# zmoon/crt1d

Hardware: AMD Instinct MI355X
Metric: (column x band) solves/sec at 60 layers (higher is better)
Workload: dtype f64

## Files before the change

crt1d_amd/_lib.py:

```python

import ctypes
import os

_HERE = os.path.dirname(os.path.abspath(__file__))
LIB_PATH = os.environ.get("CRT1D_HIP_LIB") or os.path.join(_HERE, "libcrt1d_hip.so")

SCHEME_IDS = {"2s": 0, "4s": 1, "n79": 2, "zq": 3, "bl": 4, "g77": 5, "bf": 6, "zq_pa": 7}
F32_SCHEMES = ("2s", "4s", "n79", "zq", "bl", "g77", "bf", "zq_pa")
TAU_D_METHODS = {"quad": 0, "9sky": 1}
NQ_TAU, NQ_G4, NQ_9SKY = 96, 32, 9
NQ = NQ_TAU + NQ_G4 + NQ_9SKY

FLAG_SKIP_PRECOMPUTE = 1
FLAG_PRECOMPUTE_ONLY = 2
FLAG_DIRECT_STORES = 4

MAX_LEVEL_SELECT = 64

CRT_OK = 0
CRT_ERR_BAD_ARG = -1
CRT_ERR_WORKSPACE = -2
CRT_ERR_UNSUPPORTED = -3
CRT_ERR_LAUNCH = -4
CRT_ERR_SHAPE = -5

_vp = ctypes.c_void_p


class CrtColumns(ctypes.Structure):
    _fields_ = [
        ("ncol", ctypes.c_int32),
        ("nz", ctypes.c_int32),
        ("psi", _vp),
        ("lai", _vp),
        ("mla", _vp),
        ("g_kind", _vp),
        ("g_param", _vp),
        ("g_at_psi", _vp),
        ("g_table", _vp),
    ]


class CrtBands(ctypes.Structure):
    _fields_ = [
        ("nb", ctypes.c_int32),
        ("col_stride", ctypes.c_int64),
        ("I_dr0", _vp),
        ("I_df0", _vp),
        ("leaf_r", _vp),
        ("leaf_t", _vp),
        ("soil_r", _vp),
    ]


class CrtSunSeries(ctypes.Structure):

    _fields_ = [
        ("nt", ctypes.c_int32),
        ("psi", _vp),
        ("g_at_psi", _vp),
        ("col_stride", ctypes.c_int64),
        ("I_dr0", _vp),
        ("I_df0", _vp),
    ]


class CrtSunSeriesF32(CrtSunSeries):
    """crt_sun_series_f32: the layout of crt_sun_series with float I_dr0 / I_df0 behind the pointers (crt_hip_levels_series_f32)."""


NTUNE = 16

TUNE_TILE_LDS = 0
TUNE_TILE_T = 1
TUNE_TILE_FLAGS = 2
TUNE_CLOSED_STORE_WAVES = 3
TUNE_CLOSED_PIPE_T = 4
TUNE_PACK = 5
TUNE_PACK_COMPUTE_WAVES = 6
TUNE_TRI_M = 8
TUNE_TRI_T = 9
TUNE_TRI_FAMILY = 10
TUNE_TRI_STORE_WAVES = 11
TUNE_MIN_TILE_NB = 12
TUNE_FLAT_FLUSH = 13
TUNE_K0_SEPARATE = 15
TILE_FLAG_SYNC_BARRIERS = 1
TILE_FLAG_GENERIC_FLUSH = 2
TILE_FLAG_NO_PIPELINE = 4
TILE_FLAG_NO_GENERIC_PIPELINE = 8
TILE_FLAG_FOUR_PAIR_STORE = 16
PACK_OFF = 1
PACK_FORCE = 2
TRI_FAMILY_NO_PIPELINE = 1
TRI_FAMILY_DOUBLE_BUFFERED = 2
TRI_FAMILY_REG_STAGED = 3
TRI_FAMILY_GENERIC_PIPELINE = 4
TRI_FAMILY_ZQPA_TWO_KERNEL = 1
TRI_FAMILY_ZQPA_PIPE = 5
TRI_FAMILY_ZQPA_PIPE2_DB = 6
TRI_FAMILY_ZQPA_PIPE2_RS = 7
FLAT_FLUSH_OFF = 1
FLAT_FLUSH_PART_LINE = 2
FLAT_FLUSH_WHOLE_LINE = 3


class CrtOptions(ctypes.Structure):
    _fields_ = [("mu_s", ctypes.c_double), ("tau_d_method", ctypes.c_int32), ("flags", ctypes.c_int32), ("tune", ctypes.c_int32 * NTUNE)]


def set_tune(opts, tune):
    for k in tune:
        if not isinstance(k, int) or not 0 <= k < NTUNE:
            raise ValueError(f"unknown crt_options.tune key {k!r}: keys are the TUNE_* constants, 0 .. {NTUNE - 1}")
    for k in range(NTUNE):
        opts.tune[k] = int(tune.get(k, 0))
    return opts


class CrtOutputs(ctypes.Structure):
    _fields_ = [(k, _vp) for k in ("I_dr", "I_df_d", "I_df_u", "F", "x0", "x1", "x2")]


class CrtBandsumOut(ctypes.Structure):

    _fields_ = [(k, _vp) for k in ("aI", "aI_sl", "aI_sh", "totals", "aI_dr", "I_dr", "I_df_d", "I_df_u", "F", "I_d")]


ABI_VERSION = 3


def _signatures():
    P = ctypes.POINTER
    i, i32, i64, sz, dbl, ok = ctypes.c_int, ctypes.c_int32, ctypes.c_int64, ctypes.c_size_t, ctypes.c_double, ctypes.c_int
    cols, bands, opts, outs, sums = P(CrtColumns), P(CrtBands), P(CrtOptions), P(CrtOutputs), P(CrtBandsumOut)
    solve = [cols, bands, opts, outs, _vp, sz, _vp]
    t = {
        "crt_hip_abi_version": (i, None),
        "crt_hip_strerror": (ctypes.c_char_p, [i]),
        "crt_hip_workspace_bytes": (sz, [i, i32, i32]),
        "crt_hip_workspace_bytes_nb": (sz, [i, i32, i32, i32]),
        "crt_hip_series_workspace_bytes": (sz, [i, i32, i32, i32, i32]),
        "crt_hip_levels_series_workspace_bytes": (sz, [i, i32, i32, i32]),
        "crt_hip_quad_nodes": (ok, [dbl, P(dbl)]),
        "crt_hip_integrated_series_f64": (ok, [i, cols, bands, P(CrtSunSeries), opts, _vp, i32, sums, _vp, sz, _vp]),
    }
    for suffix, sun_t in (("f64", CrtSunSeries), ("f32", CrtSunSeriesF32)):
        t[f"crt_hip_solve_{suffix}"] = (ok, [i] + solve)
        for s in SCHEME_IDS if suffix == "f64" else F32_SCHEMES:
            t[f"crt_hip_{s}_{suffix}"] = (ok, solve)
        t[f"crt_hip_absorb_{suffix}"] = (ok, [cols, bands, _vp, _vp, _vp, P(_vp), _vp, _vp, _vp])
        t[f"crt_hip_absorb_bandsum_{suffix}"] = (ok, [cols, bands, _vp, _vp, _vp, _vp, i32, _vp, _vp, _vp, _vp, _vp])
        t[f"crt_hip_absorb_bandsum2_{suffix}"] = (ok, [cols, bands, _vp, _vp, _vp, _vp, i32, sums, _vp])
        t[f"crt_hip_integrated_{suffix}"] = (ok, [i, cols, bands, opts, _vp, i32, _vp, _vp, _vp, _vp, _vp, sz, _vp])
        t[f"crt_hip_integrated2_{suffix}"] = (ok, [i, cols, bands, opts, _vp, i32, sums, _vp, sz, _vp])
        t[f"crt_hip_levels_{suffix}"] = (ok, [i, cols, bands, opts, P(i32), i32, outs, _vp, sz, _vp])
        t[f"crt_hip_levels_series_{suffix}"] = (ok, [i, cols, bands, P(sun_t), opts, P(i32), i32, outs, _vp, sz, _vp])
    t.update({
        "crt_hip_bandsum_finish_f64": (ok, [cols, i32, sums, _vp]),
        "crt_hip_band_reduce_f64": (ok, [_vp, i64, i32, _vp, i32, _vp, _vp]),
        "crt_hip_tau_d_f64": (ok, [_vp, _vp, i64, i32, _vp, _vp]),
        "crt_hip_smear_tuv_f64": (ok, [_vp, i64, i32, _vp, i32, _vp, i32, _vp, _vp]),
        "crt_hip_lai_beta_f64": (ok, [_vp, _vp, _vp, i32, i32, _vp, _vp, _vp, _vp]),
        "crt_hip_buffer_alloc_set": (ok, [i32, P(sz), P(_vp)]),
        "crt_hip_buffer_alloc": (ok, [sz, P(_vp)]),
        "crt_hip_buffer_free": (ok, [_vp]),
        "crt_hip_buffer_trim": (ok, []),
        "crt_hip_buffer_set_retain": (ok, [sz]),
        "crt_hip_buffer_describe": (ok, [_vp, ctypes.c_char_p, sz]),
        "crt_hip_buffer_stats": (ok, [P(i64)]),
        "crt_hip_last_kernel": (ctypes.c_char_p, []),
        "crt_hip_probe_fill_f64": (ok, [_vp, sz, dbl, _vp]),
        "crt_hip_probe_copy_f64": (ok, [_vp, _vp, sz, _vp]),
        "crt_hip_probe_store_set_f64": (ok, [P(_vp), i32, i64, i64, i32, dbl, _vp]),
        "crt_hip_probe_math_f64": (ok, [_vp, sz, _vp, _vp, _vp, _vp]),
    })
    return t


_SIGNATURES = _signatures()
EXPORTS = list(_SIGNATURES)

LEAF_NGL, LEAF_NMLA = 48, 64


def _leaf_signatures():
    dp, i32, dbl, ok = ctypes.POINTER(ctypes.c_double), ctypes.c_int32, ctypes.c_double, ctypes.c_int
    return {
        "crt_hip_leaf_pdf_nodes_f64": (ok, [dp, dp, dp, dp]),
        "crt_hip_g_from_pdf_f64": (ok, [_vp, _vp, i32, dbl, _vp, i32, _vp, _vp, _vp, _vp]),
    }


_LEAF_SIGNATURES = _leaf_signatures()
LEAF_EXPORTS = list(_LEAF_SIGNATURES)

LIGHT_UNIFORM, LIGHT_PLANCK, LIGHT_TABLE = 0, 1, 2
LIGHT_KINDS = {"uniform": LIGHT_UNIFORM, "planck": LIGHT_PLANCK, "table": LIGHT_TABLE}
SPECTRA_NGL = 16
SPECTRA_MAX_NB = 512
SPECTRA_MAX_ITEMS = 65536
SPECTRA_BLOCK = 512
SPECTRA_LDS_BYTES = 160 * 1024


def _spectra_signatures():
    dp, ip, i32, i64, dbl, ok = ctypes.POINTER(ctypes.c_double), ctypes.POINTER(ctypes.c_int32), ctypes.c_int32, ctypes.c_int64, ctypes.c_double, ctypes.c_int
    return {
        "crt_hip_planck_nodes_f64": (ok, [dp, dp]),
        "crt_hip_avg_optical_prop_f64": (ok, [_vp, i32, _vp, i32, _vp, i32, ip, i32, dbl, _vp, i32, _vp, i32, i32, _vp, _vp, _vp]),
        "crt_hip_bands_from_spectra_f64": (ok, [_vp, i32, _vp, i64, _vp, i64, _vp, i64, _vp, i32, _vp, i64, _vp, i64, i32, _vp, i32, ip, i32, dbl,
                                                _vp, _vp, _vp, _vp, _vp, _vp]),
    }


_SPECTRA_SIGNATURES = _spectra_signatures()
SPECTRA_EXPORTS = list(_SPECTRA_SIGNATURES)

MAX_SENSOR_BANDS = 64


class CrtSensorSet(ctypes.Structure):

    _fields_ = [("nsens", ctypes.c_int32), ("first", ctypes.POINTER(ctypes.c_int32)), ("count", ctypes.POINTER(ctypes.c_int32)), ("w", _vp)]


class CrtSensorOut(ctypes.Structure):
    _fields_ = [(k, _vp) for k in ("I_dr", "I_df_d", "I_df_u", "F")]


def _sensor_signatures():
    P = ctypes.POINTER
    i, i32, sz, ok = ctypes.c_int, ctypes.c_int32, ctypes.c_size_t, ctypes.c_int
    cols, bands, opts = P(CrtColumns), P(CrtBands), P(CrtOptions)
    tail = [opts, P(i32), i32, P(CrtSensorSet), P(CrtSensorOut), _vp, sz, _vp]
    return {
        "crt_hip_sensor_workspace_bytes": (sz, [i, i32, i32, i32, i32, i32]),
        "crt_hip_sensor_levels_f64": (ok, [i, cols, bands] + tail),
        "crt_hip_sensor_levels_f32": (ok, [i, cols, bands] + tail),
        "crt_hip_sensor_series_workspace_bytes": (sz, [i, i32, i32, i32, i32, i32, i32]),
        "crt_hip_sensor_levels_series_f64": (ok, [i, cols, bands, P(CrtSunSeries)] + tail),
    }


_SENSOR_SIGNATURES = _sensor_signatures()
SENSOR_EXPORTS = list(_SENSOR_SIGNATURES)

_lib = None


class HipLibraryMissing(RuntimeError):
    pass


def load():
    global _lib
    if _lib is not None:
        return _lib
    if not os.path.exists(LIB_PATH):
        raise HipLibraryMissing(
            f"{LIB_PATH} not found: the HIP kernels are not built. Run "
            "`python -c 'import __graft_entry__ as g; g.build()'` (or `make -C crt1d_amd/csrc`). "
            "crt1d_amd has no CPU fallback."
        )
    import torch

    lib = ctypes.CDLL(LIB_PATH)
    for name, (restype, argtypes) in {**_SIGNATURES, **_LEAF_SIGNATURES, **_SPECTRA_SIGNATURES, **_SENSOR_SIGNATURES}.items():
        f = getattr(lib, name)
        f.restype = restype
        if argtypes is not None:
            f.argtypes = argtypes
    if lib.crt_hip_abi_version() != ABI_VERSION:
        raise HipLibraryMissing(f"{LIB_PATH}: ABI version mismatch, rebuild")
    _lib = lib
    return lib


def strerror(status):
    return load().crt_hip_strerror(int(status)).decode()


def check(status, what):
    if status == CRT_OK:
        return
    msg = f"{what}: {strerror(status)} (status {status})"
    if status == CRT_ERR_SHAPE:
        raise AssertionError(msg)
    if status == CRT_ERR_BAD_ARG:
        raise ValueError(msg)
    raise RuntimeError(msg)


def quad_nodes(mu_s=0.501):
    import numpy as np

    buf = (ctypes.c_double * NQ)()
    check(load().crt_hip_quad_nodes(float(mu_s), buf), "crt_hip_quad_nodes")
    return np.frombuffer(buf, dtype=np.float64).copy()


def leaf_pdf_nodes():
    import numpy as np

    x, w = (ctypes.c_double * LEAF_NGL)(), (ctypes.c_double * LEAF_NGL)()
    xm, wm = (ctypes.c_double * LEAF_NMLA)(), (ctypes.c_double * LEAF_NMLA)()
    check(load().crt_hip_leaf_pdf_nodes_f64(x, w, xm, wm), "crt_hip_leaf_pdf_nodes_f64")
    return tuple(np.frombuffer(b, dtype=np.float64).copy() for b in (x, w, xm, wm))


def planck_nodes():
    import numpy as np

    x, w = (ctypes.c_double * SPECTRA_NGL)(), (ctypes.c_double * SPECTRA_NGL)()
    check(load().crt_hip_planck_nodes_f64(x, w), "crt_hip_planck_nodes_f64")
    return np.frombuffer(x, dtype=np.float64).copy(), np.frombuffer(w, dtype=np.float64).copy()
```

crt1d_amd/batched.py:

```python

import ctypes
import os
from dataclasses import dataclass
from typing import Optional

import torch

from . import _lib

SCHEMES = tuple(_lib.SCHEME_IDS)

OUT_KEYS = {
    "2s": ("I_dr", "I_df_d", "I_df_u", "F"),
    "4s": ("I_dr", "I_df_d", "I_df_u", "F"),
    "bl": ("I_dr", "I_df_d", "I_df_u", "F"),
    "n79": ("I_dr", "I_df_d", "I_df_u", "F", "aI_lsl", "aI_lsh"),
    "zq": ("I_dr", "I_df_d", "I_df_u", "F", "I_df_d_ss", "I_df_u_ss", "F_ss"),
    "g77": ("I_dr", "I_df_d", "I_df_u", "F", "aI_lsl", "aI_lsh", "aI_l"),
    "bf": ("I_dr", "I_df_d", "I_df_u", "F", "aI_lsl", "aI_lsh", "aI_l"),
    "zq_pa": ("I_dr", "I_df_d", "I_df_u", "F"),
}
_MID_KEYS = {"n79": ("aI_lsl", "aI_lsh")}


# ... 513 lines not shown
    def _tail(self):
        return (ctypes.byref(self._out),)


def solve(scheme, cols: Columns, bands: Bands, *, mu_s=0.501, tau_d_method="quad", out=None, workspace=None, placement="none"):
    with torch.cuda.device(cols.device):
        return Plan(scheme, cols, bands, mu_s=mu_s, tau_d_method=tau_d_method, out=out, workspace=workspace, placement=placement)()


def _io_suffix(bands):
    return "f32" if bands.dtype == torch.float32 else "f64"


def _check_epilogue_inputs(cols, bands, sol):
    _check_band_device(bands, cols.device)
    bands.col_stride(cols.ncol)
    cols.check_tables()
    for k in ("I_dr", "I_df_d", "I_df_u"):
        if k not in sol:
            raise ValueError(f"`sol` lacks {k!r}")
        if isinstance(sol[k], torch.Tensor) and sol[k].dtype != bands.dtype:
            raise TypeError(f"sol[{k!r}] is {sol[k].dtype} but the bands are {bands.dtype}: profiles and bands must share one storage type")
        _check_profile(sol[k], f"sol[{k!r}]", (cols.ncol, cols.nz, bands.nb), cols.device, bands.dtype)


BANDSUM_KEYS = ("aI", "aI_sl", "aI_sh", "totals")
PROFILE_KEYS = ("aI_dr", "I_dr", "I_df_d", "I_df_u", "F", "I_d")


def bandsum_shapes(ncol, nz, ngroup, profiles=False):
    sh = {"aI": (ncol, nz - 1, ngroup), "aI_sl": (ncol, nz - 1, ngroup), "aI_sh": (ncol, nz - 1, ngroup), "totals": (ncol, ngroup, 4)}
    if profiles:
        sh["aI_dr"] = (ncol, nz - 1, ngroup)
        for k in PROFILE_KEYS[1:]:
            sh[k] = (ncol, nz, ngroup)
    return sh


def _bandsum_out_struct(out, profiles):
    keys = BANDSUM_KEYS + (PROFILE_KEYS if profiles else ())
    return _lib.CrtBandsumOut(**{k: out[k].data_ptr() for k in keys})


def absorption_from_bandsums(res):
    return {"aI": res["aI"], "aI_dr": res["aI_dr"], "aI_df": res["aI"] - res["aI_dr"], "aI_sl": res["aI_sl"], "aI_sh": res["aI_sh"],
            "aI_df_sl": res["aI_sl"] - res["aI_dr"], "aI_df_sh": res["aI_sh"]}


class BandSumPlan:

    def __init__(self, cols: Columns, bands: Bands, sol, band_w, out=None, profiles=False):
        self.lib = _lib.load()
        ncol, nz, dev = cols.ncol, cols.nz, cols.device
        band_w = _band_weights(band_w, bands.nb, dev)
        ng = band_w.shape[0]
        _check_epilogue_inputs(cols, bands, sol)
        out = _outputs(bandsum_shapes(ncol, nz, ng, profiles), out, torch.float64, dev)
        self.cols, self.bands, self.sol, self.band_w, self.out, self.ng, self.profiles = cols, bands, sol, band_w, out, ng, profiles
        self._c, self._b = cols.c_struct(), bands.c_struct(ncol)
        self._o = _bandsum_out_struct(out, profiles)
        self._entry = f"crt_hip_absorb_bandsum2_{_io_suffix(bands)}"
        self._fn = getattr(self.lib, self._entry)

    def __call__(self, stream=None):
        dev = self.cols.device
        s = torch.cuda.current_stream(dev) if stream is None else stream
        sol = self.sol
        with torch.cuda.device(dev):
            st = self._fn(ctypes.byref(self._c), ctypes.byref(self._b), sol["I_dr"].data_ptr(), sol["I_df_d"].data_ptr(),
                          sol["I_df_u"].data_ptr(), self.band_w.data_ptr(), self.ng, ctypes.byref(self._o), s.cuda_stream)
        _lib.check(st, self._entry)
        return self.out


def absorb_bandsum(cols: Columns, bands: Bands, sol, band_w, out=None, profiles=False):
    return dict(BandSumPlan(cols, bands, sol, band_w, out=out, profiles=profiles)())


class BandSumFinishPlan:

    def __init__(self, cols: Columns, out):
        self.lib = _lib.load()
        ncol, nz, dev = cols.ncol, cols.nz, cols.device
        ng = out["aI"].shape[-1] if out["aI"].ndim == 3 else 0
        if not 1 <= ng <= 4:
            raise ValueError("out['aI'] must be (ncol, nz-1, ngroup <= 4)")
        for k, sh in bandsum_shapes(ncol, nz, ng, profiles=True).items():
            if k not in ("totals", "aI_dr"):
                _check_profile(out[k], f"out[{k!r}]", sh, dev)
        self.cols, self.out, self.ng = cols, out, ng
        self._c = cols.c_struct()
        self._o = _lib.CrtBandsumOut(**{k: out[k].data_ptr() for k in ("aI", "aI_sl", "aI_sh", "I_dr", "I_df_d", "I_df_u", "F", "I_d")})

    def __call__(self, stream=None):
        dev = self.cols.device
        s = torch.cuda.current_stream(dev) if stream is None else stream
        with torch.cuda.device(dev):
            st = self.lib.crt_hip_bandsum_finish_f64(ctypes.byref(self._c), self.ng, ctypes.byref(self._o), s.cuda_stream)
        _lib.check(st, "crt_hip_bandsum_finish_f64")
        return self.out


def bandsum_finish(cols: Columns, out):
    return BandSumFinishPlan(cols, out)()


ABSORPTION_KEYS = ("aI", "aI_df", "aI_dr", "aI_sh", "aI_sl", "aI_df_sl", "aI_df_sh")


def absorb(cols: Columns, bands: Bands, sol):
    lib = _lib.load()
    ncol, nz, nb = cols.ncol, cols.nz, bands.nb
    dev = cols.device
    _check_epilogue_inputs(cols, bands, sol)
    entry = f"crt_hip_absorb_{_io_suffix(bands)}"
    out = {k: torch.empty((ncol, nz - 1, nb), dtype=bands.dtype, device=dev) for k in ABSORPTION_KEYS}
    laim = torch.empty((ncol, nz - 1), dtype=torch.float64, device=dev)
    f_slm = torch.empty_like(laim)
    ptrs = (ctypes.c_void_p * 7)(*[out[k].data_ptr() for k in ABSORPTION_KEYS])
    c, b = cols.c_struct(), bands.c_struct(ncol)
    with torch.cuda.device(dev):
        st = getattr(lib, entry)(ctypes.byref(c), ctypes.byref(b), sol["I_dr"].data_ptr(), sol["I_df_d"].data_ptr(),
                                 sol["I_df_u"].data_ptr(), ptrs, laim.data_ptr(), f_slm.data_ptr(),
                                 torch.cuda.current_stream(dev).cuda_stream)
    _lib.check(st, entry)
    out["laim"] = laim
    out["f_slm"] = f_slm
    return out


class IntegratedPlan(_SolvePlan):

    _bad_scheme = "scheme {!r} has no integrated kernel"

    def __init__(self, scheme, cols: Columns, bands: Bands, band_w, *, mu_s=0.501, tau_d_method="quad", workspace=None, out=None,
                 profiles=False):
        self._check_options(scheme, tau_d_method)
        self._bind_sums(scheme, cols, bands, band_w, mu_s, tau_d_method, out, profiles)
        self._finish(f"crt_hip_integrated2_{_io_suffix(bands)}", workspace_bytes(scheme, cols.ncol, cols.nz, bands.nb), workspace)

    def _bind_sums(self, scheme, cols, bands, band_w, mu_s, tau_d_method, out, profiles, sun=None):
        self.band_w = _band_weights(band_w, bands.nb, cols.device)
        self._bind(scheme, cols, bands, mu_s, tau_d_method, sun=sun)
        ncol, nz, ng = cols.ncol, cols.nz, self.band_w.shape[0]
        shapes = bandsum_shapes(ncol, nz, ng, profiles) if sun is None else series_shapes(ncol, sun.nt, nz, ng, profiles)
        self.out = _outputs(shapes, out, torch.float64, cols.device)
        self.profiles = profiles
        self._out = _bandsum_out_struct(self.out, profiles)

    def _tail(self):
        return self.band_w.data_ptr(), self.band_w.shape[0], ctypes.byref(self._out)


def solve_integrated(scheme, cols: Columns, bands: Bands, band_w, **kw):
    with torch.cuda.device(cols.device):
        return IntegratedPlan(scheme, cols, bands, band_w, **kw)()


@dataclass
class SunSeries:

    psi: torch.Tensor
    I_dr0: torch.Tensor
    I_df0: torch.Tensor
    g_at_psi: Optional[torch.Tensor] = None

    _c_type = _lib.CrtSunSeries

    @staticmethod
    def _spectrum(t, name):
        return _f64(t, name)

    def __post_init__(self):
        self.psi = _f64(self.psi, "psi")
        if self.psi.ndim != 2 or self.psi.shape[1] < 1:
            raise ValueError("psi must be (ncol, nt) with nt >= 1")
        if self.g_at_psi is not None:
            self.g_at_psi = _f64(self.g_at_psi, "g_at_psi")
            if self.g_at_psi.shape != self.psi.shape:
                raise ValueError("g_at_psi must be (ncol, nt)")
        shape = None
        for name in ("I_dr0", "I_df0"):
            v = self._spectrum(getattr(self, name), name)
            if v.ndim == 2:
                v = v[None]
            if v.ndim != 3 or v.shape[1] != self.nt or v.shape[0] not in (1, self.ncol):
                raise ValueError(f"{name} must be (ncol, nt, nb) or (nt, nb) with ncol = {self.ncol}, nt = {self.nt}")
            if shape is None:
                shape = v.shape
            elif v.shape != shape:
                raise ValueError("I_dr0 and I_df0 must have the same shape")
            setattr(self, name, v)
        for name in ("I_dr0", "I_df0", "g_at_psi"):
            v = getattr(self, name)
            if v is not None and v.device != self.psi.device:
                raise ValueError(f"{name} lives on {v.device} but psi on {self.psi.device}")

    @property
    def ncol(self):
        return self.psi.shape[0]

    @property
    def nt(self):
        return self.psi.shape[1]

    @property
    def nb(self):
        return self.I_dr0.shape[2]

    @property
    def col_stride(self):
        return 0 if (self.I_dr0.shape[0] == 1 and self.ncol != 1) else self.nt * self.nb

    def slice(self, lo, hi):
        g = lambda t: t if t.shape[0] == 1 else t[lo:hi]
        return type(self)(self.psi[lo:hi], g(self.I_dr0), g(self.I_df0), None if self.g_at_psi is None else self.g_at_psi[lo:hi])

    def c_struct(self):
        return self._c_type(self.nt, self.psi.data_ptr(), None if self.g_at_psi is None else self.g_at_psi.data_ptr(), self.col_stride,
                                 self.I_dr0.data_ptr(), self.I_df0.data_ptr())

    @classmethod
    def from_host(cls, d, device="cuda"):
        t = _host_reader(d, device)
        return cls(t("psi"), t("I_dr0"), t("I_df0"), t("g_at_psi"))


def _check_sun(cols, bands, sun, f32_ok):
    ncol, nb, dev = cols.ncol, bands.nb, cols.device
    if bands.dtype != sun.I_dr0.dtype:
        if not f32_ok:
            raise TypeError("the sun-angle series has no f32 storage form: bands must be float64")
        want = "SunSeriesF32" if bands.dtype == torch.float32 else "SunSeries"
        raise TypeError(f"{bands.dtype} bands need a {want}: the spectra of sun are {sun.I_dr0.dtype}")
    if sun.ncol != ncol or sun.nb != nb:
        raise ValueError(f"sun must have ncol = {ncol} rows and nb = {nb} bands, got {sun.ncol} and {sun.nb}")
    if sun.psi.device != dev:
        raise ValueError(f"sun lives on {sun.psi.device} but the columns on {dev}")
    if bands.leaf_r is None or bands.leaf_t is None:
        raise ValueError("bands needs leaf_r and leaf_t")
    if (cols.g_table is not None or cols.g_at_psi is not None) and sun.g_at_psi is None and bool((cols.g_kind == 6).any()):
        raise ValueError("columns with g_kind = G_TABLE need sun.g_at_psi (ncol, nt)")
    if cols.g_table is None and bool((cols.g_kind == 6).any()):
        raise ValueError("columns with g_kind = G_TABLE need g_table")


@dataclass
class SunSeriesF32(SunSeries):

    _c_type = _lib.CrtSunSeriesF32

    @staticmethod
    def _spectrum(t, name):
        return _f32(t, name)

    @classmethod
    def from_host(cls, d, device="cuda"):
        t = _host_reader(d, device)
        return cls(t("psi"), t("I_dr0").to(torch.float32), t("I_df0").to(torch.float32), t("g_at_psi"))


def series_workspace_bytes(scheme, ncol, nz, nb, nt):
    return int(_lib.load().crt_hip_series_workspace_bytes(_lib.SCHEME_IDS[scheme], ncol, nz, nb, nt))


def series_shapes(ncol, nt, nz, ngroup, profiles=False):
    return {k: (sh[0], nt) + tuple(sh[1:]) for k, sh in bandsum_shapes(ncol, nz, ngroup, profiles).items()}


class IntegratedSeriesPlan(IntegratedPlan):

    def __init__(self, scheme, cols: Columns, bands: Bands, sun: SunSeries, band_w, *, mu_s=0.501, tau_d_method="quad", workspace=None,
                 out=None, profiles=False):
        self._check_options(scheme, tau_d_method)
        if not isinstance(sun, SunSeries) or isinstance(sun, SunSeriesF32):
            raise TypeError("sun must be a SunSeries (float64 spectra)")
        self._bind_sums(scheme, cols, bands, band_w, mu_s, tau_d_method, out, profiles, sun=sun)
        self._finish("crt_hip_integrated_series_f64", series_workspace_bytes(scheme, cols.ncol, cols.nz, bands.nb, sun.nt), workspace)


def solve_integrated_series(scheme, cols: Columns, bands: Bands, sun: SunSeries, band_w, **kw):
    with torch.cuda.device(cols.device):
        return IntegratedSeriesPlan(scheme, cols, bands, sun, band_w, **kw)()


LEVEL_KEYS = ("I_dr", "I_df_d", "I_df_u", "F")


def normalize_levels(levels, nz):
    import operator

    if hasattr(levels, "tolist"):
        levels = levels.tolist()
    if not hasattr(levels, "__iter__"):
        levels = [levels]
    try:
        raw = [operator.index(v) for v in levels]
    except TypeError as e:
        raise ValueError(f"levels must be integers: {e}") from None
    if not raw:
        raise ValueError("levels is empty: select at least one level")
    out = []
    for v in raw:
        if not -nz <= v < nz:
            raise ValueError(f"level {v} is out of range for nz = {nz} (valid: {-nz} .. {nz - 1})")
        out.append(v + nz if v < 0 else v)
# ... 235 lines not shown
```

crt1d_amd/csrc/api.hip:

```cpp
#include <math.h>

#include <algorithm>
#include <cstring>

#include "epilogue.hpp"

namespace crt {
namespace {

__global__ __launch_bounds__(256) void k_probe_math(const double* x, size_t n, double* e, double* sn, double* cs) {
  const size_t i = (size_t)blockIdx.x * 256 + threadIdx.x;
  if (i >= n) return;
  e[i] = fexp(x[i]);
  double s_, c_;
  fast_sincos(x[i], s_, c_);
  sn[i] = s_;
  cs[i] = c_;
}

__global__ __launch_bounds__(256) void k_fill(d2* dst, size_t n2, double v) {
  d2 t;
  t.x = v;
  t.y = v;
  for (size_t i = (size_t)blockIdx.x * 256 + threadIdx.x; i < n2; i += (size_t)gridDim.x * 256)
    __builtin_nontemporal_store(t, dst + i);
}

__global__ __launch_bounds__(256) void k_copy(d2* dst, const d2* src, size_t n2) {
  for (size_t i = (size_t)blockIdx.x * 256 + threadIdx.x; i < n2; i += (size_t)gridDim.x * 256)
    __builtin_nontemporal_store(__builtin_nontemporal_load(src + i), dst + i);
}

struct StoreSetArgs {
  double* p[8];
  int na;
  long long ncol, col;
  int run;
};
__global__ __launch_bounds__(192) void k_store_set(StoreSetArgs a, double v) {
  d2 t;
  t.x = v;
  t.y = v;
  const long long c = blockIdx.x;
  const long long base = c * a.col;
  for (long long r0 = 0; r0 < a.col; r0 += a.run) {
    const int n2 = (int)(min((long long)a.run, a.col - r0) >> 1);
    for (int k = 0; k < a.na; ++k) {
      d2* dst = reinterpret_cast<d2*>(a.p[k] + base + r0);
      for (int i = threadIdx.x; i < n2; i += 192) __builtin_nontemporal_store(t, dst + i);
    }
  }
}

bool scheme_ok(int s) { return s >= 0 && s < CRT_NUM_SCHEMES; }

}
}

using namespace crt;

static int bandsum_nopt(const crt_bandsum_out& o) {
  const int n = (o.aI_dr != nullptr) + (o.I_dr != nullptr) + (o.I_df_d != nullptr) + (o.I_df_u != nullptr) + (o.F != nullptr) + (o.I_d != nullptr);
  return n == 0 || n == 6 ? n : -1;
}

static crt_bandsum_out bandsum_out4(double* aI, double* aI_sl, double* aI_sh, double* totals) {
  crt_bandsum_out o = {};
  o.aI = aI;
  o.aI_sl = aI_sl;
  o.aI_sh = aI_sh;
  o.totals = totals;
  return o;
}

template <typename TIO>
static int bandsum_impl(const crt_columns* cols, int32_t nb, int64_t col_stride, const TIO* leaf_r, const TIO* leaf_t, const TIO* I_dr,
                        const TIO* I_df_d, const TIO* I_df_u, const double* band_w, int32_t ngroup, const crt_bandsum_out* out,
                        crt_stream_t stream) {
  if (!cols || !I_dr || !I_df_d || !I_df_u || !band_w || !out || !out->aI || !out->aI_sl || !out->aI_sh) return CRT_ERR_BAD_ARG;
  if (bandsum_nopt(*out) < 0) return CRT_ERR_BAD_ARG;
  if (cols->ncol <= 0 || cols->nz < 2 || nb <= 0 || ngroup <= 0 || ngroup > MAXG) return CRT_ERR_BAD_ARG;
  if (!cols->psi || !cols->lai || !cols->g_kind || !leaf_r || !leaf_t) return CRT_ERR_BAD_ARG;
  EpiArgsT<TIO> a;
  a.ncol = cols->ncol;
  a.nb = nb;
  a.nz = cols->nz;
  a.ngroup = ngroup;
  a.col_stride = col_stride;
  a.psi = cols->psi;
  a.lai = cols->lai;
  a.g_kind = cols->g_kind;
  a.g_param = cols->g_param;
  a.g_at_psi = cols->g_at_psi;
  a.leaf_r = leaf_r;
  a.leaf_t = leaf_t;
  a.I_dr = I_dr;
  a.I_df_d = I_df_d;
  a.I_df_u = I_df_u;
  a.band_w = band_w;
  a.aI = out->aI;
  a.aI_sl = out->aI_sl;
  a.aI_sh = out->aI_sh;
  a.totals = out->totals;
  a.aI_dr = out->aI_dr;
  a.L_dr = out->I_dr;
  a.L_dn = out->I_df_d;
  a.L_up = out->I_df_u;
  a.L_F = out->F;
  a.L_Id = out->I_d;
  return launch_bandsum(a, static_cast<hipStream_t>(stream));
}

template <typename TIO>
static int absorb_impl(const crt_columns* cols, int32_t nb, int64_t col_stride, const TIO* leaf_r, const TIO* leaf_t, const TIO* I_dr,
                       const TIO* I_df_d, const TIO* I_df_u, TIO* const* out7, double* laim, double* f_slm, crt_stream_t stream) {
  if (!cols || !I_dr || !I_df_d || !I_df_u || !out7 || !laim || !f_slm) return CRT_ERR_BAD_ARG;
  if (cols->ncol <= 0 || cols->nz < 2 || nb <= 0) return CRT_ERR_BAD_ARG;
  if (!cols->psi || !cols->lai || !cols->g_kind || !leaf_r || !leaf_t) return CRT_ERR_BAD_ARG;
  AbsArgsT<TIO> a;
  a.ncol = cols->ncol;
  a.nb = nb;
  a.nz = cols->nz;
  a.col_stride = col_stride;
  a.psi = cols->psi;
  a.lai = cols->lai;
  a.g_kind = cols->g_kind;
  a.g_param = cols->g_param;
  a.g_at_psi = cols->g_at_psi;
  a.leaf_r = leaf_r;
  a.leaf_t = leaf_t;
  a.I_dr = I_dr;
  a.I_df_d = I_df_d;
  a.I_df_u = I_df_u;
  for (int i = 0; i < 7; ++i) {
    if (!out7[i]) return CRT_ERR_BAD_ARG;
    a.o[i] = out7[i];
  }
  a.laim = laim;
  a.f_slm = f_slm;
  return launch_absorb(a, static_cast<hipStream_t>(stream));
}

extern "C" {

int crt_hip_abi_version(void) { return CRT_ABI_VERSION; }

const char* crt_hip_strerror(int st) {
  switch (st) {
    case CRT_OK: return "ok";
    case CRT_ERR_BAD_ARG: return "bad argument (null pointer, non-positive size or invalid option)";
    case CRT_ERR_WORKSPACE: return "workspace too small (see crt_hip_workspace_bytes)";
    case CRT_ERR_UNSUPPORTED: return "shape not supported by the gfx950 kernels (nz too large for LDS, or grid overflow)";
    case CRT_ERR_LAUNCH: return "HIP runtime / launch error";
    case CRT_ERR_SHAPE: return "shape violates a reference assertion";
    default: return "unknown status";
  }
}
// ... 40 lines not shown
  int method = CRT_TAU_D_QUAD, flags = 0;
  int32_t tune[CRT_NTUNE] = {};
};

static bool is_tri(int scheme) { return scheme == CRT_SCHEME_N79 || scheme == CRT_SCHEME_ZQ; }

static int check_solve(int scheme, const crt_columns* cols, const crt_bands* bands, const crt_options* opts, const crt_outputs* out,
                       const void* workspace, size_t workspace_bytes, const IntArgs* integ, const LevArgs* lev, const crt_sun_series* ser,
                       SolveOpts& o, size_t extra_ws = 0) {
  if (!scheme_ok(scheme) || !cols || !bands || !out) return CRT_ERR_BAD_ARG;
  const int ncol = cols->ncol, nz = cols->nz, nb = bands->nb;
  if (ncol <= 0 || nz <= 0 || nb <= 0) return CRT_ERR_BAD_ARG;
  if (!cols->lai || !cols->g_kind) return CRT_ERR_BAD_ARG;
  if (scheme == CRT_SCHEME_2S && !cols->mla) return CRT_ERR_BAD_ARG;
  if (!bands->leaf_r || !bands->leaf_t) return CRT_ERR_BAD_ARG;
  if (ser) {
    if ((!integ && !lev) || !ser->psi || !ser->I_dr0 || !ser->I_df0 || ser->nt < 1) return CRT_ERR_BAD_ARG;
    if (ser->col_stride != 0 && ser->col_stride < (int64_t)ser->nt * nb) return CRT_ERR_BAD_ARG;
    if (cols->g_table && !ser->g_at_psi) return CRT_ERR_BAD_ARG;
  } else if (!cols->psi || !bands->I_dr0 || !bands->I_df0) {
    return CRT_ERR_BAD_ARG;
  }
  if (scheme != CRT_SCHEME_BL && !bands->soil_r) return CRT_ERR_BAD_ARG;
  if (bands->col_stride != 0 && bands->col_stride < nb) return CRT_ERR_BAD_ARG;
  if (!integ && !lev) {
    if (!out->I_dr || !out->I_df_d || !out->I_df_u || !out->F) return CRT_ERR_BAD_ARG;
    const int nextra = scheme == CRT_SCHEME_N79 ? 2 : (scheme == CRT_SCHEME_ZQ || scheme == CRT_SCHEME_G77 || scheme == CRT_SCHEME_BF) ? 3 : 0;
    if (nextra >= 1 && !out->x0) return CRT_ERR_BAD_ARG;
    if (nextra >= 2 && !out->x1) return CRT_ERR_BAD_ARG;
    if (nextra >= 3 && !out->x2) return CRT_ERR_BAD_ARG;
  }
  if (nz < 2) return CRT_ERR_SHAPE;
  if (scheme == CRT_SCHEME_N79 && nz < 3) return CRT_ERR_SHAPE;
  if (opts) {
    o.mu_s = opts->mu_s;
    o.method = opts->tau_d_method;
    o.flags = opts->flags;
    std::memcpy(o.tune, opts->tune, sizeof o.tune);
  }
  {
    static const struct { int key, lo, hi, step; } accepted[] = {
        {CRT_TUNE_TILE_LDS, 1, 160 * 1024, 1},           {CRT_TUNE_TILE_T, 1, 64, 1},
        {CRT_TUNE_TILE_FLAGS, 1, 255, 1},                {CRT_TUNE_CLOSED_STORE_WAVES, 1, 12, 1},
        {CRT_TUNE_CLOSED_PIPE_T, 1, 32, 1},              {CRT_TUNE_PACK, CRT_PACK_OFF, CRT_PACK_FORCE, 1},
        {CRT_TUNE_PACK_COMPUTE_WAVES, 1, 4, 1},          {CRT_TUNE_TRI_M, 8, 16, 4},
        {CRT_TUNE_TRI_T, 4, 12, 4},                      {CRT_TUNE_TRI_FAMILY, 1, CRT_TRI_FAMILY_ZQPA_PIPE2_RS, 1},
        {CRT_TUNE_TRI_STORE_WAVES, 1, 12, 1},            {CRT_TUNE_MIN_TILE_NB, 1, 1024, 1},
        {CRT_TUNE_FLAT_FLUSH, CRT_FLAT_FLUSH_OFF, CRT_FLAT_FLUSH_WHOLE_LINE, 1}, {CRT_TUNE_K0_SEPARATE, 1, 1, 1}};
    bool known[CRT_NTUNE] = {};
    for (const auto& r : accepted) {
      const int v = o.tune[r.key];
      known[r.key] = true;
      if (v != 0 && (v < r.lo || v > r.hi || (v - r.lo) % r.step != 0)) return CRT_ERR_BAD_ARG;
    }
    for (int i = 0; i < CRT_NTUNE; ++i)
      if (!known[i] && o.tune[i] != 0) return CRT_ERR_BAD_ARG;
  }
  if (scheme == CRT_SCHEME_4S && !(o.mu_s > 0.0 && o.mu_s < 1.0)) return CRT_ERR_BAD_ARG;
  if (o.method != CRT_TAU_D_QUAD && o.method != CRT_TAU_D_9SKY) return CRT_ERR_BAD_ARG;
  const size_t need = !ser ? crt_hip_workspace_bytes_nb(scheme, ncol, nz, nb)
                      : lev ? crt_hip_levels_series_workspace_bytes(scheme, ncol, nz, ser->nt)
                            : crt_hip_series_workspace_bytes(scheme, ncol, nz, nb, ser->nt);
  if (need == 0 || extra_ws > SIZE_MAX - need) return CRT_ERR_UNSUPPORTED;
  if (!workspace || workspace_bytes < need + extra_ws) return CRT_ERR_WORKSPACE;
  if (ser && integ && nb > 1024) return CRT_ERR_UNSUPPORTED;
  if (ser && lev && (long long)ncol * ser->nt > 0x7fffffffLL) return CRT_ERR_UNSUPPORTED;
  return CRT_OK;
}

static void build_args(int scheme, const crt_columns* cols, const crt_bands* bands, const crt_outputs* out, void* workspace, int f32,
                       const SolveOpts& o, ColArgs& ca, SolveArgs& sa) {
  ca = {cols->ncol, cols->nz, scheme, o.method, o.mu_s, cols->psi, cols->lai, cols->mla, cols->g_kind, cols->g_param, cols->g_at_psi,
        cols->g_table, static_cast<double*>(workspace)};
  sa = {};
  sa.ncol = cols->ncol;
  sa.nb = bands->nb;
  sa.nz = cols->nz;
  sa.reclen = rec_len(scheme, cols->nz);
  sa.col_stride = bands->col_stride;
  sa.ws = static_cast<const double*>(workspace);
  sa.I_dr0 = bands->I_dr0;
  sa.I_df0 = bands->I_df0;
  sa.leaf_r = bands->leaf_r;
  sa.leaf_t = bands->leaf_t;
  sa.soil_r = bands->soil_r;
  void* const o7[7] = {out->I_dr, out->I_df_d, out->I_df_u, out->F, out->x0, out->x1, out->x2};
  std::memcpy(sa.o, o7, sizeof sa.o);
  sa.mu_s = o.mu_s;
  sa.f32 = f32;
  std::memcpy(&sa.tune, o.tune, sizeof sa.tune);
}

static int dispatch_series(int scheme, ColArgs ca, SolveArgs sa, int flags, const IntArgs* integ, const LevArgs* lev, const crt_sun_series* ser,
                           hipStream_t s, SensLaunch* sl) {
  double* const sunrec = ca.ws + (size_t)ca.ncol * can_len(scheme, ca.nz);
  ca.psi = ser->psi;
  ca.g_at_psi = ser->g_at_psi;
  sa.I_dr0 = sa.I_df0 = nullptr;
  const SeriesArgs sr = {ser->nt, scheme, ca.nz, can_len(scheme, ca.nz), sun_len(scheme, ca.nz), sa.ws, sunrec, ser->col_stride, ser->I_dr0, ser->I_df0};
  const bool tri = is_tri(scheme);
  auto lev_series = [&](bool probe) {
    if (scheme == CRT_SCHEME_ZQ_PA) return launch_zqpa_lev(sa, *lev, s, &sr, probe, sl);
    return tri ? launch_tridiag_lev(scheme, sa, *lev, s, &sr, probe, sl) : launch_closed_lev(scheme, sa, *lev, s, &sr, probe, sl);
  };
  if (lev) {
    const int st = lev_series(true);
    if (st != CRT_OK) return st;
  }
  const int st = (flags & CRT_FLAG_SKIP_PRECOMPUTE) ? init_quadrature(s) : launch_colpre_series(ca, ser->nt, sunrec, s);
  if (st != CRT_OK) return st;
  if (flags & CRT_FLAG_PRECOMPUTE_ONLY) {
    note_kernel("k_colpre<canopy> + k_colsun nt=%d", ser->nt);
    return CRT_OK;
  }
  if (lev) return lev_series(false);
  if (scheme == CRT_SCHEME_ZQ_PA) return launch_zqpa_int(sa, *integ, s, &sr);
  return tri ? launch_tridiag_int(scheme, sa, *integ, s, &sr) : launch_closed_int(scheme, sa, *integ, s, &sr);
}

static int dispatch_step(int scheme, const ColArgs& ca, const SolveArgs& sa, int flags, const IntArgs* integ, const LevArgs* lev, hipStream_t s,
                         SensLaunch* sl) {
  const bool tri = is_tri(scheme);
  auto lev_step = [&](bool probe) {
    if (scheme == CRT_SCHEME_ZQ_PA) return launch_zqpa_lev(sa, *lev, s, nullptr, probe, sl);
    return tri ? launch_tridiag_lev(scheme, sa, *lev, s, nullptr, probe, sl) : launch_closed_lev(scheme, sa, *lev, s, nullptr, probe, sl);
  };
  if (sl) {
    const int st = lev_step(true);
    if (st != CRT_OK) return st;
  }
  const bool k0_in_solve = scheme == CRT_SCHEME_2S && !integ && !lev && !(flags & (CRT_FLAG_SKIP_PRECOMPUTE | CRT_FLAG_PRECOMPUTE_ONLY)) &&
                           sa.tune.k0_separate == 0;
  if (k0_in_solve) {
    const int st = init_quadrature(s);
    if (st != CRT_OK) return st;
  } else if (!(flags & CRT_FLAG_SKIP_PRECOMPUTE)) {
    const int st = launch_colpre(ca, s);
    if (st != CRT_OK) return st;
  }
  if (flags & CRT_FLAG_PRECOMPUTE_ONLY) return CRT_OK;
  if (integ) {
    if (scheme == CRT_SCHEME_ZQ_PA) return launch_zqpa_int(sa, *integ, s);
    return tri ? launch_tridiag_int(scheme, sa, *integ, s) : launch_closed_int(scheme, sa, *integ, s);
  }
  if (lev) return lev_step(false);
  if (scheme == CRT_SCHEME_ZQ_PA) return launch_zqpa(sa, ca.ws + (size_t)sa.ncol * sa.reclen, s);
  const int force = (flags & CRT_FLAG_DIRECT_STORES) ? 1 : 0;
  return tri ? launch_tridiag(scheme, sa, s, force) : launch_closed(scheme, sa, s, force, k0_in_solve ? &ca : nullptr);
}

static int solve_impl(int scheme, const crt_columns* cols, const crt_bands* bands, const crt_options* opts,
                      const crt_outputs* out, void* workspace, size_t workspace_bytes, crt_stream_t stream, int f32,
                      const IntArgs* integ = nullptr, const LevArgs* lev = nullptr, const crt_sun_series* ser = nullptr,
                      SensLaunch* sl = nullptr, size_t extra_ws = 0) {
  SolveOpts o;
  if (const int st = check_solve(scheme, cols, bands, opts, out, workspace, workspace_bytes, integ, lev, ser, o, extra_ws)) return st;
  ColArgs ca;
  SolveArgs sa;
  build_args(scheme, cols, bands, out, workspace, f32, o, ca, sa);
  hipStream_t s = static_cast<hipStream_t>(stream);
  return ser ? dispatch_series(scheme, ca, sa, o.flags, integ, lev, ser, s, sl) : dispatch_step(scheme, ca, sa, o.flags, integ, lev, s, sl);
}

int crt_hip_solve_f64(int scheme, const crt_columns* cols, const crt_bands* bands, const crt_options* opts,
                      const crt_outputs* out, void* workspace, size_t workspace_bytes, crt_stream_t stream) {
  return solve_impl(scheme, cols, bands, opts, out, workspace, workspace_bytes, stream, 0);
}

int crt_hip_solve_f32(int scheme, const crt_columns* cols, const crt_bands_f32* bands, const crt_options* opts,
                      const crt_outputs_f32* out, void* workspace, size_t workspace_bytes, crt_stream_t stream) {
  static_assert(sizeof(crt_bands_f32) == sizeof(crt_bands) && sizeof(crt_outputs_f32) == sizeof(crt_outputs), "layout");
  return solve_impl(scheme, cols, reinterpret_cast<const crt_bands*>(bands), opts, reinterpret_cast<const crt_outputs*>(out), workspace,
                    workspace_bytes, stream, 1);
}

#define CRT_ENTRY(name, id)                                                                                        \
  int name(const crt_columns* c, const crt_bands* b, const crt_options* o, const crt_outputs* out, void* ws,       \
           size_t wsb, crt_stream_t s) {                                                                           \
    return crt_hip_solve_f64(id, c, b, o, out, ws, wsb, s);                                                        \
  }
CRT_ENTRY(crt_hip_2s_f64, CRT_SCHEME_2S)
CRT_ENTRY(crt_hip_4s_f64, CRT_SCHEME_4S)
CRT_ENTRY(crt_hip_n79_f64, CRT_SCHEME_N79)
CRT_ENTRY(crt_hip_zq_f64, CRT_SCHEME_ZQ)
CRT_ENTRY(crt_hip_bl_f64, CRT_SCHEME_BL)
CRT_ENTRY(crt_hip_g77_f64, CRT_SCHEME_G77)
CRT_ENTRY(crt_hip_bf_f64, CRT_SCHEME_BF)
CRT_ENTRY(crt_hip_zq_pa_f64, CRT_SCHEME_ZQ_PA)
#undef CRT_ENTRY

#define CRT_ENTRY32(name, id)                                                                                      \
  int name(const crt_columns* c, const crt_bands_f32* b, const crt_options* o, const crt_outputs_f32* out, void* ws, \
           size_t wsb, crt_stream_t s) {                                                                           \
    return crt_hip_solve_f32(id, c, b, o, out, ws, wsb, s);                                                        \
  }
CRT_ENTRY32(crt_hip_2s_f32, CRT_SCHEME_2S)
CRT_ENTRY32(crt_hip_4s_f32, CRT_SCHEME_4S)
CRT_ENTRY32(crt_hip_n79_f32, CRT_SCHEME_N79)
CRT_ENTRY32(crt_hip_zq_f32, CRT_SCHEME_ZQ)
CRT_ENTRY32(crt_hip_bl_f32, CRT_SCHEME_BL)
CRT_ENTRY32(crt_hip_g77_f32, CRT_SCHEME_G77)
CRT_ENTRY32(crt_hip_bf_f32, CRT_SCHEME_BF)
CRT_ENTRY32(crt_hip_zq_pa_f32, CRT_SCHEME_ZQ_PA)
#undef CRT_ENTRY32

int crt_hip_absorb_bandsum2_f64(const crt_columns* cols, const crt_bands* bands, const double* I_dr, const double* I_df_d,
                                const double* I_df_u, const double* band_w, int32_t ngroup, const crt_bandsum_out* out, crt_stream_t stream) {
  if (!bands) return CRT_ERR_BAD_ARG;
  return bandsum_impl<double>(cols, bands->nb, bands->col_stride, bands->leaf_r, bands->leaf_t, I_dr, I_df_d, I_df_u, band_w, ngroup, out,
                              stream);
}

int crt_hip_absorb_bandsum2_f32(const crt_columns* cols, const crt_bands_f32* bands, const float* I_dr, const float* I_df_d,
                                const float* I_df_u, const double* band_w, int32_t ngroup, const crt_bandsum_out* out, crt_stream_t stream) {
  if (!bands) return CRT_ERR_BAD_ARG;
  return bandsum_impl<float>(cols, bands->nb, bands->col_stride, bands->leaf_r, bands->leaf_t, I_dr, I_df_d, I_df_u, band_w, ngroup, out,
                             stream);
}

int crt_hip_absorb_bandsum_f64(const crt_columns* cols, const crt_bands* bands, const double* I_dr, const double* I_df_d,
                               const double* I_df_u, const double* band_w, int32_t ngroup, double* aI, double* aI_sl,
                               double* aI_sh, double* totals, crt_stream_t stream) {
  const crt_bandsum_out o = bandsum_out4(aI, aI_sl, aI_sh, totals);
  return crt_hip_absorb_bandsum2_f64(cols, bands, I_dr, I_df_d, I_df_u, band_w, ngroup, &o, stream);
}

int crt_hip_absorb_bandsum_f32(const crt_columns* cols, const crt_bands_f32* bands, const float* I_dr, const float* I_df_d,
                               const float* I_df_u, const double* band_w, int32_t ngroup, double* aI, double* aI_sl,
                               double* aI_sh, double* totals, crt_stream_t stream) {
  const crt_bandsum_out o = bandsum_out4(aI, aI_sl, aI_sh, totals);
  return crt_hip_absorb_bandsum2_f32(cols, bands, I_dr, I_df_d, I_df_u, band_w, ngroup, &o, stream);
}

static int integrated_impl(int scheme, const crt_columns* cols, const crt_bands* bands, const crt_options* opts, const double* band_w,
                           int32_t ngroup, const crt_bandsum_out* out, void* workspace, size_t workspace_bytes, crt_stream_t stream, int f32,
                           const crt_sun_series* ser = nullptr) {
  if (!band_w || !out || !out->aI || !out->aI_sl || !out->aI_sh || ngroup <= 0 || ngroup > INT_MAXG || !cols) return CRT_ERR_BAD_ARG;
  if (bandsum_nopt(*out) < 0) return CRT_ERR_BAD_ARG;
  IntArgs ia;
  ia.lai = cols->lai;
  ia.band_w = band_w;
  ia.ngroup = ngroup;
  ia.aI = out->aI;
  ia.aI_sl = out->aI_sl;
  ia.aI_sh = out->aI_sh;
  ia.totals = out->totals;
  ia.aI_dr = out->aI_dr;
  ia.L_dr = out->I_dr;
  ia.L_dn = out->I_df_d;
  ia.L_up = out->I_df_u;
  ia.L_F = out->F;
  ia.L_Id = out->I_d;
  crt_outputs none = {};
  return solve_impl(scheme, cols, bands, opts, &none, workspace, workspace_bytes, stream, f32, &ia, nullptr, ser);
}

int crt_hip_integrated_series_f64(int scheme, const crt_columns* cols, const crt_bands* bands, const crt_sun_series* sun,
                                  const crt_options* opts, const double* band_w, int32_t ngroup, const crt_bandsum_out* out, void* workspace,
                                  size_t workspace_bytes, crt_stream_t stream) {
  if (!sun) return CRT_ERR_BAD_ARG;
  return integrated_impl(scheme, cols, bands, opts, band_w, ngroup, out, workspace, workspace_bytes, stream, 0, sun);
}

int crt_hip_integrated2_f64(int scheme, const crt_columns* cols, const crt_bands* bands, const crt_options* opts,
                            const double* band_w, int32_t ngroup, const crt_bandsum_out* out, void* workspace, size_t workspace_bytes,
                            crt_stream_t stream) {
  return integrated_impl(scheme, cols, bands, opts, band_w, ngroup, out, workspace, workspace_bytes, stream, 0);
}

int crt_hip_integrated2_f32(int scheme, const crt_columns* cols, const crt_bands_f32* bands, const crt_options* opts,
                            const double* band_w, int32_t ngroup, const crt_bandsum_out* out, void* workspace, size_t workspace_bytes,
                            crt_stream_t stream) {
  return integrated_impl(scheme, cols, reinterpret_cast<const crt_bands*>(bands), opts, band_w, ngroup, out, workspace, workspace_bytes,
                         stream, 1);
}

int crt_hip_integrated_f64(int scheme, const crt_columns* cols, const crt_bands* bands, const crt_options* opts,
                           const double* band_w, int32_t ngroup, double* aI, double* aI_sl, double* aI_sh, double* totals,
                           void* workspace, size_t workspace_bytes, crt_stream_t stream) {
  const crt_bandsum_out o = bandsum_out4(aI, aI_sl, aI_sh, totals);
  return crt_hip_integrated2_f64(scheme, cols, bands, opts, band_w, ngroup, &o, workspace, workspace_bytes, stream);
}

int crt_hip_integrated_f32(int scheme, const crt_columns* cols, const crt_bands_f32* bands, const crt_options* opts,
                           const double* band_w, int32_t ngroup, double* aI, double* aI_sl, double* aI_sh, double* totals,
                           void* workspace, size_t workspace_bytes, crt_stream_t stream) {
  const crt_bandsum_out o = bandsum_out4(aI, aI_sl, aI_sh, totals);
  return crt_hip_integrated2_f32(scheme, cols, bands, opts, band_w, ngroup, &o, workspace, workspace_bytes, stream);
}

static int levels_impl(int scheme, const crt_columns* cols, const crt_bands* bands, const crt_options* opts, const int32_t* levels,
                       int32_t nsel, const crt_outputs* out, void* workspace, size_t workspace_bytes, crt_stream_t stream, int f32,
                       const crt_sun_series* ser = nullptr, SensLaunch* sl = nullptr, size_t extra_ws = 0) {
  if (!scheme_ok(scheme) || !cols || !levels || !out) return CRT_ERR_BAD_ARG;
  if (nsel < 1 || nsel > CRT_MAX_LEVEL_SELECT) return CRT_ERR_BAD_ARG;
  if (out->x0 || out->x1 || out->x2) return CRT_ERR_BAD_ARG;
  if (!sl && !out->I_dr && !out->I_df_d && !out->I_df_u && !out->F) return CRT_ERR_BAD_ARG;
  LevArgs la = {};
  la.o[0] = out->I_dr;
  la.o[1] = out->I_df_d;
  la.o[2] = out->I_df_u;
  la.o[3] = out->F;
  la.nsel = nsel;
  for (int r = 0; r < nsel; ++r) {
    if (levels[r] < 0 || levels[r] >= cols->nz) return CRT_ERR_BAD_ARG;
    if (r > 0 && levels[r] <= levels[r - 1]) return CRT_ERR_BAD_ARG;
    la.lev[r] = levels[r];
  }
  crt_outputs none = {};
  return solve_impl(scheme, cols, bands, opts, &none, workspace, workspace_bytes, stream, f32, nullptr, &la, ser, sl, extra_ws);
}

int crt_hip_levels_series_f64(int scheme, const crt_columns* cols, const crt_bands* bands, const crt_sun_series* sun, const crt_options* opts,
                              const int32_t* levels, int32_t nsel, const crt_outputs* out, void* workspace, size_t workspace_bytes,
                              crt_stream_t stream) {
  if (!sun) return CRT_ERR_BAD_ARG;
  return levels_impl(scheme, cols, bands, opts, levels, nsel, out, workspace, workspace_bytes, stream, 0, sun);
}

int crt_hip_levels_series_f32(int scheme, const crt_columns* cols, const crt_bands_f32* bands, const crt_sun_series_f32* sun,
                              const crt_options* opts, const int32_t* levels, int32_t nsel, const crt_outputs_f32* out, void* workspace,
                              size_t workspace_bytes, crt_stream_t stream) {
  static_assert(sizeof(crt_sun_series_f32) == sizeof(crt_sun_series) && offsetof(crt_sun_series_f32, I_dr0) == offsetof(crt_sun_series, I_dr0) &&
                    offsetof(crt_sun_series_f32, I_df0) == offsetof(crt_sun_series, I_df0) &&
                    offsetof(crt_sun_series_f32, col_stride) == offsetof(crt_sun_series, col_stride),
                "layout");
  if (!sun) return CRT_ERR_BAD_ARG;
  return levels_impl(scheme, cols, reinterpret_cast<const crt_bands*>(bands), opts, levels, nsel, reinterpret_cast<const crt_outputs*>(out),
                     workspace, workspace_bytes, stream, 1, reinterpret_cast<const crt_sun_series*>(sun));
}

int crt_hip_levels_f64(int scheme, const crt_columns* cols, const crt_bands* bands, const crt_options* opts, const int32_t* levels,
                       int32_t nsel, const crt_outputs* out, void* workspace, size_t workspace_bytes, crt_stream_t stream) {
  return levels_impl(scheme, cols, bands, opts, levels, nsel, out, workspace, workspace_bytes, stream, 0);
}

int crt_hip_levels_f32(int scheme, const crt_columns* cols, const crt_bands_f32* bands, const crt_options* opts, const int32_t* levels,
                       int32_t nsel, const crt_outputs_f32* out, void* workspace, size_t workspace_bytes, crt_stream_t stream) {
  return levels_impl(scheme, cols, reinterpret_cast<const crt_bands*>(bands), opts, levels, nsel, reinterpret_cast<const crt_outputs*>(out),
                     workspace, workspace_bytes, stream, 1);
}


static size_t sens_partial_bytes(int scheme, int32_t ncol, int32_t nz, int32_t nb, int32_t nt, int32_t nsel, int32_t nsens) {
  if (!scheme_ok(scheme) || ncol <= 0 || nz <= 0 || nb <= 0 || nt < 1 || nsel < 1 || nsel > CRT_MAX_LEVEL_SELECT || nsens < 1 ||
      nsens > CRT_MAX_SENSOR_BANDS)
    return 0;
  SolveArgs sa = {};
  sa.ncol = ncol;
  sa.nb = nb;
  sa.nz = nz;
  sa.reclen = rec_len(scheme, nz);
  LevArgs la = {};
  la.nsel = nsel;
  SensLaunch sl = {};
  const int st = scheme == CRT_SCHEME_ZQ_PA ? launch_zqpa_lev(sa, la, nullptr, nullptr, true, &sl)
                 : is_tri(scheme)           ? launch_tridiag_lev(scheme, sa, la, nullptr, nullptr, true, &sl)
                                            : launch_closed_lev(scheme, sa, la, nullptr, nullptr, true, &sl);
  if (st != CRT_OK || sl.nslice <= 1) return 0;
  const size_t per = (size_t)sl.nslice * (size_t)nsel * 4 * (size_t)nsens * sizeof(double);
  const size_t nv = (size_t)ncol * (size_t)nt;
  return nv > SIZE_MAX / per ? 0 : nv * per;
}

size_t crt_hip_sensor_workspace_bytes(int scheme, int32_t ncol, int32_t nz, int32_t nb, int32_t nsel, int32_t nsens) {
  const size_t rec = crt_hip_workspace_bytes_nb(scheme, ncol, nz, nb);
  return rec == 0 ? 0 : rec + sens_partial_bytes(scheme, ncol, nz, nb, 1, nsel, nsens);
}

size_t crt_hip_sensor_series_workspace_bytes(int scheme, int32_t ncol, int32_t nz, int32_t nb, int32_t nt, int32_t nsel, int32_t nsens) {
  const size_t rec = crt_hip_levels_series_workspace_bytes(scheme, ncol, nz, nt);
  return rec == 0 || nb <= 0 ? 0 : rec + sens_partial_bytes(scheme, ncol, nz, nb, nt, nsel, nsens);
}

static int sensor_impl(int scheme, const crt_columns* cols, const crt_bands* bands, const crt_options* opts, const int32_t* levels, int32_t nsel,
                       const crt_sensor_set* sensors, const crt_sensor_out* out, void* workspace, size_t workspace_bytes, crt_stream_t stream,
                       int f32, const crt_sun_series* ser = nullptr) {
  if (!scheme_ok(scheme) || !cols || !bands || !sensors || !out) return CRT_ERR_BAD_ARG;
  if (!sensors->first || !sensors->count || !sensors->w) return CRT_ERR_BAD_ARG;
  const int nsens = sensors->nsens, nb = bands->nb;
  if (nsens < 1 || nsens > CRT_MAX_SENSOR_BANDS || nb <= 0) return CRT_ERR_BAD_ARG;
  if (!out->I_dr && !out->I_df_d && !out->I_df_u && !out->F) return CRT_ERR_BAD_ARG;
  SensLaunch sl = {};
  SensArgs& sn = sl.sn;
// ... 134 lines not shown
```

crt1d_amd/csrc/crt_internal.hpp:

```cpp
#pragma once
#include <hip/hip_runtime.h>
#include <math.h>
#include <stddef.h>
#include <stdint.h>

#include <type_traits>

#include "crt1d_hip.h"
#include "crt1d_hip_sensor.h"

namespace crt {

enum RecScalar {
  S_KB = 0,
  S_MU = 1,
  S_G = 2,
  S_MUBAR = 3,
  S_GINT1 = 4,
  S_GINT2 = 5,
  S_DLM = 6,
  S_TAUI = 7,
  S_TPSI = 8,
  S_COS2 = 9,
  S_LT = 10,
// ... 204 lines not shown
  q = fma_vvs(q, r, 0x1.5555555553d68p-5);
  q = fma_vvs(q, r, 0x1.5555555555556p-3);
  q = fma_vvs(q, r, 0x1.0000000000001p-1);
  q = __builtin_fma(q, r, 1.0);
  q = __builtin_fma(q, r, 1.0);
  return __builtin_ldexp(q, (int)k);
}

__device__ __forceinline__ double fexpm1(double x) {
  if (__builtin_fabs(x) > 0.34657359027997264) return fexp(x) - 1.0;
  double q = fma_vvs(x, 0x1.af389ecfc4b9cp-26, 0x1.28917c89a43a7p-22);
  q = fma_vvs(q, x, 0x1.71de0db2f6b19p-19);
  q = fma_vvs(q, x, 0x1.a019b9149a41cp-16);
  q = fma_vvs(q, x, 0x1.a01a01a7c2efep-13);
  q = fma_vvs(q, x, 0x1.6c16c17889ef1p-10);
  q = fma_vvs(q, x, 0x1.11111111109b5p-7);
  q = fma_vvs(q, x, 0x1.5555555553d68p-5);
  q = fma_vvs(q, x, 0x1.5555555555556p-3);
  q = fma_vvs(q, x, 0x1.0000000000001p-1);
  return __builtin_fma(x * x, q, x);
}

__device__ inline void fast_sincos(double th, double& sn, double& cs) {
  const double k = __builtin_rint(mul_vs(th, 0.63661977236758134308));
  double r = fma_vsv(k, -1.57079632679489655800e+00, th);
  r = fma_vsv(k, -6.12323399573676603587e-17, r);
  const double z = r * r;
  double ps = fma_vvs(z, 1.58969099521155010221e-10, -2.50507602534068634195e-08);
  ps = fma_vvs(z, ps, 2.75573137070700676789e-06);
  ps = fma_vvs(z, ps, -1.98412698298579493134e-04);
  ps = fma_vvs(z, ps, 8.33333333332248946124e-03);
  ps = fma_vvs(z, ps, -1.66666666666666324348e-01);
  const double sr = __builtin_fma(z * r, ps, r);
  double pc = fma_vvs(z, -1.13596475577881948265e-11, 2.08757232129817482790e-09);
  pc = fma_vvs(z, pc, -2.75573143513906633035e-07);
  pc = fma_vvs(z, pc, 2.48015872894767294178e-05);
  pc = fma_vvs(z, pc, -1.38888888888741095749e-03);
  pc = fma_vvs(z, pc, 4.16666666666666019037e-02);
  const double cr = __builtin_fma(z * z, pc, __builtin_fma(-0.5, z, 1.0));
  const int n = (int)k;
  const bool swap = (n & 1) != 0;
  const double ss = swap ? cr : sr, cc = swap ? sr : cr;
  sn = (n & 2) ? -ss : ss;
  cs = ((n + 1) & 2) ? -cc : cc;
}

__device__ inline bool exact_level(int j) { return (j & 7) == 0; }

constexpr int INT_MAXG = 4;

struct IntArgs {
  const double* lai;
  const double* band_w;
  int ngroup;
  double* aI;
  double* aI_sl;
  double* aI_sh;
  double* totals;
  double* aI_dr;
  double* L_dr;
  double* L_dn;
  double* L_up;
  double* L_F;
  double* L_Id;
};

template <int CTRL>
__device__ inline double dpp_add(double v) {
  const int lo = __builtin_amdgcn_update_dpp(0, __double2loint(v), CTRL, 0xf, 0xf, false);
  const int hi = __builtin_amdgcn_update_dpp(0, __double2hiint(v), CTRL, 0xf, 0xf, false);
  return v + __hiloint2double(hi, lo);
}
__device__ inline double row_sum16(double v) {
  v = dpp_add<0xB1>(v);
  v = dpp_add<0x4E>(v);
  v = dpp_add<0x141>(v);
  v = dpp_add<0x140>(v);
  return v;
}
template <int CTRL, int ROW_MASK>
__device__ inline double dpp_add_rows(double v) {
  const int lo = __builtin_amdgcn_update_dpp(0, __double2loint(v), CTRL, ROW_MASK, 0xf, false);
  const int hi = __builtin_amdgcn_update_dpp(0, __double2hiint(v), CTRL, ROW_MASK, 0xf, false);
  return v + __hiloint2double(hi, lo);
}
__device__ inline double wave_sum_lane63(double v) {
  v = row_sum16(v);
  v = dpp_add_rows<0x142, 0xA>(v);
  v = dpp_add_rows<0x143, 0xC>(v);
  return v;
}
__device__ inline double swap_add32(double x, double y) {
  const auto lo = __builtin_amdgcn_permlane32_swap(__double2loint(x), __double2loint(y), false, false);
  const auto hi = __builtin_amdgcn_permlane32_swap(__double2hiint(x), __double2hiint(y), false, false);
  return __hiloint2double(hi[0], lo[0]) + __hiloint2double(hi[1], lo[1]);
}
__device__ inline double swap_add16(double x, double y) {
  const auto lo = __builtin_amdgcn_permlane16_swap(__double2loint(x), __double2loint(y), false, false);
  const auto hi = __builtin_amdgcn_permlane16_swap(__double2hiint(x), __double2hiint(y), false, false);
  return __hiloint2double(hi[0], lo[0]) + __hiloint2double(hi[1], lo[1]);
}
__device__ inline double wave_sum4(double a, double b, double c, double d) {
  return row_sum16(swap_add16(swap_add32(a, b), swap_add32(c, d)));
}
__device__ inline int wave_sum4_slot(int row) { return ((row & 1) << 1) | (row >> 1); }
template <int N>
__device__ inline void wave_sum_store(const double (&v)[N], double* dst, int nvalid, int lane) {
  const int slot = wave_sum4_slot(lane >> 4);
#pragma unroll
  for (int j = 0; j < (N + 3) / 4; ++j) {
    const double z = wave_sum4(v[4 * j], 4 * j + 1 < N ? v[4 * j + 1] : 0.0, 4 * j + 2 < N ? v[4 * j + 2] : 0.0, 4 * j + 3 < N ? v[4 * j + 3] : 0.0);
    const int idx = 4 * j + slot;
    if ((lane & 15) == 0 && idx < nvalid) dst[idx] = z;
  }
}

__device__ inline double half_sum2(double x, double y) { return row_sum16(swap_add16(x, y)); }
template <int N>
__device__ inline void half_sum_store(const double (&v)[N], double* dst, int nvalid, int lane) {
  const int which = (lane >> 4) & 1;
#pragma unroll
  for (int j = 0; j < (N + 1) / 2; ++j) {
    const double z = half_sum2(v[2 * j], 2 * j + 1 < N ? v[2 * j + 1] : 0.0);
    const int idx = 2 * j + which;
    if ((lane & 15) == 0 && idx < nvalid) dst[idx] = z;
  }
}

__device__ inline double wave_sum_all(double v) {
#pragma unroll
  for (int off = 32; off > 0; off >>= 1) v += __shfl_xor(v, off, 64);
  return v;
}

struct IntLds {
  double* part;
  double* ends;
  double* pdr;
  double* lev;
  double* pi0;
};
__device__ inline IntLds int_lds_carve(double* base, int nz, int nwave, bool prof) {
  IntLds L;
  L.part = base;
  L.ends = L.part + (size_t)nz * nwave * INT_MAXG;
  L.pdr = L.ends + (size_t)2 * nwave * 2 * INT_MAXG;
  L.lev = L.pdr + (size_t)nwave * INT_MAXG;
  L.pi0 = L.lev + (prof ? (size_t)nz * nwave * 2 * INT_MAXG : 0);
  return L;
}

template <bool ROWS, bool PROF = false>
__device__ inline void int_accumulate(const IntLds& L, int nwave, int wave, int lane, int nz, int j, int ng, const double (&w)[INT_MAXG],
                                      bool active, double idr, double dn, double up) {
  if constexpr (!ROWS) {
    if constexpr (PROF) {
      const int g2 = wave_sum4_slot(lane >> 4);
      const double dd = active ? dn : 0.0, uu = active ? up : 0.0;
      const double zd = wave_sum4(w[0] * dd, w[1] * dd, w[2] * dd, w[3] * dd);
      const double zu = wave_sum4(w[0] * uu, w[1] * uu, w[2] * uu, w[3] * uu);
      if ((lane & 15) == 0 && g2 < ng) {
        L.lev[((j * nwave + wave) * 2 + 0) * INT_MAXG + g2] = zd;
        L.lev[((j * nwave + wave) * 2 + 1) * INT_MAXG + g2] = zu;
      }
    }
    const int g = wave_sum4_slot(lane >> 4);
    const bool writer = (lane & 15) == 0 && g < ng;
    const double net = active ? idr + dn - up : 0.0;
    const double z = wave_sum4(w[0] * net, w[1] * net, w[2] * net, w[3] * net);
    if (writer) L.part[(j * nwave + wave) * INT_MAXG + g] = z;
    if (j == 0 || j == nz - 1) {
      const int e = j == 0 ? 0 : 1;
      const double dd = active ? idr + dn : 0.0, uu = active ? up : 0.0;
      const double z0 = wave_sum4(w[0] * dd, w[1] * dd, w[2] * dd, w[3] * dd);
      const double z1 = wave_sum4(w[0] * uu, w[1] * uu, w[2] * uu, w[3] * uu);
      if (writer) {
        L.ends[((e * nwave + wave) * 2 + 0) * INT_MAXG + g] = z0;
        L.ends[((e * nwave + wave) * 2 + 1) * INT_MAXG + g] = z1;
      }
    }
    return;
  }
  const int nslot = ROWS ? nwave * 4 : nwave;
  const int slot = ROWS ? wave * 4 + (lane >> 4) : wave;
  const bool writer = ROWS ? (lane & 15) == 0 : lane == 63;
  auto red = [](double v) { return ROWS ? row_sum16(v) : wave_sum_lane63(v); };
  const double net = active ? idr + dn - up : 0.0;
#pragma unroll
  for (int g = 0; g < INT_MAXG; ++g)
    if (g < ng) {
      const double t = red(w[g] * net);
      if (writer) L.part[(j * nslot + slot) * INT_MAXG + g] = t;
    }
  if (j == 0 || j == nz - 1) {
    const int e = j == 0 ? 0 : 1;
#pragma unroll
    for (int g = 0; g < INT_MAXG; ++g)
      if (g < ng) {
        const double t0 = red(active ? w[g] * (idr + dn) : 0.0);
        const double t1 = red(active ? w[g] * up : 0.0);
        if (writer) {
          L.ends[((e * nslot + slot) * 2 + 0) * INT_MAXG + g] = t0;
          L.ends[((e * nslot + slot) * 2 + 1) * INT_MAXG + g] = t1;
        }
      }
  }
}

template <bool ROWS, bool PROF = false>
__device__ inline void int_finish(const IntLds& L, const IntArgs& ia, int nwave, int nz, int c, double Kb, double invmu = 0.0) {
  __syncthreads();
  if constexpr (PROF) {
    const int ngp = ia.ngroup;
    for (int i = threadIdx.x; i < nz * ngp; i += blockDim.x) {
      const int j = i / ngp, g = i - j * ngp;
      double p0 = 0.0, sD = 0.0, sU = 0.0;
      for (int wv = 0; wv < nwave; ++wv) {
        p0 += L.pi0[wv * INT_MAXG + g];
        sD += L.lev[((j * nwave + wv) * 2 + 0) * INT_MAXG + g];
        sU += L.lev[((j * nwave + wv) * 2 + 1) * INT_MAXG + g];
      }
      const double sR = exp(-Kb * ia.lai[(long long)c * nz + j]) * p0;
      const long long o = ((long long)c * nz + j) * ngp + g;
      ia.L_dr[o] = sR;
      ia.L_dn[o] = sD;
      ia.L_up[o] = sU;
      ia.L_F[o] = sR * invmu + 2 * (sU + sD);
      ia.L_Id[o] = sR + sD;
    }
  }
  const int ng = ia.ngroup, nrow = ROWS ? nwave * 4 : nwave;
  const double* lai = ia.lai + (long long)c * nz;
  for (int i = threadIdx.x; i < (nz - 1) * ng; i += blockDim.x) {
    const int k = i / ng, g = i - k * ng;
    double p0 = 0.0, p1 = 0.0, pd = 0.0;
    for (int r = 0; r < nrow; ++r) {
      p0 += L.part[(k * nrow + r) * INT_MAXG + g];
      p1 += L.part[((k + 1) * nrow + r) * INT_MAXG + g];
    }
    for (int wv = 0; wv < nwave; ++wv) pd += L.pdr[wv * INT_MAXG + g];
    const double dl = lai[k] - lai[k + 1];
    const double fsl = exp(-Kb * ((lai[k] + lai[k + 1]) / 2));
    const double adr = (1 - exp(-Kb * dl)) * exp(-Kb * lai[k + 1]) * pd;
    const double a = p1 - p0;
    const double adf = a - adr;
    const long long o = ((long long)c * (nz - 1) + k) * ng + g;
    ia.aI[o] = a;
    ia.aI_sl[o] = adf * fsl + adr;
    ia.aI_sh[o] = adf * (1 - fsl);
    if constexpr (PROF) ia.aI_dr[o] = adr;
  }
  if (ia.totals) {
    for (int i = threadIdx.x; i < ng * 4; i += blockDim.x) {
      const int g = i >> 2, q = i & 3;
      const int e = q < 2 ? 1 : 0, which = q & 1;
      double t = 0.0;
      for (int r = 0; r < nrow; ++r) t += L.ends[((e * nrow + r) * 2 + which) * INT_MAXG + g];
      ia.totals[((long long)c * ng + g) * 4 + q] = t;
    }
  }
}

__host__ __device__ inline size_t int_lds_doubles(int nz, int nwave, bool rows = false, bool prof = false) {
  const size_t nslot = rows ? (size_t)nwave * 4 : (size_t)nwave;
  return (size_t)nz * nslot * INT_MAXG + 2 * nslot * 2 * INT_MAXG + (size_t)nwave * INT_MAXG +
         (prof ? (size_t)nz * nwave * 2 * INT_MAXG + (size_t)nwave * INT_MAXG : 0);
}

constexpr int SUN_HDR = 8;
constexpr int SER_XI = 104;
__host__ __device__ inline int sun_nvec(int scheme) {
  switch (scheme) {
    case CRT_SCHEME_N79: return 5;
    case CRT_SCHEME_ZQ_PA: return 2;
    default: return 1;
  }
}
__host__ __device__ inline int sun_vec_slot(int scheme, int sv) {
  switch (scheme) {
    case CRT_SCHEME_N79: return sv < 2 ? sv : sv + 1;
    case CRT_SCHEME_ZQ: return 0;
    case CRT_SCHEME_ZQ_PA: return sv;
    default: return 1;
  }
}
__host__ __device__ inline int sun_len(int scheme, int nz) { return SUN_HDR + sun_nvec(scheme) * nz; }
__host__ __device__ inline int can_len(int scheme, int nz) { return rec_len(scheme, nz) + (scheme == CRT_SCHEME_ZQ_PA ? SER_XI : 0); }
__device__ inline int sun_hdr_slot(int i) { return i == 0 ? S_KB : i == 1 ? S_MU : i == 2 ? S_G : i == 3 ? S_INVMU : S_TPSI; }

__host__ __device__ inline int rec_vec_sun(int scheme, int vec) {
  switch (scheme) {
    case CRT_SCHEME_N79: return vec < 2 ? vec : (vec >= 3 && vec <= 5) ? vec - 1 : -1;
    case CRT_SCHEME_ZQ: return vec == 0 ? 0 : -1;
    case CRT_SCHEME_ZQ_PA: return vec < 2 ? vec : -1;
    default: return vec == 1 ? 0 : -1;
  }
}

struct SeriesArgs {
  int nt, scheme, nz;
  int canlen, sunlen;
  const double* can;
  const double* sun;
  long long col_stride;
  const void* I_dr0;
  const void* I_df0;
};

int launch_colpre_series(const ColArgs& ca, int nt, double* sun, hipStream_t s);

inline dim3 series_grid(int ncol, int nt) {
  const unsigned gy = nt < 65535 ? (unsigned)nt : 65535u;
  return dim3((unsigned)ncol, gy, (unsigned)((nt + (long long)gy - 1) / gy));
}

inline void gauss_unit(int n, double* x, double* w) {
  for (int i = 0; i < (n + 1) / 2; ++i) {
    double z = cos(3.14159265358979323846 * (i + 0.75) / (n + 0.5)), pp = 1.0;
    for (int it = 0; it < 100; ++it) {
      double p1 = 1.0, p2 = 0.0;
      for (int j = 0; j < n; ++j) {
        const double p3 = p2;
        p2 = p1;
        p1 = ((2.0 * j + 1.0) * z * p2 - j * p3) / (j + 1.0);
      }
      pp = n * (z * p1 - p2) / (z * z - 1.0);
      const double dz = p1 / pp;
      z -= dz;
      if (fabs(dz) < 1e-16) break;
    }
    const double wt = 2.0 / ((1.0 - z * z) * pp * pp);
    x[i] = 0.5 * (1.0 - z);
    x[n - 1 - i] = 0.5 * (1.0 + z);
    w[i] = w[n - 1 - i] = 0.5 * wt;
  }
}

template <class K, class... Args>
inline int launch_kernel(K kern, dim3 grid, int nthr, size_t sh, hipStream_t s, Args... args) {
  if (sh > 64 * 1024 &&
      hipFuncSetAttribute(reinterpret_cast<const void*>(kern), hipFuncAttributeMaxDynamicSharedMemorySize, (int)sh) != hipSuccess)
    return (int)CRT_ERR_LAUNCH;
  hipLaunchKernelGGL(kern, grid, dim3(nthr), sh, s, args...);
  return hipGetLastError() == hipSuccess ? (int)CRT_OK : (int)CRT_ERR_LAUNCH;
}

__device__ __forceinline__ void series_assemble(const SeriesArgs& sr, int reclen, int c, long long v, double* lds) {
  const int tid = threadIdx.x, nthr = blockDim.x, nz = sr.nz;
  {
    const double* can = sr.can + (long long)c * sr.canlen;
    const double* sun = sr.sun + v * sr.sunlen;
    if (tid < REC_HDR) {
      int si = -1;
#pragma unroll
      for (int i = 0; i < 5; ++i)
        if (sun_hdr_slot(i) == tid) si = i;
      lds[tid] = si >= 0 ? sun[si] : can[tid];
    }
    const int nvec = (reclen - REC_HDR) / nz;
    for (int vec = 0; vec < nvec; ++vec) {
      const int sv = rec_vec_sun(sr.scheme, vec);
      const double* src = sv >= 0 ? sun + SUN_HDR + sv * nz : can + REC_HDR + vec * nz;
      for (int j = tid; j < nz; j += nthr) lds[REC_HDR + vec * nz + j] = src[j];
    }
  }
  __syncthreads();
}

template <class Body>
__device__ __forceinline__ void series_step(const SolveArgs& a, const IntArgs& ia, const SeriesArgs& sr, double* lds, Body body) {
  const int c = blockIdx.x, nz = sr.nz, ng = ia.ngroup;
  const long long tl = (long long)blockIdx.z * gridDim.y + blockIdx.y;
  if (tl >= sr.nt) return;
  const int t = (int)tl;
  const long long v = (long long)c * sr.nt + t;
  series_assemble(sr, a.reclen, c, v, lds);
  SolveArgs at = a;
  IntArgs it = ia;
  const long long din = (long long)c * sr.col_stride + (long long)t * a.nb - (long long)c * a.col_stride;
  at.I_dr0 = static_cast<const double*>(sr.I_dr0) + din;
  at.I_df0 = static_cast<const double*>(sr.I_df0) + din;
  const long long sh = v - c, sa = sh * (nz - 1) * ng, sl = sh * nz * ng;
  it.aI += sa;
  it.aI_sl += sa;
  it.aI_sh += sa;
  if (it.totals) it.totals += sh * ng * 4;
  if (it.L_dr) {
    it.aI_dr += sa;
    it.L_dr += sl;
    it.L_dn += sl;
    it.L_up += sl;
    it.L_F += sl;
    it.L_Id += sl;
  }
  body(at, it);
}

int launch_closed_int(int scheme, const SolveArgs& a, const IntArgs& ia, hipStream_t s, const SeriesArgs* sr = nullptr);
int launch_tridiag_int(int scheme, const SolveArgs& a, const IntArgs& ia, hipStream_t s, const SeriesArgs* sr = nullptr);

struct LevArgs {
  void* o[4];
  int nsel;
  int32_t lev[CRT_MAX_LEVEL_SELECT];
};

struct LevSlices {
  int nslice, per, nthr;
};
inline LevSlices lev_slices(int nb, int wmax) {
  LevSlices ls;
  ls.nslice = (nb + wmax - 1) / wmax;
  ls.per = (nb + ls.nslice - 1) / ls.nslice;
  ls.nthr = ((ls.per + 63) / 64) * 64;
  return ls;
}

inline bool lev_series_grid(int ncol, int nt, int nslice, dim3* grid) {
  const unsigned gy = nt < 65535 ? (unsigned)nt : 65535u;
// ... 130 lines not shown
```

crt1d_amd/csrc/solve_closed.hip:

```cpp
#include <algorithm>
#include <type_traits>

#include "col_record.hpp"

namespace crt {
namespace {

constexpr double PI = 3.14159265358979323846;

struct BandIn {
  double I_dr0, I_df0, r, t, s;
};

template <int MODE>
__device__ __forceinline__ bool exact_here(bool unif, int j) {
  if constexpr (MODE == 0) return true;
  if constexpr (MODE == 1) return exact_level(j);
  return !unif || exact_level(j);
}

template <typename TIO>
__device__ inline BandIn load_band(const SolveArgs& a, int c, int b, bool need_soil) {
  const long long i = (long long)c * a.col_stride + b;
  BandIn in;
// ... 391 lines not shown
        p4 = fexp(-lam2 * (LT - x));
      } else {
        p2 = E1L * fast_rcp(p1);
        p4 = E2L * fast_rcp(p3);
      }
      if (osc) fast_sincos(lam2 * x, p4, p3);
    } else {
      p1 *= q1p;
      p2 *= q1m;
      if (osc) {
        const double c = p3 * q2a + p4 * q2b;
        p4 = p4 * q2a - p3 * q2b;
        p3 = c;
      } else {
        p3 *= q2a;
        p4 *= q2b;
      }
    }
    const double dn = __builtin_fma(d[0], p1, __builtin_fma(d[1], p2, __builtin_fma(d[2], p3, __builtin_fma(d[3], p4, d[4] * eK))));
    const double up = __builtin_fma(u[0], p1, __builtin_fma(u[1], p2, __builtin_fma(u[2], p3, __builtin_fma(u[3], p4, u[4] * eK))));
    const double idr = I0 * eK;
    o[0] = idr;
    o[1] = dn;
    o[2] = up;
    o[3] = __builtin_fma(idr, invmu, 2 * (up + dn));
  }
};

constexpr int DBLOCK = 256;

template <class S, typename TIO, int VEC, bool USE_LDS>
__global__ __launch_bounds__(DBLOCK) void k_direct(SolveArgs a) {
  extern __shared__ double lds[];
  const Item it = locate<DBLOCK, VEC>(a.ncol, a.nb);
  const double* rec = stage_records<DBLOCK, VEC, USE_LDS>(a, it, lds);
  if (!it.active) return;
  S st[VEC];
#pragma unroll
  for (int v = 0; v < VEC; ++v) st[v].init(rec, load_band<TIO>(a, it.c, it.b + v, S::SOIL), a);
  const int nz = a.nz;
  long long o = ((long long)it.c * nz) * a.nb + it.b;
  for (int j = 0; j < nz; ++j, o += a.nb) {
    double val[VEC][S::NARR];
#pragma unroll
    for (int v = 0; v < VEC; ++v) st[v].level(j, rec, nz, val[v]);
#pragma unroll
    for (int k = 0; k < S::NARR; ++k) {
      double pk[VEC];
#pragma unroll
      for (int v = 0; v < VEC; ++v) pk[v] = val[v][k];
      store_stream<TIO, VEC>(outp<TIO>(a.o[k]) + o, pk);
    }
  }
}

struct TileCfg {
  int CB;
  int T;
  int rec_dbl;
  int flags;
};


template <class S, typename TIO, int MAXT, bool FUSED>
__global__ __launch_bounds__(MAXT) void k_tile(SolveArgs a, TileCfg cfg) {
  constexpr int VW = 16 / (int)sizeof(TIO);
  typedef TIO vt __attribute__((ext_vector_type(VW)));
  extern __shared__ double lds[];
  const int nb = a.nb, nz = a.nz, CB = cfg.CB, T = cfg.T;
  const int tid = threadIdx.x, nthr = blockDim.x;
  const int c0 = blockIdx.x * CB;
  const int ncb = min(CB, a.ncol - c0);
  const int cl = tid / nb, b = tid - cl * nb;
  const bool active = cl < ncb;
  BandIn bin = {};
  if (active) bin = load_band<TIO>(a, c0 + cl, b, S::SOIL);
  {
    const double* src = a.ws + (long long)c0 * a.reclen;
    const int n = ncb * a.reclen;
    for (int i = tid; i < n; i += nthr) lds[i] = src[i];
  }
  __syncthreads();
  TIO* tile = reinterpret_cast<TIO*>(lds + cfg.rec_dbl);
  const double* rec = lds + (active ? cl : 0) * a.reclen;
  S st;
  if (active) st.init(rec, bin, a);
  const int colrun = T * nb;
  const int nbv = nb / VW;
  const int f_toff = FUSED ? tid / nbv : 0;
  const int f_p = FUSED ? tid - f_toff * nbv : 0;
  const int f_rpi = FUSED ? nthr / nbv : 1;

  for (int j0 = 0; j0 < nz; j0 += T) {
    const int Tc = min(T, nz - j0);
    if (active) {
      TIO* tl = tile + cl * colrun + b;
      for (int t = 0; t < Tc; ++t) {
        double val[S::NARR];
        st.level(j0 + t, rec, nz, val);
#pragma unroll
        for (int k = 0; k < S::NARR; ++k) tl[k * (CB * colrun) + t * nb] = (TIO)val[k];
      }
    }
    if (cfg.flags & CRT_TILE_FLAG_SYNC_BARRIERS) __syncthreads(); else lds_barrier();
    if constexpr (FUSED) {
      if (f_toff < f_rpi) {
        const vt* tv = reinterpret_cast<const vt*>(tile);
        for (int t = f_toff; t < Tc; t += f_rpi) {
          const long long go = ((long long)c0 * nz + j0 + t) * nbv + f_p;
          vt v[S::NARR];
#pragma unroll
          for (int k = 0; k < S::NARR; ++k) v[k] = tv[(k * colrun + t * nb) / VW + f_p];
#pragma unroll
          for (int k = 0; k < S::NARR; ++k) __builtin_nontemporal_store(v[k], reinterpret_cast<vt*>(a.o[k]) + go);
        }
      }
    } else {
    const int n = Tc * nb;
    for (int k = 0; k < S::NARR; ++k) {
      for (int q = 0; q < ncb; ++q) {
        TIO* g = outp<TIO>(a.o[k]) + ((long long)(c0 + q) * nz + j0) * nb;
        const TIO* s = tile + k * (CB * colrun) + q * colrun;
        int mis = (int)(((16 - (reinterpret_cast<uintptr_t>(g) & 15)) & 15) / sizeof(TIO));
        if (mis > n) mis = n;
        const int nvec = (n - mis) / VW;
        const int tail = (n - mis) - nvec * VW;
        vt* gv = reinterpret_cast<vt*>(g + mis);
        if ((reinterpret_cast<uintptr_t>(s + mis) & 15) == 0) {
          const vt* sv = reinterpret_cast<const vt*>(s + mis);
          for (int i = tid; i < nvec; i += nthr) gv[i] = sv[i];
        } else {
          for (int i = tid; i < nvec; i += nthr) {
            vt v;
#pragma unroll
            for (int w = 0; w < VW; ++w) v[w] = s[mis + VW * i + w];
            gv[i] = v;
          }
        }
        if (tid < mis) g[tid] = s[tid];
        if (tid < tail) g[mis + nvec * VW + tid] = s[mis + nvec * VW + tid];
      }
    }
    }
    if (cfg.flags & CRT_TILE_FLAG_SYNC_BARRIERS) __syncthreads(); else lds_barrier();
  }
}

struct PipeTileCfg {
  int ncomp;
  int T;
  int rec_dbl;
};

template <class S, typename TIO, int MAXT, bool FUSED, bool K0 = false>
__global__ __launch_bounds__(MAXT) void k_pipe(SolveArgs a, PipeTileCfg cfg, ColArgs ca) {
  static_assert(!K0 || std::is_same<S, Sch2s>::value, "the record prologue forms the 2s record only");
  constexpr int VW = 16 / (int)sizeof(TIO);
  typedef TIO vt __attribute__((ext_vector_type(VW)));
  extern __shared__ double lds[];
  const int nb = a.nb, nz = a.nz, T = cfg.T;
  const int c = blockIdx.x;
  const int tid = threadIdx.x;
#ifdef CRT_STAMP
  if ((threadIdx.x & 63) == 0) {
    double* dbg = const_cast<double*>(a.ws) + (long long)c * a.reclen + 100 + 3 * (threadIdx.x >> 6);
    dbg[0] = (double)__builtin_amdgcn_s_getreg((31 << 11) | 4);
    dbg[1] = (double)__builtin_amdgcn_s_getreg((31 << 11) | 6);
    dbg[2] = (double)(tid >> 6);
  }
#endif
  BandIn bin = {};
  if (tid < cfg.ncomp) bin = load_band<TIO>(a, c, tid < nb ? tid : 0, S::SOIL);
  if constexpr (K0) {
    col_record_2s(ca, c, lds, tid, blockDim.x);
  } else {
    const double* src = a.ws + (long long)c * a.reclen;
    for (int i = threadIdx.x; i < a.reclen; i += blockDim.x) lds[i] = src[i];
  }
  __syncthreads();
  const double* rec = lds;
  constexpr int HEAD = FUSED ? 0 : 128 / (int)sizeof(TIO);
  TIO* tile = reinterpret_cast<TIO*>(lds + cfg.rec_dbl) + HEAD;
  const int colrun = HEAD + T * nb, bufrun = S::NARR * colrun;
  if (tid < cfg.ncomp) {
    const bool active = tid < nb;
    const int b = active ? tid : 0;
#ifdef CRT_STAMP
    double* stamp = const_cast<double*>(a.ws) + (long long)c * a.reclen;
    int nstamp = 0;
    const bool stamper = tid == 0;
#define STAMP() do { if (stamper && nstamp < 60) stamp[nstamp++] = (double)wall_clock64(); } while (0)
    STAMP();
#else
#define STAMP() do {} while (0)
#endif
    S st;
    st.init(rec, bin, a);
    STAMP();
    const bool unif = __builtin_amdgcn_readfirstlane((int)(rec[S_UNIF] != 0.0)) != 0;
    auto sweep = [&](auto mode) {
      constexpr int MODE = decltype(mode)::value;
      int buf = 0;
      for (int j0 = 0; j0 < nz; j0 += T) {
        const int Tc = min(T, nz - j0);
        TIO* tl = tile + buf * bufrun + b;
        for (int t = 0; t < Tc; ++t) {
          double val[S::NARR];
          st.template level<MODE>(j0 + t, rec, nz, val);
          if (active) {
#pragma unroll
            for (int k = 0; k < S::NARR; ++k) tl[k * colrun + t * nb] = (TIO)val[k];
          }
        }
        STAMP();
        lds_barrier();
        STAMP();
        buf ^= 1;
      }
    };
    if (unif)
      sweep(std::integral_constant<int, 1>{});
    else
      sweep(std::integral_constant<int, 0>{});
  } else if constexpr (!FUSED) {
    constexpr int LINE = 128 / (int)sizeof(TIO);
    const int sid = tid - cfg.ncomp, nst = blockDim.x - cfg.ncomp;
    const long long col0 = (long long)c * nz * nb;
    int F[S::NARR];
#pragma unroll
    for (int k = 0; k < S::NARR; ++k) F[k] = 0;
    int buf = 0;
    for (int j0 = 0; j0 < nz; j0 += T) {
      const int Tc = min(T, nz - j0);
      lds_barrier();
      const int t0e = j0 * nb;
      const int avail = t0e + Tc * nb;
      const bool last = j0 + Tc >= nz;
#pragma unroll
      for (int k = 0; k < S::NARR; ++k) {
        TIO* gk = outp<TIO>(a.o[k]) + col0;
        const int f = F[k];
        const TIO* src = tile + buf * bufrun + k * colrun - (t0e - f);
        int end = avail;
        if (!last) end -= (int)((reinterpret_cast<uintptr_t>(gk + avail) / sizeof(TIO)) % LINE);
        if (end < f) end = f;
        const int n = end - f;
        TIO* g = gk + f;
        int mis = (int)(((16 - (reinterpret_cast<uintptr_t>(g) & 15)) & 15) / sizeof(TIO));
        if (mis > n) mis = n;
        const int nvec = (n - mis) / VW;
        const int tail = (n - mis) - nvec * VW;
        vt* gv = reinterpret_cast<vt*>(g + mis);
        for (int i = sid; i < nvec; i += nst) {
          vt v;
#pragma unroll
          for (int w = 0; w < VW; ++w) v[w] = src[mis + VW * i + w];
          __builtin_nontemporal_store(v, gv + i);
        }
        if (sid < mis) __builtin_nontemporal_store(src[sid], g + sid);
        if (sid < tail) __builtin_nontemporal_store(src[mis + nvec * VW + sid], g + mis + nvec * VW + sid);
        const int npark = avail - end;
        if (sid < npark) tile[(buf ^ 1) * bufrun + k * colrun - npark + sid] = src[n + sid];
        F[k] = end;
      }
      buf ^= 1;
    }
  } else {
    const int nbv = nb / VW;
    const int sid = tid - cfg.ncomp, nst = blockDim.x - cfg.ncomp;
    const int dt = nst / nbv, dp = nst - dt * nbv;
    const int t0 = sid / nbv, p0 = sid - t0 * nbv;
#ifdef CRT_STAMP
    double* sstamp = const_cast<double*>(a.ws) + (long long)c * a.reclen + 64;
    int nsstamp = 0;
#define SSTAMP() do { if (sid == 0 && nsstamp < 60) sstamp[nsstamp++] = (double)wall_clock64(); } while (0)
#else
#define SSTAMP() do {} while (0)
#endif
    SSTAMP();
    int buf = 0;
    for (int j0 = 0; j0 < nz; j0 += T) {
      const int Tc = min(T, nz - j0);
      lds_barrier();
      SSTAMP();
      const vt* tv = reinterpret_cast<const vt*>(tile + buf * bufrun);
      int t = t0, p = p0;
      while (t < Tc) {
        const long long go = ((long long)c * nz + j0 + t) * nbv + p;
        vt v[S::NARR];
#pragma unroll
        for (int k = 0; k < S::NARR; ++k) v[k] = tv[(k * colrun + t * nb) / VW + p];
#pragma unroll
        for (int k = 0; k < S::NARR; ++k) __builtin_nontemporal_store(v[k], reinterpret_cast<vt*>(a.o[k]) + go);
        p += dp;
        t += dt;
        if (p >= nbv) {
          p -= nbv;
          ++t;
        }
      }
      SSTAMP();
      buf ^= 1;
    }
#ifdef CRT_STAMP
    asm volatile("s_waitcnt vmcnt(0)" ::: "memory");
    SSTAMP();
#endif
  }
}

struct PackCfg {
  int ncw;
  int cpw;
  int T;
};

template <class S, typename TIO, int MAXT>
__global__ __launch_bounds__(MAXT) void k_pipe_pack(SolveArgs a, PackCfg cfg) {
  constexpr int VW = 16 / (int)sizeof(TIO);
  typedef TIO vt __attribute__((ext_vector_type(VW)));
  extern __shared__ double lds[];
  const int nb = a.nb, nz = a.nz, T = cfg.T;
  const int tid = threadIdx.x;
  const int cpw = cfg.cpw;
  const int c0 = blockIdx.x * cpw;
  const int ncol_here = min(cpw, a.ncol - c0);
  const int ncomp = 64 * cfg.ncw;
  const int cl = tid / nb;
  const bool active = tid < ncomp && cl < ncol_here;
  const int b = active ? tid - cl * nb : 0;
  BandIn bin = {};
  if (tid < ncomp) bin = load_band<TIO>(a, c0 + (active ? cl : 0), b, S::SOIL);
  {
    const double* src = a.ws + (long long)c0 * a.reclen;
    for (int i = tid; i < ncol_here * a.reclen; i += blockDim.x) lds[i] = src[i];
  }
  __syncthreads();
  const int rec_dbl = (cpw * a.reclen + 1) & ~1;
  TIO* tile = reinterpret_cast<TIO*>(lds + rec_dbl);
  const int arrrun = T * nb, colrun = S::NARR * arrrun, bufrun = cpw * colrun;
  if (tid < ncomp) {
    const double* rec = lds + (active ? cl : 0) * a.reclen;
    S st;
    st.init(rec, bin, a);
    int buf = 0;
    for (int j0 = 0; j0 < nz; j0 += T) {
      const int Tc = min(T, nz - j0);
      TIO* tl = tile + buf * bufrun + (active ? cl : 0) * colrun + b;
      for (int t = 0; t < Tc; ++t) {
        double val[S::NARR];
        st.template level<2>(j0 + t, rec, nz, val);
        if (active) {
#pragma unroll
          for (int k = 0; k < S::NARR; ++k) tl[k * arrrun + t * nb] = (TIO)val[k];
        }
      }
      lds_barrier();
      buf ^= 1;
    }
  } else {
    const int sid = tid - ncomp, nst = blockDim.x - ncomp;
    const int nbv = nb / VW, arrv = arrrun / VW;
    int buf = 0;
    for (int j0 = 0; j0 < nz; j0 += T) {
      const int Tc = min(T, nz - j0);
      lds_barrier();
      const int per = Tc * nbv;
      const int total = ncol_here * per;
      int c = sid / per, v = sid - c * per;
      const int dc = nst / per, dv = nst - dc * per;
      for (int idx = sid; idx < total; idx += nst) {
        const vt* src = reinterpret_cast<const vt*>(tile + buf * bufrun + c * colrun) + v;
        const long long go = ((long long)(c0 + c) * nz + j0) * nbv + v;
        vt x[S::NARR];
#pragma unroll
        for (int k = 0; k < S::NARR; ++k) x[k] = src[k * arrv];
#pragma unroll
        for (int k = 0; k < S::NARR; ++k) __builtin_nontemporal_store(x[k], reinterpret_cast<vt*>(a.o[k]) + go);
        v += dv;
        c += dc;
        if (v >= per) {
          v -= per;
          ++c;
        }
      }
      buf ^= 1;
    }
  }
}

constexpr int MAX_DIRECT_LDS = 64 * 1024;
constexpr int DEFAULT_TILE_LDS = 78 * 1024;
constexpr int MIN_TILE_NB = 4;

int gcd(int x, int y) { return y ? gcd(y, x % y) : x; }

int k0_before(const ColArgs* k0, hipStream_t s) { return k0 ? launch_colpre(*k0, s) : (int)CRT_OK; }

template <class S, typename TIO>
int launch_tile(const SolveArgs& a, hipStream_t s, bool& done, const ColArgs* k0) {
  done = false;
  const int nb = a.nb;
  const Tune& tune = a.tune;
  if (nb < tune.min_nb(MIN_TILE_NB) || nb > 1024) return CRT_OK;
  if ((nb <= 32 || tune.pack == CRT_PACK_FORCE) && nb <= 128 && tune.pack != CRT_PACK_OFF) {
    constexpr int VWp = 16 / (int)sizeof(TIO);
    bool ok = nb % VWp == 0 && (a.nz * nb) % VWp == 0;
    for (int i = 0; i < S::NARR && ok; ++i)
      if (reinterpret_cast<uintptr_t>(a.o[i]) & 15) ok = false;
    if (ok) {
      PackCfg pc;
      pc.ncw = tune.pack_compute_waves > 0 ? tune.pack_compute_waves : (nb <= 32 ? 1 : 2);
      if (64 * pc.ncw < nb) pc.ncw = (nb + 63) / 64;
      pc.cpw = 64 * pc.ncw / nb;
      const int linep = 128 / (int)sizeof(TIO);
      const int Tap = linep / gcd(nb, linep);
      int Tp = tune.closed_pipe_t > 0 ? tune.closed_pipe_t : std::max(4, Tap);
      if (Tp > a.nz) Tp = a.nz;
      pc.T = Tp;
      const int cpw = pc.cpw;
      const int nswp = tune.closed_store_waves > 0 ? tune.closed_store_waves : 1;
      const size_t shp = (size_t)((cpw * a.reclen + 1) & ~1) * sizeof(double) + (size_t)2 * cpw * S::NARR * Tp * nb * sizeof(TIO);
      const int thr = 64 * (pc.ncw + nswp);
      if (shp <= 160 * 1024 && thr <= 512 && (Tp * nb) % VWp == 0) {
        if (const int st = k0_before(k0, s)) return st;
        if (const int st = launch_kernel(k_pipe_pack<S, TIO, 512>, dim3((a.ncol + cpw - 1) / cpw), thr, shp, s, a, pc)) return st;
        note_kernel("k_pipe_pack<%s,%s> columns=%d compute_waves=%d T=%d store_waves=%d lds=%zu", S::NAME, sizeof(TIO) == 8 ? "f64" : "f32", pc.cpw,
                    pc.ncw, Tp, nswp, shp);
        done = true;
        return (int)CRT_OK;
      }
    }
  }
  const int CB = nb <= 256 ? 256 / nb : 1;
  const int nthr = CB > 1 ? 256 : ((nb + 63) / 64) * 64;
  const int line = 128 / (int)sizeof(TIO);
  const int Ta = line / gcd(nb, line);
  const size_t per_level = (size_t)S::NARR * CB * nb * sizeof(TIO);
  const size_t target = (size_t)(tune.tile_lds > 0 ? tune.tile_lds : DEFAULT_TILE_LDS);
  int T = Ta;
  if (per_level * Ta > target) {
    T = (int)(target / per_level);
    if (T < 2) return CRT_OK;
  } else {
    while (per_level * (T + Ta) <= target && T + Ta <= a.nz) T += Ta;
  }
  if (tune.tile_t > 0) T = tune.tile_t;
  if (T > a.nz) T = a.nz;
  TileCfg cfg;
  cfg.CB = CB;
  cfg.T = T;
  cfg.rec_dbl = (CB * a.reclen + 1) & ~1;
  cfg.flags = tune.tile_flags;
  const size_t sh = cfg.rec_dbl * sizeof(double) + (size_t)S::NARR * CB * T * nb * sizeof(TIO);
  if (sh > 160 * 1024) return CRT_OK;
  constexpr int VW = 16 / (int)sizeof(TIO);
  bool fused = CB == 1 && nb % VW == 0 && !(tune.tile_flags & CRT_TILE_FLAG_GENERIC_FLUSH);
  for (int i = 0; i < S::NARR && fused; ++i)
    if (reinterpret_cast<uintptr_t>(a.o[i]) & 15) fused = false;
  const int grid = (a.ncol + CB - 1) / CB;
  bool pfused = nb % VW == 0 && !(tune.tile_flags & CRT_TILE_FLAG_GENERIC_FLUSH);
  for (int i = 0; i < S::NARR && pfused; ++i)
    if (reinterpret_cast<uintptr_t>(a.o[i]) & 15) pfused = false;
  if (!(tune.tile_flags & CRT_TILE_FLAG_NO_PIPELINE) && (pfused || !(tune.tile_flags & CRT_TILE_FLAG_NO_GENERIC_PIPELINE))) {
    const bool fused = pfused;
    const int pcomp = ((nb + 63) / 64) * 64;
    const size_t plevel = (size_t)S::NARR * nb * sizeof(TIO);
    int nsw = tune.closed_store_waves > 0 ? tune.closed_store_waves : (pcomp <= 64 || (S::HEAVY_INIT && pcomp <= 128 && !fused) ? 1 : pcomp <= 128 ? 2 : 3);
    if (pcomp + 64 * nsw > 1024) nsw = (1024 - pcomp) / 64;
    size_t budget = target;
    if (S::HEAVY_INIT && 2 * plevel * 4 <= 40 * 1024) budget = 40 * 1024;
    if (sizeof(TIO) == 4 && std::is_same<S, Sch2s>::value && 2 * plevel * 4 <= 40 * 1024) budget = 40 * 1024;
    if (!fused && pcomp <= 128 && budget > 32 * 1024) budget = 32 * 1024;
    int Tmax = (int)std::min<size_t>(8, budget / (2 * plevel));
    if (fused && pcomp <= 64 && nb >= 32 && Tmax > 4) Tmax = 4;
    if (Tmax < 4 && 2 * plevel * 4 <= target) Tmax = 4;
    int Tp = Ta <= Tmax ? (Tmax / Ta) * Ta : Tmax;
    if (tune.closed_pipe_t > 0) Tp = tune.closed_pipe_t;
    if (Tp > a.nz) Tp = a.nz;
    PipeTileCfg pc;
    pc.ncomp = pcomp;
    pc.T = Tp;
    pc.rec_dbl = (a.reclen + 1) & ~1;
    const size_t psh = pc.rec_dbl * sizeof(double) + 2 * plevel * Tp + (fused ? 0 : 2 * S::NARR * 128);
    if (nsw >= 1 && Tp >= 2 && psh <= 160 * 1024 && (fused ? (2 * plevel * Ta <= target || tune.closed_pipe_t > 0) : true)) {
      const int pthr = pcomp + 64 * nsw;
      constexpr bool can_k0 = std::is_same<S, Sch2s>::value;
      const bool own_k0 = can_k0 && k0 != nullptr;
      auto gop = [&](auto kern) {
        if (!own_k0)
          if (const int st = k0_before(k0, s)) return st;
        if (const int st = launch_kernel(kern, dim3(a.ncol), pthr, psh, s, a, pc, own_k0 ? *k0 : ColArgs{})) return st;
        note_kernel("k_pipe<%s,%s>%s T=%d store_waves=%d lds=%zu%s", S::NAME, sizeof(TIO) == 8 ? "f64" : "f32", fused ? "" : " generic-flush", Tp, nsw, psh,
                    own_k0 ? " k0=fused" : "");
        return (int)CRT_OK;
      };
      int st;
      if (own_k0) {
        if (fused) st = pthr <= 512 ? gop(k_pipe<S, TIO, 512, true, can_k0>) : gop(k_pipe<S, TIO, 1024, true, can_k0>);
        else st = pthr <= 512 ? gop(k_pipe<S, TIO, 512, false, can_k0>) : gop(k_pipe<S, TIO, 1024, false, can_k0>);
      } else {
        if (fused) st = pthr <= 512 ? gop(k_pipe<S, TIO, 512, true>) : gop(k_pipe<S, TIO, 1024, true>);
        else st = pthr <= 512 ? gop(k_pipe<S, TIO, 512, false>) : gop(k_pipe<S, TIO, 1024, false>);
      }
      done = st == CRT_OK;
      return st;
    }
  }
  auto go = [&](auto kern) {
    if (const int st = k0_before(k0, s)) return st;
    if (const int st = launch_kernel(kern, dim3(grid), nthr, sh, s, a, cfg)) return st;
    note_kernel("k_tile<%s,%s>%s CB=%d T=%d lds=%zu", S::NAME, sizeof(TIO) == 8 ? "f64" : "f32", fused ? "" : " generic-flush", CB, T, sh);
    return (int)CRT_OK;
  };
  int st;
  if (fused) {
    if (nthr <= 256) st = go(k_tile<S, TIO, 256, true>);
    else if (nthr <= 512) st = go(k_tile<S, TIO, 512, true>);
    else st = go(k_tile<S, TIO, 1024, true>);
  } else {
    if (nthr <= 256) st = go(k_tile<S, TIO, 256, false>);
    else if (nthr <= 512) st = go(k_tile<S, TIO, 512, false>);
    else st = go(k_tile<S, TIO, 1024, false>);
  }
  done = st == CRT_OK;
  return st;
}

template <class S, typename TIO, int VEC, bool USE_LDS>
int launch_direct_v(const SolveArgs& a, size_t lds_bytes, hipStream_t s) {
  const long long items = (long long)a.ncol * (a.nb / VEC);
  const long long nblk = (items + DBLOCK - 1) / DBLOCK;
  if (nblk > 0x7fffffffLL) return CRT_ERR_UNSUPPORTED;
  hipLaunchKernelGGL((k_direct<S, TIO, VEC, USE_LDS>), dim3((unsigned)nblk), dim3(DBLOCK), USE_LDS ? lds_bytes : 0, s, a);
  if (hipGetLastError() != hipSuccess) return CRT_ERR_LAUNCH;
  note_kernel("k_direct<%s,%s> VEC=%d", S::NAME, sizeof(TIO) == 8 ? "f64" : "f32", VEC);
  return CRT_OK;
}

template <class S, typename TIO>
int launch_scheme(const SolveArgs& a, hipStream_t s, int force, const ColArgs* k0) {
  if (force != 1) {
    bool done;
    int st = launch_tile<S, TIO>(a, s, done, k0);
    if (st != CRT_OK || done) return st;
  }
  if (const int st = k0_before(k0, s)) return st;
  bool vec2 = (a.nb % 2 == 0) && (a.col_stride % 2 == 0);
  for (int i = 0; i < S::NARR && vec2; ++i)
    if (reinterpret_cast<uintptr_t>(a.o[i]) & (2 * sizeof(TIO) - 1)) vec2 = false;
  const int nbv = a.nb / (vec2 ? 2 : 1);
  const long long cols_per_block = (DBLOCK - 1) / nbv + 2;
  const size_t lds_bytes = (size_t)cols_per_block * a.reclen * sizeof(double);
  const bool use_lds = lds_bytes <= (size_t)MAX_DIRECT_LDS;
  if (vec2)
    return use_lds ? launch_direct_v<S, TIO, 2, true>(a, lds_bytes, s) : launch_direct_v<S, TIO, 2, false>(a, lds_bytes, s);
  return use_lds ? launch_direct_v<S, TIO, 1, true>(a, lds_bytes, s) : launch_direct_v<S, TIO, 1, false>(a, lds_bytes, s);
}

template <class S>
int launch_io(const SolveArgs& a, hipStream_t s, int force, const ColArgs* k0) {
  return a.f32 ? launch_scheme<S, float>(a, s, force, k0) : launch_scheme<S, double>(a, s, force, k0);
}

template <class S, typename TIO, bool PROF>
__device__ __forceinline__ void int_body(const SolveArgs& a, const IntArgs& ia, int rec_dbl, double* lds) {
  const int nb = a.nb, nz = a.nz, ng = ia.ngroup;
  const int tid = threadIdx.x, nthr = blockDim.x, lane = tid & 63, wave = tid >> 6, nwave = nthr >> 6;
  const int c = blockIdx.x;
  const double* rec = lds;
  const IntLds L = int_lds_carve(lds + rec_dbl, nz, nwave, PROF);
  const bool active = tid < nb;
  const int b = active ? tid : 0;
  const BandIn in = load_band<TIO>(a, c, b, S::SOIL);
  S st;
  st.init(rec, in, a);
  double w[INT_MAXG];
#pragma unroll
  for (int g = 0; g < INT_MAXG; ++g) w[g] = (g < ng && active) ? ia.band_w[(long long)g * nb + b] : 0.0;
#pragma unroll
  for (int g = 0; g < INT_MAXG; ++g)
    if (g < ng) {
      const double t = wave_sum_all(w[g] * (1 - (in.r + in.t)) * in.I_dr0);
      if (lane == 0) L.pdr[wave * INT_MAXG + g] = t;
      if constexpr (PROF) {
        const double t0 = wave_sum_all(w[g] * in.I_dr0);
        if (lane == 0) L.pi0[wave * INT_MAXG + g] = t0;
      }
    }
  for (int j = 0; j < nz; ++j) {
    double val[S::NARR];
    st.level(j, rec, nz, val);
    int_accumulate<false, PROF>(L, nwave, wave, lane, nz, j, ng, w, active, val[0], val[1], val[2]);
  }
  int_finish<false, PROF>(L, ia, nwave, nz, c, rec[S_KB], rec[S_INVMU]);
}

template <class S, typename TIO, int MAXT, bool PROF>
__global__ __launch_bounds__(MAXT) void k_int(SolveArgs a, IntArgs ia, int rec_dbl) {
  extern __shared__ double lds[];
  {
    const double* src = a.ws + (long long)blockIdx.x * a.reclen;
    for (int i = threadIdx.x; i < a.reclen; i += blockDim.x) lds[i] = src[i];
  }
  __syncthreads();
  int_body<S, TIO, PROF>(a, ia, rec_dbl, lds);
}

template <class S, int MAXT, bool PROF>
__global__ __launch_bounds__(MAXT) void k_int_series(SolveArgs a, IntArgs ia, SeriesArgs sr, int rec_dbl) {
  extern __shared__ double lds[];
  series_step(a, ia, sr, lds, [&](const SolveArgs& at, const IntArgs& it) { int_body<S, double, PROF>(at, it, rec_dbl, lds); });
}

template <class S, typename TIO>
int launch_int(const SolveArgs& a, const IntArgs& ia, hipStream_t s, const SeriesArgs* sr) {
  if (a.nb > 1024) return CRT_ERR_UNSUPPORTED;
  const int nthr = ((a.nb + 63) / 64) * 64;
  const int rec_dbl = (a.reclen + 1) & ~1;
  const bool prof = ia.L_dr != nullptr;
  const size_t sh = (rec_dbl + int_lds_doubles(a.nz, nthr / 64, false, prof)) * sizeof(double);
  if (sh > 160 * 1024) return CRT_ERR_UNSUPPORTED;
  if (sr) {
    if constexpr (sizeof(TIO) == 8) {
      auto gos = [&](auto kern) {
        const int st = launch_kernel(kern, series_grid(a.ncol, sr->nt), nthr, sh, s, a, ia, *sr, rec_dbl);
        if (st == CRT_OK) note_kernel("k_colpre<canopy> + k_colsun + k_int_series<%s>%s nt=%d", S::NAME, prof ? " + level profiles" : " wave totals", sr->nt);
        return st;
      };
      if (prof) return nthr <= 256 ? gos(k_int_series<S, 256, true>) : nthr <= 512 ? gos(k_int_series<S, 512, true>) : gos(k_int_series<S, 1024, true>);
      return nthr <= 256 ? gos(k_int_series<S, 256, false>) : nthr <= 512 ? gos(k_int_series<S, 512, false>) : gos(k_int_series<S, 1024, false>);
    }
    return CRT_ERR_UNSUPPORTED;
  }
  auto go = [&](auto kern) {
    if (const int st = launch_kernel(kern, dim3(a.ncol), nthr, sh, s, a, ia, rec_dbl)) return st;
    note_kernel("k_int<%s>%s%s", S::NAME, sizeof(TIO) == 8 ? "" : " f32", prof ? " + level profiles" : " wave totals");
    return (int)CRT_OK;
  };
  if (prof) {
    if (nthr <= 256) return go(k_int<S, TIO, 256, true>);
    if (nthr <= 512) return go(k_int<S, TIO, 512, true>);
    return go(k_int<S, TIO, 1024, true>);
  }
  if (nthr <= 256) return go(k_int<S, TIO, 256, false>);
  if (nthr <= 512) return go(k_int<S, TIO, 512, false>);
  return go(k_int<S, TIO, 1024, false>);
}

// ... 189 lines not shown
```

crt1d_amd/csrc/solve_tridiag_tile.hip:

```cpp
#include "crt_internal.hpp"

namespace crt {

#include <stdarg.h>
#include <stdio.h>

namespace {
thread_local char g_last_kernel[192] = "";
}

void note_kernel(const char* fmt, ...) {
  va_list ap;
  va_start(ap, fmt);
  vsnprintf(g_last_kernel, sizeof g_last_kernel, fmt, ap);
  va_end(ap);
}
const char* last_kernel() { return g_last_kernel; }

int launch_tridiag_int(int scheme, const SolveArgs& a, const IntArgs& ia, hipStream_t s, const SeriesArgs* sr) {
  if (scheme == CRT_SCHEME_N79) return a.f32 ? launch_tri_int_n79_f32(a, ia, s, sr) : launch_tri_int_n79_f64(a, ia, s, sr);
  if (scheme == CRT_SCHEME_ZQ) return a.f32 ? launch_tri_int_zq_f32(a, ia, s, sr) : launch_tri_int_zq_f64(a, ia, s, sr);
  return CRT_ERR_BAD_ARG;
}

int launch_tridiag_lev(int scheme, const SolveArgs& a, const LevArgs& la, hipStream_t s, const SeriesArgs* sr, bool probe, SensLaunch* sl) {
  if (scheme == CRT_SCHEME_N79) return a.f32 ? launch_tri_lev_n79_f32(a, la, s, sr, probe, sl) : launch_tri_lev_n79_f64(a, la, s, sr, probe, sl);
  if (scheme == CRT_SCHEME_ZQ) return a.f32 ? launch_tri_lev_zq_f32(a, la, s, sr, probe, sl) : launch_tri_lev_zq_f64(a, la, s, sr, probe, sl);
  return CRT_ERR_BAD_ARG;
}

int launch_tridiag_tile(int scheme, const SolveArgs& a, hipStream_t s, bool& done) {
  if (scheme == CRT_SCHEME_N79) return a.f32 ? launch_tri_tile_n79_f32(a, s, done) : launch_tri_tile_n79_f64(a, s, done);
  if (scheme == CRT_SCHEME_ZQ) return a.f32 ? launch_tri_tile_zq_f32(a, s, done) : launch_tri_tile_zq_f64(a, s, done);
  done = false;
  return CRT_ERR_BAD_ARG;
}

}
```

crt1d_amd/csrc/tri_tile_impl.hpp:

```cpp
#pragma once
#include <type_traits>

#include "crt_internal.hpp"
#include "tri_schemes.hpp"

namespace crt {
namespace {

constexpr size_t MAX_WG_LDS = 160 * 1024;

struct TriCfg {
  int T;
  int nck;
  int off_bc;
  int off_ck;
  int off_tile;
  int flat;
};

template <class S, typename TIO, int ARR>
__device__ inline void flush_array(const SolveArgs& a, const double* rec, const double* bandc, const double* tile, int tstride,
                                   int c, int j0, int nrows, double invmu, float inv_nb, int tid, int nthr) {
  if (nrows <= 0) return;
  typedef TIO vt __attribute__((ext_vector_type(2)));
// ... 655 lines not shown
  series_lev_step<double>(a, la, sr, nslice, lds, [&](const SolveArgs& at, int slice, long long, long long vcol) {
    if constexpr (!std::is_same<S, SU>::value) {
      if (lds[S_UNIF] != 0.0) {
        tri_lev_body<SU, double, M, true>(at, la, per, off_ck, lds, slice, 0, &sn, lds + off_st, nslice, vcol);
        return;
      }
    }
    tri_lev_body<S, double, M, true>(at, la, per, off_ck, lds, slice, 0, &sn, lds + off_st, nslice, vcol);
  });
}

template <class S, typename TIO, int M, int MAXT>
__global__ __launch_bounds__(MAXT) __attribute__((amdgpu_waves_per_eu(M <= 8 ? 5 : 3))) void k_tri_lev(SolveArgs a, LevArgs la, int per,
                                                                                                        int off_ck) {
  extern __shared__ double lds[];
  {
    const double* src = a.ws + (long long)blockIdx.x * a.reclen;
    for (int i = threadIdx.x; i < a.reclen; i += blockDim.x) lds[i] = src[i];
  }
  __syncthreads();
  typedef typename UniformOf<S>::type SU;
  if constexpr (!std::is_same<S, SU>::value) {
    if (lds[S_UNIF] != 0.0) {
      tri_lev_body<SU, TIO, M>(a, la, per, off_ck, lds, blockIdx.y, 0);
      return;
    }
  }
  tri_lev_body<S, TIO, M>(a, la, per, off_ck, lds, blockIdx.y, 0);
}

template <class S, typename TIO, int M, int MAXT>
__global__ __launch_bounds__(MAXT) __attribute__((amdgpu_waves_per_eu(M <= 8 ? 5 : 3))) void k_tri_lev_series(SolveArgs a, LevArgs la, SeriesArgs sr,
                                                                                                               int per, int off_ck, int nslice) {
  extern __shared__ double lds[];
  typedef typename UniformOf<S>::type SU;
  series_lev_step<TIO>(a, la, sr, nslice, lds, [&](const SolveArgs& at, int slice, long long oshift) {
    if constexpr (!std::is_same<S, SU>::value) {
      if (lds[S_UNIF] != 0.0) {
        tri_lev_body<SU, TIO, M>(at, la, per, off_ck, lds, slice, oshift);
        return;
      }
    }
    tri_lev_body<S, TIO, M>(at, la, per, off_ck, lds, slice, oshift);
  });
}

template <class S>
inline size_t tri_lev_lds_bytes(const SolveArgs& a, int M, int nthr, int* off_ck = nullptr) {
  const int K = S::rows(a.nz);
  const int nck = (K - 1) / M + 1;
  const int ock = (a.reclen + 1) & ~1;
  if (off_ck) *off_ck = ock;
  return ((size_t)ock + 2 * (size_t)nck * nthr) * sizeof(double);
}

template <class S, typename TIO, int M>
int launch_lev_sens_m(const SolveArgs& a, const LevArgs& la, hipStream_t s, const SeriesArgs* sr, bool probe, SensLaunch* sl) {
  auto bytes = [&](int nthr) { return tri_lev_lds_bytes<S>(a, M, nthr) + (size_t)SENS_STAGE * nthr * sizeof(double); };
  const LevSlices ls = lev_slices_fit(a.nb, MAX_WG_LDS, bytes);
  if (ls.nslice == 0 || ls.nslice > 65535) return CRT_ERR_UNSUPPORTED;
  int off_ck;
  const int off_st = (int)(tri_lev_lds_bytes<S>(a, M, ls.nthr, &off_ck) / sizeof(double));
  const size_t sh = bytes(ls.nthr);
  const long long nv = (long long)a.ncol * (sr ? sr->nt : 1);
  dim3 grid(a.ncol, ls.nslice);
  if (sr && (sizeof(TIO) != 8 || !lev_series_grid(a.ncol, sr->nt, ls.nslice, &grid))) return CRT_ERR_UNSUPPORTED;
  int st = sens_probe(sl, ls, nv, la.nsel);
  if (probe || st != CRT_OK) return st;
  if (sr) {
    if constexpr (sizeof(TIO) == 8) {
      auto gos = [&](auto kern) { return launch_kernel(kern, grid, ls.nthr, sh, s, a, la, sl->sn, *sr, ls.per, off_ck, off_st, ls.nslice); };
      st = ls.nthr <= 256   ? gos(k_tri_lev_sens_series<S, M, 256>)
           : ls.nthr <= 512 ? gos(k_tri_lev_sens_series<S, M, 512>)
                            : gos(k_tri_lev_sens_series<S, M, 1024>);
    } else {
      return CRT_ERR_UNSUPPORTED;
    }
  } else {
    auto go = [&](auto kern) { return launch_kernel(kern, grid, ls.nthr, sh, s, a, la, sl->sn, ls.per, off_ck, off_st); };
    st = ls.nthr <= 256 ? go(k_tri_lev_sens<S, TIO, M, 256>) : ls.nthr <= 512 ? go(k_tri_lev_sens<S, TIO, M, 512>) : go(k_tri_lev_sens<S, TIO, M, 1024>);
  }
  if (st != CRT_OK || (st = sens_finish(sl, ls, nv, a.nb, la.nsel, s)) != CRT_OK) return st;
  note_kernel("%sk_tri_lev_sens%s<%s>%s M=%d nsel=%d nsens=%d slice=%d%s", sr ? "k_colpre<canopy> + k_colsun + " : "", sr ? "_series" : "", S::NAME,
              sizeof(TIO) == 8 ? "" : " f32", M, la.nsel, sl->sn.nsens, ls.per, ls.nslice > 1 ? " + k_sens_finish" : "");
  return CRT_OK;
}

template <class S, typename TIO, int M>
int launch_lev_m(const SolveArgs& a, const LevArgs& la, hipStream_t s, const SeriesArgs* sr, bool probe) {
  const LevSlices ls = lev_slices_fit(a.nb, MAX_WG_LDS, [&](int nthr) { return tri_lev_lds_bytes<S>(a, M, nthr); });
  if (ls.nslice == 0 || ls.nslice > 65535) return CRT_ERR_UNSUPPORTED;
  int off_ck;
  const size_t sh = tri_lev_lds_bytes<S>(a, M, ls.nthr, &off_ck);
  if (sr) {
    dim3 grid;
    if (!lev_series_grid(a.ncol, sr->nt, ls.nslice, &grid)) return CRT_ERR_UNSUPPORTED;
    if (probe) return CRT_OK;
    auto gos = [&](auto kern) {
      const int st = launch_kernel(kern, grid, ls.nthr, sh, s, a, la, *sr, ls.per, off_ck, ls.nslice);
      if (st == CRT_OK)
        note_kernel("k_colpre<canopy> + k_colsun + k_tri_lev_series<%s>%s M=%d nsel=%d slice=%d nt=%d", S::NAME, sizeof(TIO) == 8 ? "" : " f32", M,
                    la.nsel, ls.per, sr->nt);
      return st;
    };
    return ls.nthr <= 256   ? gos(k_tri_lev_series<S, TIO, M, 256>)
           : ls.nthr <= 512 ? gos(k_tri_lev_series<S, TIO, M, 512>)
                            : gos(k_tri_lev_series<S, TIO, M, 1024>);
  }
  if (probe) return CRT_OK;
  auto go = [&](auto kern) {
    if (const int st = launch_kernel(kern, dim3(a.ncol, ls.nslice), ls.nthr, sh, s, a, la, ls.per, off_ck)) return st;
    note_kernel("k_tri_lev<%s>%s M=%d nsel=%d slice=%d", S::NAME, sizeof(TIO) == 8 ? "" : " f32", M, la.nsel, ls.per);
    return (int)CRT_OK;
  };
  if (ls.nthr <= 256) return go(k_tri_lev<S, TIO, M, 256>);
  if (ls.nthr <= 512) return go(k_tri_lev<S, TIO, M, 512>);
  return go(k_tri_lev<S, TIO, M, 1024>);
}

template <class S, typename TIO>
int launch_lev_scheme(const SolveArgs& a, const LevArgs& la, hipStream_t s, const SeriesArgs* sr, bool probe, SensLaunch* sl) {
  if (sl) {
    int st = launch_lev_sens_m<S, TIO, 8>(a, la, s, sr, probe, sl);
    if (st == CRT_ERR_UNSUPPORTED) st = launch_lev_sens_m<S, TIO, 16>(a, la, s, sr, probe, sl);
    return st;
  }
  int st = launch_lev_m<S, TIO, 8>(a, la, s, sr, probe);
  if (st == CRT_ERR_UNSUPPORTED) st = launch_lev_m<S, TIO, 16>(a, la, s, sr, probe);
  return st;
}

template <class S, typename TIO, bool FUSED>
int launch_cfg(const SolveArgs& a, hipStream_t s, int M, int T, int nthr) {
  if (M == 8 && T == 4) return launch_mt<S, TIO, 8, 4, FUSED>(a, s, nthr);
  if (M == 8 && T == 8) return launch_mt<S, TIO, 8, 8, FUSED>(a, s, nthr);
  if (M == 12 && T == 4) return launch_mt<S, TIO, 12, 4, FUSED>(a, s, nthr);
  if (M == 12 && T == 12) return launch_mt<S, TIO, 12, 12, FUSED>(a, s, nthr);
  if (M == 16 && T == 4) return launch_mt<S, TIO, 16, 4, FUSED>(a, s, nthr);
  if (M == 16 && T == 8) return launch_mt<S, TIO, 16, 8, FUSED>(a, s, nthr);
  return CRT_ERR_UNSUPPORTED;
}

struct PipeCfg {
  int ncomp;
  int nck;
  int off_bc, off_ck, off_tile;
  int flat;
  int off_park;
  int cpw;
  int nz_out, off_halo;
  void* out[4];
};

template <class S, typename TIO, int M, int T, int RS, int NSTG = S::NST, bool PACK = false>
__device__ __forceinline__ void tri_pipe_compute(const SolveArgs& a, const PipeCfg& cfg, double* lds, const TriBand* band = nullptr) {
  const int nb = a.nb, nz = a.nz;
  const int tid = threadIdx.x, nthr = cfg.ncomp;
  const int cl = PACK ? tid / nb : 0;
  const bool active = PACK ? (cl < cfg.cpw && (int)blockIdx.x * cfg.cpw + cl < a.ncol) : tid < nb;
  const int b = active ? tid - cl * nb : 0;
  const int c = PACK ? (int)blockIdx.x * cfg.cpw + (active ? cl : 0) : (int)blockIdx.x;
  const double* rec = PACK ? lds + (active ? cl : 0) * a.reclen : lds;
  double* bandc = lds + cfg.off_bc + (PACK && active ? cl * nb : 0);
  double* ck = lds + cfg.off_ck + tid;
  double* tile = lds + cfg.off_tile + (PACK && active ? cl * (T * nb) : 0);
  const int tstride = (PACK ? cfg.cpw : 1) * T * nb, bstride = NSTG * tstride;
#ifdef CRT_STAMP
  double* stamp = const_cast<double*>(a.ws) + (long long)c * a.reclen;
  int nstamp = 0;
#define TSTAMP() do { if (tid == 0 && nstamp < a.reclen) stamp[nstamp++] = (double)wall_clock64(); } while (0)
#else
#define TSTAMP() do {} while (0)
#endif
  TSTAMP();
  S st;
  if (band)
    st.init_band(rec, a, *band);
  else
    st.template init<TIO>(rec, a, c, b);
  if (active) bandc[b] = st.band_const();
  const int K = S::rows(nz);
  TSTAMP();
  const int seg_top = (K - 1) / M, k_top = seg_top * M;
  double be[M], bf[M];
  typename S::St fs;
  st.first(rec, nz, fs);
  tri_forward<S, M>(st, rec, nz, fs, k_top, [&](int level, const typename S::St& cs) {
    if (level < k_top) {
      const int sidx = level / M - 1;
      double e, f;
      st.pair(cs, e, f);
      ck[(2 * sidx) * nthr] = e;
      ck[(2 * sidx + 1) * nthr] = f;
    }
  });
  st.pair(fs, be[0], bf[0]);
  if constexpr (S::RENORM > 0 && M % (S::RENORM > 0 ? S::RENORM : 1) != 0) st.seed(fs, be[0], bf[0]);
#pragma unroll
  for (int i = 1; i < M; ++i) {
    be[i] = be[i - 1];
    bf[i] = bf[i - 1];
    if (k_top + i <= K - 1) tri_step(st, k_top + i - 1, rec, nz, fs, be[i], bf[i]);
  }
  TSTAMP();
  int buf = 0;
  for (int seg = seg_top; seg >= 0; --seg) {
    const int k0 = seg * M;
    const int kend = min(k0 + M - 1, K - 1);
    TSTAMP();
    if (seg != seg_top) {
      typename S::St rs;
      if (seg == 0) {
        st.first(rec, nz, rs);
        st.pair(rs, be[0], bf[0]);
      } else {
        be[0] = ck[(2 * (seg - 1)) * nthr];
        bf[0] = ck[(2 * (seg - 1) + 1) * nthr];
        st.seed(rs, be[0], bf[0]);
      }
#pragma unroll
      for (int i = 1; i < M; ++i) {
        be[i] = be[i - 1];
        bf[i] = bf[i - 1];
        if (k0 + i <= kend) tri_step(st, k0 + i - 1, rec, nz, rs, be[i], bf[i]);
      }
    }
    TSTAMP();
#pragma unroll
    for (int i = M - 1; i >= 0; --i) {
      const int k = k0 + i;
      if (k <= kend) {
        double o[S::NST];
        if (k == K - 1)
          st.top(rec, nz, be[i], bf[i], o);
        else
          st.back(k, rec, nz, be[i], bf[i], o);
        if (active) {
#pragma unroll
          for (int q = 0; q < NSTG; ++q) tile[buf * bstride + q * tstride + (i % T) * nb + b] = o[q];
        }
        if (i % T == 0) {
          TSTAMP();
          lds_barrier();
          if constexpr (RS > 0)
            lds_barrier();
          else
            buf ^= 1;
          TSTAMP();
        }
      }
    }
  }
}

template <class S, typename TIO, int M, int T, int RS>
__device__ __forceinline__ void tri_pipe_store_rs(const SolveArgs& a, const PipeCfg& cfg, double* lds) {
  const int nb2 = a.nb >> 1, nz = a.nz;
  const int c = blockIdx.x;
  const int sid = threadIdx.x - cfg.ncomp, nst = blockDim.x - cfg.ncomp;
  const double* rec = lds;
  const d2* bandc2 = reinterpret_cast<const d2*>(lds + cfg.off_bc);
  const d2* tb = reinterpret_cast<const d2*>(lds + cfg.off_tile);
  const double invmu = rec[S_INVMU];
  const int K = S::rows(nz);
  const int dt = nst / nb2, dp = nst - dt * nb2;
  const int t0 = sid / nb2, p0 = sid - t0 * nb2;
  for (int seg = (K - 1) / M; seg >= 0; --seg) {
    const int k0 = seg * M;
    const int kend = min(k0 + M - 1, K - 1);
    for (int i = M - T; i >= 0; i -= T) {
      const int k = k0 + i;
      if (k > kend) continue;
      const int jmax = min(kend, nz - 1);
      d2 v[RS][S::NST];
      int tt[RS], pp[RS];
      lds_barrier();
      {
        int t = t0, p = p0;
#pragma unroll
        for (int it = 0; it < RS; ++it) {
          tt[it] = t;
          pp[it] = p;
          if (t < T) {
#pragma unroll
            for (int q = 0; q < S::NST; ++q) v[it][q] = tb[(q * T + t) * nb2 + p];
          }
          p += dp;
          t += dt;
          if (p >= nb2) {
            p -= nb2;
            ++t;
          }
        }
      }
      lds_barrier();
#pragma unroll
      for (int it = 0; it < RS; ++it) {
        __builtin_amdgcn_sched_barrier(0);
        const int j = k + tt[it];
        if (tt[it] < T && j <= jmax) {
          d2 o[S::NOUT];
          S::emit(rec, nz, j, bandc2[pp[it]], invmu, v[it], o);
#pragma unroll
          for (int r = 0; r < S::NOUT; ++r) {
            const int rows = S::out_rows(r, nz);
            if (j < rows) {
              typedef TIO vt __attribute__((ext_vector_type(2)));
              vt w;
              w.x = (TIO)o[r].x;
              w.y = (TIO)o[r].y;
              vt* colbase = reinterpret_cast<vt*>(a.o[r]) + (long long)c * rows * nb2;
              store_rows<S, TIO>(colbase + (unsigned)(j * nb2 + pp[it]), w);
            }
          }
        }
      }
    }
  }
}

template <class S, typename TIO, int M, int T>
__device__ __forceinline__ void tri_pack_store(const SolveArgs& a, const PipeCfg& cfg, double* lds) {
  constexpr int RS = 2;
  const int nb2 = a.nb >> 1, nz = a.nz, cpw = cfg.cpw;
  const int c0 = blockIdx.x * cpw;
  const int ncol_here = min(cpw, a.ncol - c0);
  const int sid = threadIdx.x - cfg.ncomp, nst = blockDim.x - cfg.ncomp;
  const d2* bandc2 = reinterpret_cast<const d2*>(lds + cfg.off_bc);
  const d2* tb = reinterpret_cast<const d2*>(lds + cfg.off_tile);
  const int K = S::rows(nz);
  const int per = T * nb2, qstride = cpw * per;
  int ff[RS], cc[RS], tt[RS], pp[RS];
#pragma unroll
  for (int it = 0; it < RS; ++it) {
    const int f = sid + it * nst;
    const int c = f / per, r = f - c * per, t = r / nb2;
    ff[it] = f;
    cc[it] = c < ncol_here ? c : -1;
    tt[it] = t;
    pp[it] = r - t * nb2;
  }
  for (int seg = (K - 1) / M; seg >= 0; --seg) {
    const int k0 = seg * M;
    const int kend = min(k0 + M - 1, K - 1);
    for (int i = M - T; i >= 0; i -= T) {
      const int k = k0 + i;
      if (k > kend) continue;
      const int jmax = min(kend, nz - 1);
      d2 v[RS][S::NST];
      lds_barrier();
#pragma unroll
      for (int it = 0; it < RS; ++it)
        if (cc[it] >= 0) {
#pragma unroll
          for (int q = 0; q < S::NST; ++q) v[it][q] = tb[q * qstride + ff[it]];
        }
      lds_barrier();
#pragma unroll
      for (int it = 0; it < RS; ++it) {
        __builtin_amdgcn_sched_barrier(0);
        const int j = k + tt[it];
        if (cc[it] >= 0 && j <= jmax) {
          const double* rec = lds + cc[it] * a.reclen;
          d2 o[S::NOUT];
          S::emit(rec, nz, j, bandc2[cc[it] * nb2 + pp[it]], rec[S_INVMU], v[it], o);
#pragma unroll
          for (int r = 0; r < S::NOUT; ++r) {
            const int rows = S::out_rows(r, nz);
            if (j < rows) {
              typedef TIO vt __attribute__((ext_vector_type(2)));
              vt w;
              w.x = (TIO)o[r].x;
              w.y = (TIO)o[r].y;
              store_rows<S, TIO>(reinterpret_cast<vt*>(a.o[r]) + ((long long)(c0 + cc[it]) * rows + j) * nb2 + pp[it], w);
            }
          }
        }
      }
    }
  }
}

template <class S, typename TIO, int M, int T>
__device__ __forceinline__ void tri_pipe_store_generic(const SolveArgs& a, const PipeCfg& cfg, double* lds) {
  const int nb = a.nb, nz = a.nz;
  const int c = blockIdx.x;
  const int sid = threadIdx.x - cfg.ncomp, nst = blockDim.x - cfg.ncomp;
  const double* rec = lds;
  const double* bandc = lds + cfg.off_bc;
  const double* tile = lds + cfg.off_tile;
  const int tstride = T * nb, bstride = S::NST * tstride;
  const double invmu = rec[S_INVMU];
  const float inv_nb = 1.0f / (float)nb;
  const int K = S::rows(nz);
  int buf = 0;
  for (int seg = (K - 1) / M; seg >= 0; --seg) {
    const int k0 = seg * M;
    const int kend = min(k0 + M - 1, K - 1);
    for (int i = M - T; i >= 0; i -= T) {
      const int k = k0 + i;
      if (k > kend) continue;
      lds_barrier();
      if (cfg.flat == 3)
        flush_flat_wl<S, TIO>(a, rec, bandc, tile + buf * bstride, tstride, c, k, min(T, kend - k + 1), invmu, sid, nst, lds + cfg.off_park, buf);
      else if (cfg.flat)
        flush_flat<S, TIO>(a, rec, bandc, tile + buf * bstride, tstride, c, k, min(T, kend - k + 1), invmu, sid, nst, cfg.flat == 2);
      else
        flush_arrays<S, TIO, 0>(a, rec, bandc, tile + buf * bstride, tstride, c, k, min(T, kend - k + 1), invmu, inv_nb, sid, nst);
      buf ^= 1;
    }
  }
}

template <class S, typename TIO, int M, int T>
__device__ __forceinline__ void tri_pipe_store(const SolveArgs& a, const PipeCfg& cfg, double* lds) {
  const int nb2 = a.nb >> 1, nz = a.nz;
  const int c = blockIdx.x;
  const int sid = threadIdx.x - cfg.ncomp, nst = blockDim.x - cfg.ncomp;
  const double* rec = lds;
  const d2* bandc2 = reinterpret_cast<const d2*>(lds + cfg.off_bc);
  const d2* tile2 = reinterpret_cast<const d2*>(lds + cfg.off_tile);
  const double invmu = rec[S_INVMU];
  const int K = S::rows(nz);
  const int dt = nst / nb2, dp = nst - dt * nb2;
  const int t0 = sid / nb2, p0 = sid - t0 * nb2;
  int buf = 0;
  for (int seg = (K - 1) / M; seg >= 0; --seg) {
    const int k0 = seg * M;
    const int kend = min(k0 + M - 1, K - 1);
    for (int i = M - T; i >= 0; i -= T) {
      const int k = k0 + i;
      if (k > kend) continue;
      lds_barrier();
      const d2* tb = tile2 + (size_t)buf * (S::NST * T * nb2);
      const int jmax = min(kend, nz - 1);
      int t = t0, p = p0;
      while (t < T) {
        const int j = k + t;
        if (j <= jmax) {
          d2 st[S::NST], o[S::NOUT];
#pragma unroll
          for (int q = 0; q < S::NST; ++q) st[q] = tb[(q * T + t) * nb2 + p];
          S::emit(rec, nz, j, bandc2[p], invmu, st, o);
#pragma unroll
          for (int r = 0; r < S::NOUT; ++r) {
            const int rows = S::out_rows(r, nz);
            if (j < rows) {
              typedef TIO vt __attribute__((ext_vector_type(2)));
              vt v;
              v.x = (TIO)o[r].x;
              v.y = (TIO)o[r].y;
              vt* colbase = reinterpret_cast<vt*>(a.o[r]) + (long long)c * rows * nb2;
              store_rows<S, TIO>(colbase + (unsigned)(j * nb2 + p), v);
            }
          }
        }
        p += dp;
        t += dt;
        if (p >= nb2) {
          p -= nb2;
          ++t;
        }
      }
      buf ^= 1;
    }
  }
}

template <class S, typename TIO, int M, int T, int MAXT, int RS>
__global__ __launch_bounds__(MAXT) __attribute__((amdgpu_waves_per_eu((RS == 2 || RS == 3) ? 5 : 4))) void k_tri_pipe(SolveArgs a, PipeCfg cfg) {
  static_assert(M % T == 0, "tile height must divide the checkpoint spacing");
  extern __shared__ double lds[];
  if constexpr (RS == 3) {
    const int c0 = blockIdx.x * cfg.cpw;
    const int nhere = min(cfg.cpw, a.ncol - c0);
    const double* src = a.ws + (long long)c0 * a.reclen;
    for (int i = threadIdx.x; i < nhere * a.reclen; i += blockDim.x) lds[i] = src[i];
    __syncthreads();
    if ((int)threadIdx.x >= cfg.ncomp) {
      tri_pack_store<S, TIO, M, T>(a, cfg, lds);
      return;
    }
    typedef typename UniformOf<S>::type SU;
    if constexpr (!std::is_same<S, SU>::value) {
      bool all_unif = true;
      for (int i = 0; i < nhere; ++i) all_unif = all_unif && lds[i * a.reclen + S_UNIF] != 0.0;
      if (all_unif) {
        tri_pipe_compute<SU, TIO, M, T, 2, S::NST, true>(a, cfg, lds);
        return;
      }
    }
    tri_pipe_compute<S, TIO, M, T, 2, S::NST, true>(a, cfg, lds);
    return;
  }
  {
    const double* src = a.ws + (long long)blockIdx.x * a.reclen;
    for (int i = threadIdx.x; i < a.reclen; i += blockDim.x) lds[i] = src[i];
  }
  __syncthreads();
  if ((int)threadIdx.x >= cfg.ncomp) {
    if constexpr (RS > 0)
      tri_pipe_store_rs<S, TIO, M, T, RS>(a, cfg, lds);
    else if constexpr (RS < 0)
      tri_pipe_store_generic<S, TIO, M, T>(a, cfg, lds);
    else
      tri_pipe_store<S, TIO, M, T>(a, cfg, lds);
    return;
  }
  typedef typename UniformOf<S>::type SU;
  if constexpr (!std::is_same<S, SU>::value) {
    if (lds[S_UNIF] != 0.0) {
      tri_pipe_compute<SU, TIO, M, T, RS>(a, cfg, lds);
      return;
    }
  }
  tri_pipe_compute<S, TIO, M, T, RS>(a, cfg, lds);
}

constexpr int PIPE_RS = 4;

template <class S, typename TIO, int M, int T>
int launch_pipe_generic(const SolveArgs& a, hipStream_t s, int nstore_waves) {
  const int ncomp = ((a.nb + 63) / 64) * 64;
  const int nthr = ncomp + 64 * nstore_waves;
  if (nthr > 512) return CRT_ERR_UNSUPPORTED;
  const int K = S::rows(a.nz);
  PipeCfg cfg{};
  cfg.ncomp = ncomp;
  cfg.nck = std::max((K - 1) / M - 1, 0);
  cfg.off_bc = (a.reclen + 1) & ~1;
  cfg.off_ck = cfg.off_bc + ((a.nb + 1) & ~1);
  cfg.off_tile = cfg.off_ck + 2 * cfg.nck * ncomp;
  cfg.flat = a.tune.flat_flush != CRT_FLAT_FLUSH_OFF ? flat_flush_ok<S, TIO>(a) : 0;
  cfg.off_park = cfg.off_tile + 2 * S::NST * T * a.nb;
  const bool wl_default = flush_classes<S>() == 1;
  const int ff = a.tune.flat_flush;
  if (cfg.flat == 2 && a.nb >= 128 / (int)sizeof(TIO) && (ff == CRT_FLAT_FLUSH_WHOLE_LINE || (ff == 0 && wl_default))) cfg.flat = 3;
  const size_t sh = ((size_t)cfg.off_park + (cfg.flat == 3 ? park_doubles<S, TIO>() : 0)) * sizeof(double);
  if (sh > MAX_WG_LDS) return CRT_ERR_UNSUPPORTED;
  if (const int st = launch_kernel(k_tri_pipe<S, TIO, M, T, 512, -1>, dim3(a.ncol), nthr, sh, s, a, cfg)) return st;
  note_kernel("k_tri_pipe<%s,%s> %s M=%d T=%d store_waves=%d lds=%zu", S::NAME, sizeof(TIO) == 8 ? "f64" : "f32", cfg.flat == 3 ? "whole-line flat-flush" : cfg.flat ? "flat-flush" : "generic-flush", M, T,
              nstore_waves, sh);
  return (int)CRT_OK;
}

template <class S, typename TIO>
int launch_tri_pack(const SolveArgs& a, hipStream_t s) {
  constexpr int M = 8, T = 4;
  {
    const int ncw_set = a.tune.pack_compute_waves, ncw = ncw_set > 0 ? ncw_set : (a.nb <= 32 ? 1 : 2);
    if (a.nb % 2 || a.nb < 2 || 64 * ncw / a.nb < 2 || (a.nb > 42 && ncw_set == 0)) return CRT_ERR_UNSUPPORTED;
    for (int i = 0; i < S::NOUT; ++i)
      if (reinterpret_cast<uintptr_t>(a.o[i]) & (2 * sizeof(TIO) - 1)) return CRT_ERR_UNSUPPORTED;
    const int K = S::rows(a.nz);
    PipeCfg cfg{};
    cfg.ncomp = 64 * ncw;
    cfg.cpw = cfg.ncomp / a.nb;
    const int nsw = (cfg.cpw * T * (a.nb / 2) + 127) / 128;
    if (cfg.ncomp + 64 * nsw > 512) return CRT_ERR_UNSUPPORTED;
    cfg.nck = std::max((K - 1) / M - 1, 0);
    cfg.off_bc = (cfg.cpw * a.reclen + 1) & ~1;
    cfg.off_ck = cfg.off_bc + cfg.ncomp;
    cfg.off_tile = cfg.off_ck + 2 * cfg.nck * cfg.ncomp;
    const size_t sh = ((size_t)cfg.off_tile + (size_t)S::NST * cfg.cpw * T * a.nb) * sizeof(double);
    if (sh > MAX_WG_LDS / 2) return CRT_ERR_UNSUPPORTED;
    if (a.nb > 32 && ncw_set == 0 && (std::is_same<S, typename UniformOf<S>::type>::value || sh > 40 * 1024)) return CRT_ERR_UNSUPPORTED;
    if (const int st = launch_kernel(k_tri_pipe<S, TIO, M, T, 512, 3>, dim3((a.ncol + cfg.cpw - 1) / cfg.cpw), cfg.ncomp + 64 * nsw, sh, s, a, cfg)) return st;
    note_kernel("k_tri_pipe<%s,%s> packed columns=%d compute_waves=%d register-staged(2 pairs) M=%d T=%d store_waves=%d lds=%zu", S::NAME,
                sizeof(TIO) == 8 ? "f64" : "f32", cfg.cpw, ncw, M, T, nsw, sh);
    return (int)CRT_OK;
  }
}

template <class S, typename TIO, int M, int T>
int launch_pipe_mt(const SolveArgs& a, hipStream_t s, int nstore_waves, bool regstage) {
  const int ncomp = ((a.nb + 63) / 64) * 64;
  const int nthr = ncomp + 64 * nstore_waves;
  if (nthr > 1024) return CRT_ERR_UNSUPPORTED;
  if (regstage && T * (a.nb / 2) > PIPE_RS * 64 * nstore_waves) return CRT_ERR_UNSUPPORTED;
  const int K = S::rows(a.nz);
  PipeCfg cfg{};
  cfg.ncomp = ncomp;
  cfg.nck = std::max((K - 1) / M - 1, 0);
  cfg.off_bc = (a.reclen + 1) & ~1;
  cfg.off_ck = cfg.off_bc + ((a.nb + 1) & ~1);
  cfg.off_tile = cfg.off_ck + 2 * cfg.nck * ncomp;
  const size_t sh = ((size_t)cfg.off_tile + (size_t)(regstage ? 1 : 2) * S::NST * T * a.nb) * sizeof(double);
  if (sh > (regstage ? MAX_WG_LDS / 2 : MAX_WG_LDS)) return CRT_ERR_UNSUPPORTED;
  const bool narrow_rs = T == 4 && M == 8 && regstage && nthr <= 512 && T * (a.nb / 2) <= 2 * 64 * nstore_waves &&
                         !(a.tune.tile_flags & CRT_TILE_FLAG_FOUR_PAIR_STORE);
  auto go = [&](auto kern) {
    if (const int st = launch_kernel(kern, dim3(a.ncol), nthr, sh, s, a, cfg)) return st;
    note_kernel("k_tri_pipe<%s,%s> %s M=%d T=%d store_waves=%d lds=%zu", S::NAME, sizeof(TIO) == 8 ? "f64" : "f32",
                regstage ? (narrow_rs ? "register-staged(2 pairs)" : "register-staged") : "double-buffered", M, T, nstore_waves, sh);
    return (int)CRT_OK;
  };
  if constexpr (T == 4 && M == 8) {
    if (narrow_rs) return go(k_tri_pipe<S, TIO, M, T, 512, 2>);
  }
  if (regstage) return nthr <= 512 ? go(k_tri_pipe<S, TIO, M, T, 512, PIPE_RS>) : go(k_tri_pipe<S, TIO, M, T, 1024, PIPE_RS>);
  return nthr <= 512 ? go(k_tri_pipe<S, TIO, M, T, 512, 0>) : go(k_tri_pipe<S, TIO, M, T, 1024, 0>);
}

template <class S, typename TIO>
int launch_pipe(const SolveArgs& a, hipStream_t s, int M, int T, int nsw, bool regstage) {
  if (M == 8 && T == 4) return launch_pipe_mt<S, TIO, 8, 4>(a, s, nsw, regstage);
  if (M == 12 && T == 4) return launch_pipe_mt<S, TIO, 12, 4>(a, s, nsw, regstage);
  if (M == 16 && T == 4) return launch_pipe_mt<S, TIO, 16, 4>(a, s, nsw, regstage);
  if (M == 16 && T == 8) return launch_pipe_mt<S, TIO, 16, 8>(a, s, nsw, regstage);
  return CRT_ERR_UNSUPPORTED;
}

template <class S, typename TIO>
int launch_scheme(const SolveArgs& a, hipStream_t s, bool& done, int min_nb = 10) {
  done = false;
  const Tune& tune = a.tune;
  const int family = tune.tri_family;
  if (a.nb <= 64 && tune.pack != CRT_PACK_OFF && tune.tri_m == 0 && family == 0) {
    const int st = launch_tri_pack<S, TIO>(a, s);
    if (st != CRT_ERR_UNSUPPORTED) {
      done = st == CRT_OK;
      return st;
    }
  }
  if (a.nb < tune.min_nb(min_nb) || a.nb > 1024) return CRT_OK;
  const int nthr = ((a.nb + 63) / 64) * 64;
  const int K = S::rows(a.nz);
  auto lds_bytes = [&](int M, int T) {
    const int nck = (K - 1) / M + 1;
    return ((size_t)a.reclen + a.nb + 4 + 2 * (size_t)nck * nthr + (size_t)S::NST * T * a.nb) * sizeof(double);
  };
  int M = 0, T = 0;
  const int pref_n79[6][2] = {{12, 4}, {8, 8}, {16, 8}, {8, 4}, {16, 4}, {12, 12}};
  const int pref_zq[6][2] = {{8, 8}, {16, 8}, {12, 4}, {8, 4}, {16, 4}, {12, 12}};
  const int (*pref)[2] = S::NOUT == 6 ? pref_n79 : pref_zq;
  for (int i = 0; i < 6 && !M; ++i) {
    const size_t need = lds_bytes(pref[i][0], pref[i][1]);
    const size_t budget = pref[i][1] == 4 && i == 0 ? 78 * 1024 : MAX_WG_LDS;
    if (need <= budget) { M = pref[i][0]; T = pref[i][1]; }
  }
  if (tune.tri_m > 0) {
    M = tune.tri_m;
    T = tune.tri_t > 0 ? tune.tri_t : 4;
    if (lds_bytes(M, T) > MAX_WG_LDS) return CRT_OK;
  }
  if (!M) return CRT_OK;
  bool fused = (a.nb % 2 == 0);
  for (int i = 0; i < S::NOUT && fused; ++i)
    if (reinterpret_cast<uintptr_t>(a.o[i]) & (2 * sizeof(TIO) - 1)) fused = false;
  const bool flat_ok = tune.flat_flush != CRT_FLAT_FLUSH_OFF && flat_flush_ok<S, TIO>(a);
  if (!fused && family != CRT_TRI_FAMILY_NO_PIPELINE && tune.tri_m == 0 &&
      ((nthr <= 128 && a.nb >= 16 && (S::NOUT == 7 || flat_ok)) || family == CRT_TRI_FAMILY_GENERIC_PIPELINE)) {
    const int nsw = tune.tri_store_waves > 0 ? tune.tri_store_waves : (nthr == 64 ? 1 : 2);
    int st = launch_pipe_generic<S, TIO, 12, 4>(a, s, nsw);
    if (st == CRT_ERR_UNSUPPORTED) st = launch_pipe_generic<S, TIO, 16, 4>(a, s, nsw);
    if (st != CRT_ERR_UNSUPPORTED) {
      done = st == CRT_OK;
      return st;
    }
  }
  if (fused && family != CRT_TRI_FAMILY_NO_PIPELINE && (a.nb >= 16 || family >= CRT_TRI_FAMILY_DOUBLE_BUFFERED)) {
    int nsw = tune.tri_store_waves > 0 ? tune.tri_store_waves : 4;
    if (nthr + 64 * nsw > 1024) nsw = (1024 - nthr) / 64;
    int st = CRT_ERR_UNSUPPORTED;
    if (nsw >= 1) {
      const bool try_rs = family != CRT_TRI_FAMILY_DOUBLE_BUFFERED, try_db = family != CRT_TRI_FAMILY_REG_STAGED;
      const int nsw_rs = tune.tri_store_waves > 0 ? nsw : (nthr == 64 ? 1 : min(nsw, 3));
      if (tune.tri_m > 0) {
        if (try_rs) st = launch_pipe<S, TIO>(a, s, M, T, nsw_rs, true);
        if (st == CRT_ERR_UNSUPPORTED && try_db) st = launch_pipe<S, TIO>(a, s, M, T, nsw, false);
      } else {
        const int pp_n79[3][2] = {{12, 4}, {16, 4}, {8, 4}};
        const int pp_zq[3][2] = {{8, 4}, {12, 4}, {16, 4}};
        const int (*pp)[2] = (S::NOUT == 6 && !(nthr == 64 && a.nz <= 80)) ? pp_n79 : pp_zq;
        for (int i = 0; i < 3 && st == CRT_ERR_UNSUPPORTED && try_rs; ++i) st = launch_pipe<S, TIO>(a, s, pp[i][0], pp[i][1], nsw_rs, true);
        for (int i = 0; i < 3 && st == CRT_ERR_UNSUPPORTED && try_db; ++i) st = launch_pipe<S, TIO>(a, s, pp[i][0], pp[i][1], nsw, false);
      }
    }
    if (st != CRT_ERR_UNSUPPORTED) {
      done = st == CRT_OK;
      return st;
    }
  }
  const int st = fused ? launch_cfg<S, TIO, true>(a, s, M, T, nthr) : launch_cfg<S, TIO, false>(a, s, M, T, nthr);
  if (st == CRT_ERR_UNSUPPORTED) return CRT_OK;
  done = st == CRT_OK;
  return st;
}

}
}
```

crt1d_amd/dist.py:

```python

import torch
import torch.distributed as dist

from .batched import PROFILE_KEYS, bandsum_shapes

KEYS = ("aI", "aI_sl", "aI_sh", "totals")
MSG_KEYS = ("aI_sl", "aI_sh", "totals")
PROFILE_MSG_KEYS = ("aI_dr", "I_dr", "I_df_d", "I_df_u")


def block_range(n, rank, world, unit=1):
    if unit > 1:
        lo, hi = block_range(n // unit, rank, world)
        return lo * unit, hi * unit
    q, r = divmod(n, world)
    lo = rank * q + min(rank, r)
    return lo, lo + q + (1 if rank < r else 0)


def band_block_range(nb, rank, world):
    return block_range(nb, rank, world, unit=2 if nb % 2 == 0 and nb >= 2 * world else 1)


def _world(group):
    if dist.is_available() and dist.is_initialized():
        return dist.get_world_size(group), dist.get_rank(group)
    return 1, 0


class _Tile:

    def __init__(self, clo, chi, nz, ng, like, profiles=False):
        self.clo, self.chi = clo, chi
        shapes = bandsum_shapes(chi - clo, nz, ng, profiles)
        msg = MSG_KEYS + (PROFILE_MSG_KEYS if profiles else ())

        def numel(k):
            m = 1
            for s in shapes[k]:
                m *= s
            return m

        self.flat = torch.empty(sum(numel(k) for k in msg), dtype=torch.float64, device=like.device)
        self.views, off = {}, 0
        for k in msg:
            self.views[k] = self.flat[off:off + numel(k)].view(shapes[k])
            off += numel(k)
        for k in ("aI", "F", "I_d") if profiles else ("aI",):
            self.views[k] = torch.empty(shapes[k], dtype=torch.float64, device=like.device)
        self.launch = None
        self.finish = None
        self.work = None
        self.reduced = False
        self.profiles = None


class BandShardPlan:

    def __init__(self, scheme, cols, bands, band_w, *, group=None, column_tiles=1, keep_profiles=True, share_profiles=False,
                 solve_fn=None, epilogue_fn=None, integrated_fn=None, placement="auto", always_reduce=False, level_profiles=False,
                 finish_fn=None, **opts):
        self.scheme, self.group = scheme, group
        self.level_profiles = bool(level_profiles)
        self.always_reduce = always_reduce
        self.world, self.rank = _world(group)
        self.ncol, self.nz = cols.ncol, cols.nz
        self.band_range = band_block_range(bands.nb, self.rank, self.world)
        lo, hi = self.band_range
        b = bands.band_slice(lo, hi)
        bw = band_w[:, lo:hi].contiguous()
        self.ng = bw.shape[0]
        self.ntile = max(1, min(int(column_tiles), cols.ncol))
        self.keep_profiles = keep_profiles
        functional = solve_fn is not None or epilogue_fn is not None or integrated_fn is not None
        if functional and keep_profiles and (solve_fn is None or epilogue_fn is None):
            raise ValueError("give both solve_fn and epilogue_fn (or neither)")
        self.tiles = []
        shared = None
        for t in range(self.ntile):
            clo, chi = block_range(cols.ncol, t, self.ntile)
            ct, bt = (cols, b) if self.ntile == 1 else (cols.slice(clo, chi), b.slice(clo, chi))
            tile = _Tile(clo, chi, self.nz, self.ng, bw, profiles=self.level_profiles)
            if self.level_profiles and self.world > 1:
                tile.finish = self._finish(tile, ct, finish_fn)
            if functional:
                tile.launch = self._functional_launch(tile, ct, bt, bw, solve_fn, epilogue_fn, integrated_fn, opts)
            else:
                from . import batched

                if keep_profiles:
                    if share_profiles and shared is not None and chi - clo == shared[0]:
                        out = shared[1]
                    else:
                        out = None
                    plan = batched.Plan(scheme, ct, bt, out=out, placement=placement, **opts)
                    if share_profiles and shared is None:
                        shared = (chi - clo, plan.out)
                    epi = batched.BandSumPlan(ct, bt, plan.out, bw, out=tile.views, profiles=self.level_profiles)
                    tile.launch = self._planned_launch(plan, epi)
                    tile.kernel_plan = plan
                else:
                    ip = batched.IntegratedPlan(scheme, ct, bt, bw, out=tile.views, profiles=self.level_profiles, **opts)
                    tile.launch = lambda ip=ip: (ip(), None)[1]
                    tile.kernel_plan = ip
            self.tiles.append(tile)

    @staticmethod
    def _planned_launch(plan, epi):
        def go():
            out = plan()
            epi()
            return out

        return go

    @staticmethod
    def _finish(tile, ct, finish_fn):
        if finish_fn is not None:
            return lambda: finish_fn(ct, tile.views)
        from . import batched

        return batched.BandSumFinishPlan(ct, tile.views)

    def _functional_launch(self, tile, ct, bt, bw, solve_fn, epilogue_fn, integrated_fn, opts):
        prof = {"profiles": True} if self.level_profiles else {}
        keys = KEYS + (PROFILE_KEYS if self.level_profiles else ())

        def go():
            if self.keep_profiles:
                sol = solve_fn(self.scheme, ct, bt, **opts)
                res = epilogue_fn(ct, bt, sol, bw, **prof)
            else:
                sol = None
                res = dict(integrated_fn(self.scheme, ct, bt, bw, **prof, **opts))
            for k in keys:
                tile.views[k].copy_(res[k])
            return sol

        return go

    @property
    def message_bytes(self):
        return sum(t.flat.numel() * 8 for t in self.tiles)

    def __call__(self, reduce=True):
        for tile in self.tiles:
            if tile.work is not None:
                tile.work.wait()
                tile.work = None
            tile.profiles = tile.launch()
            tile.work = None
            tile.reduced = False
            if reduce and (self.world > 1 or (self.always_reduce and dist.is_initialized())):
                tile.work = dist.all_reduce(tile.flat, op=dist.ReduceOp.SUM, group=self.group, async_op=True)
                tile.reduced = self.world > 1
        return self

    def wait(self):
        for tile in self.tiles:
            if tile.work is not None:
                tile.work.wait()
                tile.work = None
            if tile.reduced:
                if tile.finish is not None:
                    tile.finish()
                else:
                    torch.add(tile.views["aI_sl"], tile.views["aI_sh"], out=tile.views["aI"])
                tile.reduced = False
        if self.ntile == 1:
            res = dict(self.tiles[0].views)
            prof = self.tiles[0].profiles
        else:
            res = {k: torch.cat([t.views[k] for t in self.tiles], dim=0) for k in KEYS + (PROFILE_KEYS if self.level_profiles else ())}
            prof = [t.profiles for t in self.tiles]
        tot = res["totals"]
        res["reflectance"] = tot[..., 1] / tot[..., 0]
        res["columns"] = (0, self.ncol)
        res["profiles"] = prof if self.keep_profiles else None
        return res


def _default_fns():
    from . import batched

    return batched.solve, batched.absorb_bandsum


def solve_sharded(scheme, cols, bands, band_w, *, partition="column", group=None, solve_fn=None, epilogue_fn=None,
                  keep_profiles=True, integrated_fn=None, column_tiles=1, level_profiles=False, finish_fn=None, **opts):
    if partition == "band":
        if keep_profiles and solve_fn is None and epilogue_fn is None:
            solve_fn, epilogue_fn = _default_fns()
        elif keep_profiles and (solve_fn is None or epilogue_fn is None):
            s, e = _default_fns()
            solve_fn, epilogue_fn = solve_fn or s, epilogue_fn or e
        if not keep_profiles and integrated_fn is None:
            from . import batched

            integrated_fn = batched.solve_integrated
        plan = BandShardPlan(scheme, cols, bands, band_w, group=group, column_tiles=column_tiles, keep_profiles=keep_profiles,
                             solve_fn=solve_fn if keep_profiles else None, epilogue_fn=epilogue_fn if keep_profiles else None,
                             integrated_fn=None if keep_profiles else integrated_fn, level_profiles=level_profiles, finish_fn=finish_fn,
                             **opts)
        return plan().wait()
    if partition != "column":
        raise ValueError("partition must be 'column' or 'band'")
    if solve_fn is None or epilogue_fn is None:
        s, e = _default_fns()
        solve_fn = solve_fn or s
        epilogue_fn = epilogue_fn or e
    world, rank = _world(group)
    lo, hi = block_range(cols.ncol, rank, world)
    c, b = cols.slice(lo, hi), bands.slice(lo, hi)
    prof = {"profiles": True} if level_profiles else {}
    if keep_profiles:
        sol = solve_fn(scheme, c, b, **opts)
        res = dict(epilogue_fn(c, b, sol, band_w, **prof))
    else:
        if integrated_fn is None:
            from . import batched

            integrated_fn = batched.solve_integrated
        sol = None
        res = dict(integrated_fn(scheme, c, b, band_w, **prof, **opts))
    tot = res["totals"]
    res["reflectance"] = tot[..., 1] / tot[..., 0]
    res["columns"] = (lo, hi)
    res["profiles"] = sol
    return res


def grid_mean(res, ncol_total, group=None):
    keys = ("aI", "aI_sl", "aI_sh", "totals") + (PROFILE_KEYS if all(k in res for k in PROFILE_KEYS) else ())
    flat = torch.cat([res[k].sum(dim=0).reshape(-1) for k in keys])
    world, _ = _world(group)
    if world > 1 or (dist.is_available() and dist.is_initialized()):
        dist.all_reduce(flat, op=dist.ReduceOp.SUM, group=group)
    flat = flat / float(ncol_total)
    out, off = {}, 0
    for k in keys:
        shape = res[k].shape[1:]
        n = 1
        for x in shape:
            n *= x
        out[k] = flat[off:off + n].view(shape)
        off += n
    out["reflectance"] = out["totals"][..., 1] / out["totals"][..., 0]
    return out


def gather_columns(local, ncol, group=None):
    world, _ = _world(group)
# ... 10 lines not shown
```

Measured before the change: 3.469 billion.

## Fuse band-weighted absorption sums into pipelined solve kernels

Adds a combined solve+band-sum entry point that accumulates band-weighted net fluxes into LDS inside the pipelined closed-form and tridiagonal solve kernels. The store waves then fold each tile into per-layer absorption outputs, which avoids a separate kernel that rereads the full flux profiles from global memory. The fused path costs extra LDS per workgroup, which can reduce occupancy, and it adds reductions inside the compute loop. It only applies to f64 storage, some schemes, and configurations whose LDS fits the budget; otherwise it falls back to the separate kernel.

```diff
diff --git a/crt1d_amd/_lib.py b/crt1d_amd/_lib.py
--- a/crt1d_amd/_lib.py
+++ b/crt1d_amd/_lib.py
@@ -14,6 +14,7 @@
 FLAG_SKIP_PRECOMPUTE = 1
 FLAG_PRECOMPUTE_ONLY = 2
 FLAG_DIRECT_STORES = 4
+FLAG_BANDSUM_SEPARATE = 8
 
 MAX_LEVEL_SELECT = 64
 
@@ -246,6 +247,22 @@
 _SENSOR_SIGNATURES = _sensor_signatures()
 SENSOR_EXPORTS = list(_SENSOR_SIGNATURES)
 
+BANDSUM_TWO_WG_LDS = 80 * 1024
+
+
+def _bandsum_signatures():
+    P = ctypes.POINTER
+    i, i32, sz, ok = ctypes.c_int, ctypes.c_int32, ctypes.c_size_t, ctypes.c_int
+    return {
+        "crt_hip_solve_bandsum_f64": (ok, [i, P(CrtColumns), P(CrtBands), P(CrtOptions), _vp, i32, P(CrtOutputs), P(CrtBandsumOut), _vp, sz, _vp]),
+        "crt_hip_solve_bandsum_lds_fits": (i, [sz, sz]),
+        "crt_hip_solve_bandsum_lds_bytes": (sz, [i32, i32]),
+    }
+
+
+_BANDSUM_SIGNATURES = _bandsum_signatures()
+BANDSUM_EXPORTS = list(_BANDSUM_SIGNATURES)
+
 _lib = None
 
 
@@ -266,7 +283,7 @@
     import torch
 
     lib = ctypes.CDLL(LIB_PATH)
-    for name, (restype, argtypes) in {**_SIGNATURES, **_LEAF_SIGNATURES, **_SPECTRA_SIGNATURES, **_SENSOR_SIGNATURES}.items():
+    for name, (restype, argtypes) in {**_SIGNATURES, **_LEAF_SIGNATURES, **_SPECTRA_SIGNATURES, **_SENSOR_SIGNATURES, **_BANDSUM_SIGNATURES}.items():
         f = getattr(lib, name)
         f.restype = restype
         if argtypes is not None:
diff --git a/crt1d_amd/batched.py b/crt1d_amd/batched.py
--- a/crt1d_amd/batched.py
+++ b/crt1d_amd/batched.py
@@ -689,6 +689,37 @@
         return self.band_w.data_ptr(), self.band_w.shape[0], ctypes.byref(self._out)
 
 
+class SolveBandSumPlan(Plan):
+
+    _scheme_arg = True
+
+    def __init__(self, scheme, cols: Columns, bands: Bands, band_w, *, mu_s=0.501, tau_d_method="quad", out=None, bandsum_out=None,
+                 workspace=None, placement="auto", tune=None, profiles=False, separate=False):
+        if bands.dtype != torch.float64:
+            raise TypeError("SolveBandSumPlan serves float64 bands (f32 storage: Plan + BandSumPlan)")
+        super().__init__(scheme, cols, bands, mu_s=mu_s, tau_d_method=tau_d_method, out=out, workspace=workspace, placement=placement, tune=tune)
+        self.band_w = _band_weights(band_w, bands.nb, cols.device)
+        ng = self.band_w.shape[0]
+        self.sums = _outputs(bandsum_shapes(cols.ncol, cols.nz, ng, profiles), bandsum_out, torch.float64, cols.device)
+        self.profiles, self.separate = profiles, bool(separate)
+        self._sums = _bandsum_out_struct(self.sums, profiles)
+        self._entry = "crt_hip_solve_bandsum_f64"
+        self._fn = getattr(self.lib, self._entry)
+
+    def _tail(self):
+        return self.band_w.data_ptr(), self.band_w.shape[0], ctypes.byref(self._out), ctypes.byref(self._sums)
+
+    def __call__(self, stream=None, *, flags=0):
+        return super().__call__(stream, flags=int(flags) | (_lib.FLAG_BANDSUM_SEPARATE if self.separate else 0))
+
+
+def solve_bandsum(scheme, cols: Columns, bands: Bands, band_w, **kw):
+    kw.setdefault("placement", "none")
+    with torch.cuda.device(cols.device):
+        plan = SolveBandSumPlan(scheme, cols, bands, band_w, **kw)
+        return plan(), plan.sums
+
+
 def solve_integrated(scheme, cols: Columns, bands: Bands, band_w, **kw):
     with torch.cuda.device(cols.device):
         return IntegratedPlan(scheme, cols, bands, band_w, **kw)()
diff --git a/crt1d_amd/csrc/api.hip b/crt1d_amd/csrc/api.hip
--- a/crt1d_amd/csrc/api.hip
+++ b/crt1d_amd/csrc/api.hip
@@ -1,8 +1,10 @@
 #include <math.h>
 
 #include <algorithm>
+#include <cstdio>
 #include <cstring>
 
+#include "crt1d_hip_bandsum.h"
 #include "epilogue.hpp"
 
 namespace crt {
@@ -349,14 +351,19 @@
 static int solve_impl(int scheme, const crt_columns* cols, const crt_bands* bands, const crt_options* opts,
                       const crt_outputs* out, void* workspace, size_t workspace_bytes, crt_stream_t stream, int f32,
                       const IntArgs* integ = nullptr, const LevArgs* lev = nullptr, const crt_sun_series* ser = nullptr,
-                      SensLaunch* sl = nullptr, size_t extra_ws = 0) {
+                      SensLaunch* sl = nullptr, size_t extra_ws = 0, BandsumReq* bsr = nullptr) {
   SolveOpts o;
   if (const int st = check_solve(scheme, cols, bands, opts, out, workspace, workspace_bytes, integ, lev, ser, o, extra_ws)) return st;
   ColArgs ca;
   SolveArgs sa;
   build_args(scheme, cols, bands, out, workspace, f32, o, ca, sa);
+  o.flags &= ~CRT_FLAG_BANDSUM_SEPARATE;
   hipStream_t s = static_cast<hipStream_t>(stream);
-  return ser ? dispatch_series(scheme, ca, sa, o.flags, integ, lev, ser, s, sl) : dispatch_step(scheme, ca, sa, o.flags, integ, lev, s, sl);
+  if (ser) return dispatch_series(scheme, ca, sa, o.flags, integ, lev, ser, s, sl);
+  set_bandsum_request(bsr);
+  const int st = dispatch_step(scheme, ca, sa, o.flags, integ, lev, s, sl);
+  set_bandsum_request(nullptr);
+  return st;
 }
 
 int crt_hip_solve_f64(int scheme, const crt_columns* cols, const crt_bands* bands, const crt_options* opts,
@@ -427,6 +434,42 @@
                                double* aI_sh, double* totals, crt_stream_t stream) {
   const crt_bandsum_out o = bandsum_out4(aI, aI_sl, aI_sh, totals);
   return crt_hip_absorb_bandsum2_f32(cols, bands, I_dr, I_df_d, I_df_u, band_w, ngroup, &o, stream);
+}
+
+int crt_hip_solve_bandsum_f64(int scheme, const crt_columns* cols, const crt_bands* bands, const crt_options* opts, const double* band_w,
+                              int32_t ngroup, const crt_outputs* out, const crt_bandsum_out* sums, void* workspace, size_t workspace_bytes,
+                              crt_stream_t stream) {
+  if (!band_w || !sums || !sums->aI || !sums->aI_sl || !sums->aI_sh || ngroup <= 0 || ngroup > MAXG || !cols || !out) return CRT_ERR_BAD_ARG;
+  const int nopt = bandsum_nopt(*sums);
+  if (nopt < 0) return CRT_ERR_BAD_ARG;
+  const int flags = opts ? opts->flags : 0;
+  BandsumReq rq = {};
+  rq.ia.lai = cols->lai;
+  rq.ia.band_w = band_w;
+  rq.ia.ngroup = ngroup;
+  rq.ia.aI = sums->aI;
+  rq.ia.aI_sl = sums->aI_sl;
+  rq.ia.aI_sh = sums->aI_sh;
+  rq.ia.totals = sums->totals;
+  const bool ask = nopt == 0 && ngroup <= INT_MAXG && !(flags & (CRT_FLAG_BANDSUM_SEPARATE | CRT_FLAG_PRECOMPUTE_ONLY | CRT_FLAG_DIRECT_STORES));
+  if (const int st = solve_impl(scheme, cols, bands, opts, out, workspace, workspace_bytes, stream, 0, nullptr, nullptr, nullptr, nullptr, 0,
+                                ask ? &rq : nullptr))
+    return st;
+  if ((flags & CRT_FLAG_PRECOMPUTE_ONLY) || rq.done) return CRT_OK;
+  char solve_name[160];
+  snprintf(solve_name, sizeof solve_name, "%s", last_kernel());
+  if (const int st = bandsum_impl<double>(cols, bands->nb, bands->col_stride, bands->leaf_r, bands->leaf_t, out->I_dr, out->I_df_d, out->I_df_u,
+                                          band_w, ngroup, sums, stream))
+    return st;
+  note_kernel("%s | band sums: separate kernel", solve_name);
+  return CRT_OK;
+}
+
+int crt_hip_solve_bandsum_lds_fits(size_t solve_lds_bytes, size_t bandsum_lds_bytes) { return bs_lds_fits(solve_lds_bytes, bandsum_lds_bytes) ? 1 : 0; }
+
+size_t crt_hip_solve_bandsum_lds_bytes(int32_t tile_levels, int32_t compute_waves) {
+  if (tile_levels < 1 || compute_waves < 1) return 0;
+  return bs_lds_doubles(tile_levels, compute_waves) * sizeof(double);
 }
 
 static int integrated_impl(int scheme, const crt_columns* cols, const crt_bands* bands, const crt_options* opts, const double* band_w,
diff --git a/crt1d_amd/csrc/crt_internal.hpp b/crt1d_amd/csrc/crt_internal.hpp
--- a/crt1d_amd/csrc/crt_internal.hpp
+++ b/crt1d_amd/csrc/crt_internal.hpp
@@ -380,7 +380,7 @@
 
 template <bool ROWS, bool PROF = false>
 __device__ inline void int_accumulate(const IntLds& L, int nwave, int wave, int lane, int nz, int j, int ng, const double (&w)[INT_MAXG],
-                                      bool active, double idr, double dn, double up) {
+                                      bool active, double idr, double dn, double up, int jrow = -1) {
   if constexpr (!ROWS) {
     if constexpr (PROF) {
       const int g2 = wave_sum4_slot(lane >> 4);
@@ -396,7 +396,7 @@
     const bool writer = (lane & 15) == 0 && g < ng;
     const double net = active ? idr + dn - up : 0.0;
     const double z = wave_sum4(w[0] * net, w[1] * net, w[2] * net, w[3] * net);
-    if (writer) L.part[(j * nwave + wave) * INT_MAXG + g] = z;
+    if (writer) L.part[((jrow < 0 ? j : jrow) * nwave + wave) * INT_MAXG + g] = z;
     if (j == 0 || j == nz - 1) {
       const int e = j == 0 ? 0 : 1;
       const double dd = active ? idr + dn : 0.0, uu = active ? up : 0.0;
@@ -493,6 +493,85 @@
   const size_t nslot = rows ? (size_t)nwave * 4 : (size_t)nwave;
   return (size_t)nz * nslot * INT_MAXG + 2 * nslot * 2 * INT_MAXG + (size_t)nwave * INT_MAXG +
          (prof ? (size_t)nz * nwave * 2 * INT_MAXG + (size_t)nwave * INT_MAXG : 0);
+}
+
+struct BandsumReq {
+  IntArgs ia;
+  bool done;
+};
+void set_bandsum_request(BandsumReq* rq);
+BandsumReq* bandsum_request();
+struct BsArgs {
+  IntArgs ia;
+  int off;
+};
+constexpr size_t BS_TWO_WG_LDS = 80 * 1024;
+__host__ __device__ inline size_t bs_lds_doubles(int T, int nwave) {
+  return (size_t)2 * T * nwave * INT_MAXG + (size_t)2 * nwave * 2 * INT_MAXG + (size_t)nwave * INT_MAXG + INT_MAXG;
+}
+inline bool bs_lds_fits(size_t solve_bytes, size_t extra_bytes) {
+  return solve_bytes <= BS_TWO_WG_LDS && extra_bytes <= BS_TWO_WG_LDS - solve_bytes;
+}
+__device__ inline IntLds bs_lds_carve(double* base, int T, int nwave) {
+  IntLds L;
+  L.part = base;
+  L.ends = L.part + (size_t)2 * T * nwave * INT_MAXG;
+  L.pdr = L.ends + (size_t)2 * nwave * 2 * INT_MAXG;
+  L.lev = L.pdr + (size_t)nwave * INT_MAXG;
+  L.pi0 = nullptr;
+  return L;
+}
+__device__ inline void bs_setup(const IntLds& L, const IntArgs& ia, int nb, int b, bool active, int wave, int lane, double absorbed_dr0,
+                                double (&w)[INT_MAXG]) {
+#pragma unroll
+  for (int g = 0; g < INT_MAXG; ++g) w[g] = (g < ia.ngroup && active) ? ia.band_w[(long long)g * nb + b] : 0.0;
+#pragma unroll
+  for (int g = 0; g < INT_MAXG; ++g)
+    if (g < ia.ngroup) {
+      const double t = wave_sum_all(w[g] * absorbed_dr0);
+      if (lane == 0) L.pdr[wave * INT_MAXG + g] = t;
+    }
+}
+__device__ inline int wave_lane() { return __builtin_amdgcn_mbcnt_hi(~0u, __builtin_amdgcn_mbcnt_lo(~0u, 0u)); }
+template <bool DESC>
+__device__ inline void bs_fold_tile(const IntLds& L, const IntArgs& ia, int T, int nwave, int pbuf, int nz, int c, int j0, int nrows, double Kb,
+                                    int lane, bool last) {
+  const int ng = ia.ngroup;
+  if (nrows > 0) {
+    const int r = lane / ng, g = lane - r * ng;
+    const bool mine = r < nrows;
+    double phi = 0.0, pd = 0.0;
+    if (mine) {
+      for (int wv = 0; wv < nwave; ++wv) phi += L.part[(((size_t)pbuf * T + r) * nwave + wv) * INT_MAXG + g];
+      for (int wv = 0; wv < nwave; ++wv) pd += L.pdr[wv * INT_MAXG + g];
+    }
+    const double next = __shfl(phi, DESC ? lane + ng : lane - ng, 64);
+    const int j = j0 + r;
+    const bool inner = DESC ? r + 1 < nrows : r > 0;
+    const double other = (inner || !mine) ? next : L.lev[g];
+    const int k = DESC ? j : j - 1;
+    if (mine && k >= 0 && k < nz - 1) {
+      const double p1 = DESC ? other : phi, p0 = DESC ? phi : other;
+      const double* lai = ia.lai + (long long)c * nz;
+      const double dl = lai[k] - lai[k + 1];
+      const double fsl = exp(-Kb * ((lai[k] + lai[k + 1]) / 2));
+      const double adr = (1 - exp(-Kb * dl)) * exp(-Kb * lai[k + 1]) * pd;
+      const double a = p1 - p0;
+      const double adf = a - adr;
+      const long long o = ((long long)c * (nz - 1) + k) * ng + g;
+      ia.aI[o] = a;
+      ia.aI_sl[o] = adf * fsl + adr;
+      ia.aI_sh[o] = adf * (1 - fsl);
+    }
+    if (mine && r == (DESC ? 0 : nrows - 1)) L.lev[g] = phi;
+  }
+  if (last && ia.totals && lane < ng * 4) {
+    const int g = lane >> 2, q = lane & 3;
+    const int e = q < 2 ? 1 : 0, which = q & 1;
+    double t = 0.0;
+    for (int wv = 0; wv < nwave; ++wv) t += L.ends[((e * nwave + wv) * 2 + which) * INT_MAXG + g];
+    ia.totals[((long long)c * ng + g) * 4 + q] = t;
+  }
 }
 
 constexpr int SUN_HDR = 8;
diff --git a/crt1d_amd/csrc/solve_closed.hip b/crt1d_amd/csrc/solve_closed.hip
--- a/crt1d_amd/csrc/solve_closed.hip
+++ b/crt1d_amd/csrc/solve_closed.hip
@@ -567,12 +567,19 @@
   int rec_dbl;
 };
 
-template <class S, typename TIO, int MAXT, bool FUSED, bool K0 = false>
-__global__ __launch_bounds__(MAXT) void k_pipe(SolveArgs a, PipeTileCfg cfg, ColArgs ca) {
+struct ColArgsBs : ColArgs {
+  BsArgs bs;
+};
+
+template <class S, typename TIO, int MAXT, bool FUSED, bool K0 = false, bool BS = false>
+__global__ __launch_bounds__(MAXT) void k_pipe(SolveArgs a, PipeTileCfg cfg, std::conditional_t<BS, ColArgsBs, ColArgs> ca) {
   static_assert(!K0 || std::is_same<S, Sch2s>::value, "the record prologue forms the 2s record only");
+  static_assert(!BS || (FUSED && sizeof(TIO) == 8), "band sums: fused flush, f64 storage");
   constexpr int VW = 16 / (int)sizeof(TIO);
   typedef TIO vt __attribute__((ext_vector_type(VW)));
   extern __shared__ double lds[];
+  [[maybe_unused]] const BsArgs* bs = nullptr;
+  if constexpr (BS) bs = &ca.bs;
   const int nb = a.nb, nz = a.nz, T = cfg.T;
   const int c = blockIdx.x;
   const int tid = threadIdx.x;
@@ -611,6 +618,12 @@
 #endif
     S st;
     st.init(rec, bin, a);
+    [[maybe_unused]] IntLds BL = {};
+    [[maybe_unused]] double bw[INT_MAXG] = {};
+    if constexpr (BS) {
+      BL = bs_lds_carve(lds + bs->off, T, cfg.ncomp >> 6);
+      bs_setup(BL, bs->ia, nb, b, active, tid >> 6, tid & 63, (1 - (bin.r + bin.t)) * bin.I_dr0, bw);
+    }
     STAMP();
     const bool unif = __builtin_amdgcn_readfirstlane((int)(rec[S_UNIF] != 0.0)) != 0;
     auto sweep = [&](auto mode) {
@@ -626,6 +639,9 @@
 #pragma unroll
             for (int k = 0; k < S::NARR; ++k) tl[k * colrun + t * nb] = (TIO)val[k];
           }
+          if constexpr (BS)
+            int_accumulate<false, false>(BL, cfg.ncomp >> 6, tid >> 6, tid & 63, nz, j0 + t, bs->ia.ngroup, bw, active, val[0], val[1], val[2],
+                                         buf * T + t);
         }
         STAMP();
         lds_barrier();
@@ -693,6 +709,8 @@
 #define SSTAMP() do {} while (0)
 #endif
     SSTAMP();
+    [[maybe_unused]] IntLds BL = {};
+      if constexpr (BS) BL = bs_lds_carve(lds + bs->off, T, cfg.ncomp >> 6);
     int buf = 0;
     for (int j0 = 0; j0 < nz; j0 += T) {
       const int Tc = min(T, nz - j0);
@@ -713,6 +731,9 @@
           p -= nbv;
           ++t;
         }
+      }
+      if constexpr (BS) {
+        if (sid < 64) bs_fold_tile<false>(BL, bs->ia, T, cfg.ncomp >> 6, buf, nz, c, j0, Tc, rec[S_KB], wave_lane(), j0 + Tc >= nz);
       }
       SSTAMP();
       buf ^= 1;
@@ -910,6 +931,29 @@
                     own_k0 ? " k0=fused" : "");
         return (int)CRT_OK;
       };
+      constexpr bool bs_scheme = sizeof(TIO) == 8 && (std::is_same<S, Sch2s>::value || std::is_same<S, Sch4s>::value || std::is_same<S, SchBl>::value);
+      if constexpr (bs_scheme) {
+        const size_t bsb = bs_lds_doubles(Tp, pcomp / 64) * sizeof(double);
+        BandsumReq* const rq = bandsum_request();
+        if (rq && fused && Tp * rq->ia.ngroup <= 64 && bs_lds_fits(psh, bsb)) {
+          ColArgsBs cab;
+          static_cast<ColArgs&>(cab) = own_k0 ? *k0 : ColArgs{};
+          cab.bs = {rq->ia, (int)(psh / sizeof(double))};
+          auto gob = [&](auto kern) {
+            if (!own_k0)
+              if (const int st = k0_before(k0, s)) return st;
+            if (const int st = launch_kernel(kern, dim3(a.ncol), pthr, psh + bsb, s, a, pc, cab)) return st;
+            note_kernel("k_pipe<%s,f64> T=%d store_waves=%d lds=%zu%s +bandsum", S::NAME, Tp, nsw, psh + bsb, own_k0 ? " k0=fused" : "");
+            rq->done = true;
+            return (int)CRT_OK;
+          };
+          int st;
+          if (own_k0) st = pthr <= 512 ? gob(k_pipe<S, TIO, 512, true, can_k0, true>) : gob(k_pipe<S, TIO, 1024, true, can_k0, true>);
+          else st = pthr <= 512 ? gob(k_pipe<S, TIO, 512, true, false, true>) : gob(k_pipe<S, TIO, 1024, true, false, true>);
+          done = st == CRT_OK;
+          return st;
+        }
+      }
       int st;
       if (own_k0) {
         if (fused) st = pthr <= 512 ? gop(k_pipe<S, TIO, 512, true, can_k0>) : gop(k_pipe<S, TIO, 1024, true, can_k0>);
diff --git a/crt1d_amd/csrc/solve_tridiag_tile.hip b/crt1d_amd/csrc/solve_tridiag_tile.hip
--- a/crt1d_amd/csrc/solve_tridiag_tile.hip
+++ b/crt1d_amd/csrc/solve_tridiag_tile.hip
@@ -16,6 +16,12 @@
   va_end(ap);
 }
 const char* last_kernel() { return g_last_kernel; }
+
+namespace {
+thread_local BandsumReq* g_bandsum_request = nullptr;
+}
+void set_bandsum_request(BandsumReq* rq) { g_bandsum_request = rq; }
+BandsumReq* bandsum_request() { return g_bandsum_request; }
 
 int launch_tridiag_int(int scheme, const SolveArgs& a, const IntArgs& ia, hipStream_t s, const SeriesArgs* sr) {
   if (scheme == CRT_SCHEME_N79) return a.f32 ? launch_tri_int_n79_f32(a, ia, s, sr) : launch_tri_int_n79_f64(a, ia, s, sr);
diff --git a/crt1d_amd/csrc/tri_tile_impl.hpp b/crt1d_amd/csrc/tri_tile_impl.hpp
--- a/crt1d_amd/csrc/tri_tile_impl.hpp
+++ b/crt1d_amd/csrc/tri_tile_impl.hpp
@@ -831,8 +831,10 @@
   void* out[4];
 };
 
-template <class S, typename TIO, int M, int T, int RS, int NSTG = S::NST, bool PACK = false>
-__device__ __forceinline__ void tri_pipe_compute(const SolveArgs& a, const PipeCfg& cfg, double* lds, const TriBand* band = nullptr) {
+template <class S, typename TIO, int M, int T, int RS, int NSTG = S::NST, bool PACK = false, bool BS = false>
+__device__ __forceinline__ void tri_pipe_compute(const SolveArgs& a, const PipeCfg& cfg, double* lds, const TriBand* band = nullptr,
+                                                 const BsArgs* bs = nullptr) {
+  static_assert(!BS || (RS > 0 && !PACK), "band sums: register-staged pipelines with one column per workgroup");
   const int nb = a.nb, nz = a.nz;
   const int tid = threadIdx.x, nthr = cfg.ncomp;
   const int cl = PACK ? tid / nb : 0;
@@ -859,6 +861,15 @@
     st.template init<TIO>(rec, a, c, b);
   if (active) bandc[b] = st.band_const();
   const int K = S::rows(nz);
+  [[maybe_unused]] IntLds BL = {};
+  [[maybe_unused]] double bw[INT_MAXG] = {};
+  [[maybe_unused]] int pbuf = 0;
+  if constexpr (BS) {
+    BL = bs_lds_carve(lds + bs->off, T, nthr >> 6);
+    const long long ib = (long long)c * a.col_stride + b;
+    const double leaf_a = 1 - (ldio<TIO>(a.leaf_r, ib) + ldio<TIO>(a.leaf_t, ib));
+    bs_setup(BL, bs->ia, nb, b, active, tid >> 6, tid & 63, leaf_a * st.band_const(), bw);
+  }
   TSTAMP();
   const int seg_top = (K - 1) / M, k_top = seg_top * M;
   double be[M], bf[M];
@@ -918,9 +929,15 @@
 #pragma unroll
           for (int q = 0; q < NSTG; ++q) tile[buf * bstride + q * tstride + (i % T) * nb + b] = o[q];
         }
+        if constexpr (BS) {
+          if (k < nz)
+            int_accumulate<false, false>(BL, nthr >> 6, tid >> 6, tid & 63, nz, k, bs->ia.ngroup, bw, active, st.band_const() * rec[REC_HDR + k], o[0],
+                                         o[1], pbuf * T + i % T);
+        }
         if (i % T == 0) {
           TSTAMP();
           lds_barrier();
+          if constexpr (BS) pbuf ^= 1;
           if constexpr (RS > 0)
             lds_barrier();
           else
@@ -932,9 +949,15 @@
   }
 }
 
-template <class S, typename TIO, int M, int T, int RS>
-__device__ __forceinline__ void tri_pipe_store_rs(const SolveArgs& a, const PipeCfg& cfg, double* lds) {
+constexpr int PIPE_RS = 4;
+
+template <class S, typename TIO, int M, int T, int RS, bool BS = false>
+__device__ __forceinline__ void tri_pipe_store_rs(const SolveArgs& a, const PipeCfg& cfg, double* lds, const BsArgs* bs = nullptr) {
   const int nb2 = a.nb >> 1, nz = a.nz;
+  [[maybe_unused]] IntLds BL = {};
+  [[maybe_unused]] int pbuf = 0;
+  if constexpr (BS) BL = bs_lds_carve(lds + bs->off, T, cfg.ncomp >> 6);
+  [[maybe_unused]] const bool fold_wave = BS && __builtin_amdgcn_readfirstlane((int)threadIdx.x - cfg.ncomp) < 64;
   const int c = blockIdx.x;
   const int sid = threadIdx.x - cfg.ncomp, nst = blockDim.x - cfg.ncomp;
   const double* rec = lds;
@@ -993,6 +1016,10 @@
             }
           }
         }
+      }
+      if constexpr (BS) {
+        if (fold_wave) bs_fold_tile<true>(BL, bs->ia, T, cfg.ncomp >> 6, pbuf, nz, c, k, jmax - k + 1, rec[S_KB], wave_lane(), k == 0);
+        pbuf ^= 1;
       }
     }
   }
@@ -1146,10 +1173,18 @@
   }
 }
 
-template <class S, typename TIO, int M, int T, int MAXT, int RS>
-__global__ __launch_bounds__(MAXT) __attribute__((amdgpu_waves_per_eu((RS == 2 || RS == 3) ? 5 : 4))) void k_tri_pipe(SolveArgs a, PipeCfg cfg) {
+struct PipeCfgBs : PipeCfg {
+  BsArgs bs;
+};
+
+template <class S, typename TIO, int M, int T, int MAXT, int RS, bool BS = false>
+__global__ __launch_bounds__(MAXT) __attribute__((amdgpu_waves_per_eu((RS == 2 || RS == 3) ? 5 : 4))) void k_tri_pipe(
+    SolveArgs a, std::conditional_t<BS, PipeCfgBs, PipeCfg> cfg) {
   static_assert(M % T == 0, "tile height must divide the checkpoint spacing");
+  static_assert(!BS || (RS == PIPE_RS && sizeof(TIO) == 8), "band sums: four-pair register-staged form, f64 storage");
   extern __shared__ double lds[];
+  [[maybe_unused]] const BsArgs* bs = nullptr;
+  if constexpr (BS) bs = &cfg.bs;
   if constexpr (RS == 3) {
     const int c0 = blockIdx.x * cfg.cpw;
     const int nhere = min(cfg.cpw, a.ncol - c0);
@@ -1179,7 +1214,7 @@
   __syncthreads();
   if ((int)threadIdx.x >= cfg.ncomp) {
     if constexpr (RS > 0)
-      tri_pipe_store_rs<S, TIO, M, T, RS>(a, cfg, lds);
+      tri_pipe_store_rs<S, TIO, M, T, RS, BS>(a, cfg, lds, bs);
     else if constexpr (RS < 0)
       tri_pipe_store_generic<S, TIO, M, T>(a, cfg, lds);
     else
@@ -1189,14 +1224,13 @@
   typedef typename UniformOf<S>::type SU;
   if constexpr (!std::is_same<S, SU>::value) {
     if (lds[S_UNIF] != 0.0) {
-      tri_pipe_compute<SU, TIO, M, T, RS>(a, cfg, lds);
+      tri_pipe_compute<SU, TIO, M, T, RS, SU::NST, false, BS>(a, cfg, lds, nullptr, bs);
       return;
     }
   }
-  tri_pipe_compute<S, TIO, M, T, RS>(a, cfg, lds);
-}
-
-constexpr int PIPE_RS = 4;
+  tri_pipe_compute<S, TIO, M, T, RS, S::NST, false, BS>(a, cfg, lds, nullptr, bs);
+}
+
 
 template <class S, typename TIO, int M, int T>
 int launch_pipe_generic(const SolveArgs& a, hipStream_t s, int nstore_waves) {
@@ -1274,6 +1308,22 @@
                 regstage ? (narrow_rs ? "register-staged(2 pairs)" : "register-staged") : "double-buffered", M, T, nstore_waves, sh);
     return (int)CRT_OK;
   };
+  if constexpr (std::is_same<S, TriZq>::value && sizeof(TIO) == 8 && M <= 12) {
+    const size_t bsb = bs_lds_doubles(T, ncomp / 64) * sizeof(double);
+    BandsumReq* const rq = bandsum_request();
+    if (rq && regstage && !narrow_rs && T * rq->ia.ngroup <= 64 && bs_lds_fits(sh, bsb)) {
+      PipeCfgBs cb;
+      static_cast<PipeCfg&>(cb) = cfg;
+      cb.bs = {rq->ia, (int)(sh / sizeof(double))};
+      auto gob = [&](auto kern) {
+        if (const int st = launch_kernel(kern, dim3(a.ncol), nthr, sh + bsb, s, a, cb)) return st;
+        note_kernel("k_tri_pipe<%s,f64> register-staged M=%d T=%d store_waves=%d lds=%zu +bandsum", S::NAME, M, T, nstore_waves, sh + bsb);
+        rq->done = true;
+        return (int)CRT_OK;
+      };
+      return nthr <= 512 ? gob(k_tri_pipe<S, TIO, M, T, 512, PIPE_RS, true>) : gob(k_tri_pipe<S, TIO, M, T, 1024, PIPE_RS, true>);
+    }
+  }
   if constexpr (T == 4 && M == 8) {
     if (narrow_rs) return go(k_tri_pipe<S, TIO, M, T, 512, 2>);
   }
diff --git a/crt1d_amd/dist.py b/crt1d_amd/dist.py
--- a/crt1d_amd/dist.py
+++ b/crt1d_amd/dist.py
@@ -59,7 +59,7 @@
 
     def __init__(self, scheme, cols, bands, band_w, *, group=None, column_tiles=1, keep_profiles=True, share_profiles=False,
                  solve_fn=None, epilogue_fn=None, integrated_fn=None, placement="auto", always_reduce=False, level_profiles=False,
-                 finish_fn=None, **opts):
+                 finish_fn=None, bandsum_separate=False, **opts):
         self.scheme, self.group = scheme, group
         self.level_profiles = bool(level_profiles)
         self.always_reduce = always_reduce
@@ -96,8 +96,13 @@
                     plan = batched.Plan(scheme, ct, bt, out=out, placement=placement, **opts)
                     if share_profiles and shared is None:
                         shared = (chi - clo, plan.out)
-                    epi = batched.BandSumPlan(ct, bt, plan.out, bw, out=tile.views, profiles=self.level_profiles)
-                    tile.launch = self._planned_launch(plan, epi)
+                    if self.level_profiles or bt.dtype != torch.float64:
+                        epi = batched.BandSumPlan(ct, bt, plan.out, bw, out=tile.views, profiles=self.level_profiles)
+                        tile.launch = self._planned_launch(plan, epi)
+                    else:
+                        both = batched.SolveBandSumPlan(scheme, ct, bt, bw, out=plan.out, bandsum_out=tile.views, workspace=plan.workspace,
+                                                        separate=bandsum_separate, **opts)
+                        tile.launch = both
                     tile.kernel_plan = plan
                 else:
                     ip = batched.IntegratedPlan(scheme, ct, bt, bw, out=tile.views, profiles=self.level_profiles, **opts)
diff --git a/include/crt1d_hip_bandsum.h b/include/crt1d_hip_bandsum.h
--- /dev/null
+++ b/include/crt1d_hip_bandsum.h
@@ -0,0 +1,22 @@
+#ifndef CRT1D_HIP_BANDSUM_H
+#define CRT1D_HIP_BANDSUM_H
+
+#include "crt1d_hip.h"
+
+#ifdef __cplusplus
+extern "C" {
+#endif
+
+#define CRT_FLAG_BANDSUM_SEPARATE 8
+
+int crt_hip_solve_bandsum_f64(int scheme, const crt_columns* cols, const crt_bands* bands, const crt_options* opts,
+                              const double* band_w, int32_t ngroup, const crt_outputs* out, const crt_bandsum_out* sums,
+                              void* workspace, size_t workspace_bytes, crt_stream_t stream);
+
+int crt_hip_solve_bandsum_lds_fits(size_t solve_lds_bytes, size_t bandsum_lds_bytes);
+size_t crt_hip_solve_bandsum_lds_bytes(int32_t tile_levels, int32_t compute_waves);
+
+#ifdef __cplusplus
+}
+#endif
+#endif
```

Measured after the change: 3.555 billion, median of 5. 2.5% higher.
